# hey-yahei/Quantization.MXNet

Hardware: AMD Instinct MI355X
Metric: images/sec int8-sim MobileNet1.0 (per-layer W8A8, online input quant) (higher is better)
Workload: dtype f32

## Files before the change

### include/fakequant.h

```cpp
#ifndef FAKEQUANT_H_
#define FAKEQUANT_H_

#include <stddef.h>
#include <stdint.h>

#ifdef __cplusplus
extern "C" {
#endif

#define FQ_OK 0
#define FQ_ERR_INVALID 1
#define FQ_ERR_HIP 2

typedef void* fqStream_t;

#define FQ_ACT_SIGNED 1u
#define FQ_ACT_LO_NEG_MAX 2u
#define FQ_ACT_NO_ABS 4u
#define FQ_ACT_NO_EPS 8u

#define FQ_CODES_INT8 0
#define FQ_CODES_UINT8 1
#define FQ_CODES_RANGE 2
#define FQ_CODES_SCALE 3
// ... 10 lines not shown
#define FQ_KERNEL_HISTOGRAM 4
#define FQ_KERNEL_BN_ACT 5
#define FQ_KERNEL_DWCONV 6
#define FQ_KERNEL_PWCONV 7
#define FQ_KERNEL_STEM 8
#define FQ_KERNEL_POOL 9
#define FQ_KERNEL_GLOBAL_MAX 10
#define FQ_KERNEL_CONV3X3 11
#define FQ_KERNEL_DENSE 12
#define FQ_KERNEL_COUNT 13
int fq_profile_enable(int on);
int fq_profile_reset(void);
int fq_profile_read(int kernel_id, double* total_ms, int64_t* launches, double* total_bytes);
int fq_profile_read_moved(int kernel_id, double* total_moved_bytes);
int fq_profile_calibrate(void* scratch, int repeats, double* pair_ms, double* null_kernel_ms, fqStream_t stream);
int fq_profile_launch_overhead(void* scratch, int repeats, double spin_us, double* overhead_ms, double* spin_ms,
                               fqStream_t stream);

size_t fq_act_workspace_bytes(int64_t n);

int fq_absmax_per_sample(const float* x, int64_t n, int64_t inner, unsigned flags, float* out_max,
                         fqStream_t stream);

int fq_batch_mean(const float* v, int64_t n, float* out, fqStream_t stream);
int fq_batch_mean_rows(const float* v, int64_t rows, int64_t n, int64_t row_stride, float* out, fqStream_t stream);

int fq_stat_rows_sum(const float* v, int64_t rows, int64_t n, int64_t row_stride, double* out, fqStream_t stream);
int fq_mean_from_sums(const double* sums, int64_t rows, float* out, fqStream_t stream);

int fq_batch_mean_gathered(const float* packs, int world, int64_t stride, float* out, fqStream_t stream);

int fq_fake_quant_online(const float* x, float* y, int64_t n, int64_t inner, int width, unsigned flags,
                         float* out_current_max, int32_t* codes, void* ws, fqStream_t stream);

int fq_fake_quant_offline(const float* x, float* y, int64_t n, int64_t inner, const float* threshold, int width,
                          unsigned flags, float* out_current_max, int32_t* codes, void* ws, fqStream_t stream);

int fq_fake_quant_online_prestat(const float* x, float* y, int64_t n, int64_t inner, const float* stat, int width,
                                 unsigned flags, float* out_current_max, int32_t* codes, fqStream_t stream);

#define FQ_ACT_NONE 0
#define FQ_ACT_RELU 1
#define FQ_ACT_RELU6 2
#define FQ_STAT_PREZEROED 0x100
int fq_bn_act_stat(const float* x, float* y, int64_t n, int64_t c, int64_t hw, const float* scale,
                   const float* shift, int act, float* stat_out, fqStream_t stream);
int fq_bn_act_maxpool_stat(const float* x, float* y, int64_t n, int64_t c, int64_t h, int64_t w, const float* scale,
                           const float* shift, int act, float* stat_out, fqStream_t stream);

int fq_add_act_stat(const float* a, const float* b, float* y, int64_t n, int64_t inner, int act, float* stat_out,
                    fqStream_t stream);

int fq_bn_act_stat_hist(const float* x, float* y, int64_t n, int64_t c, int64_t hw, const float* scale,
                        const float* shift, int act, float* stat_out, const float* hist_max, int bins, uint64_t* hist,
                        uint32_t* neg_count, fqStream_t stream);
int fq_add_act_stat_hist(const float* a, const float* b, float* y, int64_t n, int64_t inner, int act, float* stat_out,
                         const float* hist_max, int bins, uint64_t* hist, uint32_t* neg_count, fqStream_t stream);

int fq_bn_add_act_stat(const float* x, const float* residual, float* y, int64_t n, int64_t c, int64_t hw, const float* scale,
                       const float* shift, int act, float* stat_out, fqStream_t stream);
int fq_bn_add_act_stat_hist(const float* x, const float* residual, float* y, int64_t n, int64_t c, int64_t hw,
                            const float* scale, const float* shift, int act, float* stat_out, const float* hist_max, int bins,
                            uint64_t* hist, uint32_t* neg_count, fqStream_t stream);

int fq_global_avg_pool_stat(const float* x, float* y, int64_t n, int64_t c, int64_t hw, int flags, float* stat_out,
                            fqStream_t stream);

int fq_gemm_i8_codes(const int8_t* xcodes, const int8_t* wcodes, const int32_t* wsum, int32_t* out, int64_t n,
                     int64_t l, int64_t k_pad, int64_t cout, int zoff, fqStream_t stream);

int fq_eval_counters(const float* logits, const int64_t* labels, int64_t n, int64_t classes, float* counters,
                     fqStream_t stream);

int fq_stem_conv3x3s2(const float* x, const float* w_tap_major, const float* bias, float* y, int64_t n, int64_t cin,
                      int64_t cout, int64_t h, int64_t w, const float* bn_scale, const float* bn_shift, int act,
                      float* stat_out, fqStream_t stream);
int fq_stem_conv3x3s2_c16(const float* x, const float* w_tap_major, const float* bias, void* y16, int64_t n, int64_t cin,
                          int64_t cout, int64_t h, int64_t w, const float* bn_scale, const float* bn_shift, int act,
                          float* stat_out, const float* out_thr, int out_width, unsigned out_flags, fqStream_t stream);
int fq_stem_conv7x7s2(const float* x, const float* w_tap_major, const float* bias, float* y, int64_t n, int64_t cin,
                      int64_t cout, int64_t h, int64_t w, const float* bn_scale, const float* bn_shift, int act,
                      float* stat_out, fqStream_t stream);
int fq_stem_conv7x7s2_pool_supported(int64_t h, int64_t w);
int fq_stem_conv7x7s2_pool(const float* x, const float* w_tap_major, const float* bias, float* y, int64_t n, int64_t cin,
                           int64_t cout, int64_t h, int64_t w, const float* bn_scale, const float* bn_shift, int act,
                           float* stat_out, fqStream_t stream);

int fq_dwconv3x3(const float* x, const float* w, const float* bias, float* y, int64_t n, int64_t c, int64_t h,
                 int64_t wdt, int stride, const float* in_stat, const float* in_thr, int in_width, unsigned in_flags,
                 float* out_current_max, const float* bn_scale, const float* bn_shift, int act, float* stat_out,
                 fqStream_t stream, void* x_codes_out);

int fq_weight_codes(const float* w, int64_t rows, int64_t row_len, int rows_per_scale, int width, int64_t row_pad,
                    int64_t rows_pad, int8_t* codes, float* scales, int32_t* rowsum, void* ws, fqStream_t stream);
#define FQ_PW_FORM(f) ((f) << 12)
size_t fq_pwconv_workspace_bytes(int64_t n, int64_t cin_pad, int64_t hw);
int fq_pwconv_i8(const float* x, const int8_t* wcodes, const float* wscale, const int32_t* wsum, const float* bias,
                 float* y, int64_t n, int64_t cin, int64_t cin_pad, int64_t cout, int64_t hw, const float* in_stat,
                 const float* in_thr, int in_width, unsigned in_flags, float* out_current_max,
                 const float* bn_scale, const float* bn_shift, int act, float* stat_out, void* ws,
                 fqStream_t stream);

size_t fq_dense_i8_eval_workspace_bytes(int64_t n, int64_t cout);
int fq_dense_i8_eval(const float* x, const int8_t* wcodes, const float* wscale, const int32_t* wsum, const float* bias,
                     float* y, int64_t n, int64_t cin, int64_t cin_pad, int64_t cout, const float* in_stat,
                     const float* in_thr, int in_width, unsigned in_flags, float* out_current_max,
                     const int64_t* labels, float* counters, void* eval_ws, void* ws, fqStream_t stream);

int fq_pwconv_i8_strided(const float* x, const int8_t* wcodes, const float* wscale, const int32_t* wsum,
                         const float* bias, float* y, int64_t n, int64_t cin, int64_t cin_pad, int64_t cout, int64_t h,
                         int64_t w, int stride, const float* in_stat, const float* in_thr, int in_width,
                         unsigned in_flags, float* out_current_max, const float* bn_scale, const float* bn_shift,
                         int act, float* stat_out, const float* residual, void* ws, fqStream_t stream);

int fq_pwconv_i8_sub2_supported(int64_t cin, int64_t cout);
int fq_pwconv_i8_sub2(const float* x, const int8_t* wcodes, const float* wscale, const int32_t* wsum, const float* bias,
                      float* y, int64_t n, int64_t cin, int64_t cin_pad, int64_t cout, int64_t h, int64_t w,
                      const float* in_stat, const float* in_thr, int in_width, unsigned in_flags, float* out_current_max,
                      const float* bn_scale, const float* bn_shift, int act, float* stat_out, const float* residual, void* ws,
                      fqStream_t stream);

int fq_pwconv_i8_shortcut_supported(int64_t cin, int64_t cin2, int64_t cout);
int fq_pwconv_i8_shortcut(const float* x, const int8_t* wcodes, const float* wscale, const int32_t* wsum, const float* bias,
                          float* y, int64_t n, int64_t cin, int64_t cin_pad, int64_t cout, int64_t hw, const float* in_stat,
                          const float* in_thr, int in_width, unsigned in_flags, float* out_current_max, const float* bn_scale,
                          const float* bn_shift, int act, float* stat_out, const float* x2, const int8_t* wcodes2,
                          const float* wscale2, const int32_t* wsum2, int64_t cin2, int64_t cin2_pad, const float* in_stat2,
                          const float* in_thr2, int in_width2, unsigned in_flags2, float* out_current_max2,
                          const float* bn_scale2, const float* bn_shift2, fqStream_t stream);

int fq_pwconv_i8_shortcut_c16(const void* x, const int8_t* wcodes, const float* wscale, const int32_t* wsum, const float* bias,
                              float* y, void* y16, int64_t n, int64_t cin, int64_t cin_pad, int64_t cout, int64_t hw,
                              const float* in_stat, const float* in_thr, int in_width, unsigned in_flags, float* out_current_max,
                              const float* bn_scale, const float* bn_shift, int act, float* stat_out, const void* x2, int x2_is_c16,
                              const int8_t* wcodes2, const float* wscale2, const int32_t* wsum2, int64_t cin2, int64_t cin2_pad,
                              const float* in_stat2, const float* in_thr2, int in_width2, unsigned in_flags2,
                              float* out_current_max2, const float* bn_scale2, const float* bn_shift2, const float* out_thr,
                              int out_width, unsigned out_flags, fqStream_t stream);

int fq_pwconv_i8_gap_supported(int64_t n, int64_t cin, int64_t cout, int64_t hw, int has_residual);
int fq_pwconv_i8_gap(const float* x, const int8_t* wcodes, const float* wscale, const int32_t* wsum, const float* bias,
                     float* y, int64_t n, int64_t cin, int64_t cin_pad, int64_t cout, int64_t hw, const float* in_stat,
                     const float* in_thr, int in_width, unsigned in_flags, float* out_current_max, const float* bn_scale,
                     const float* bn_shift, int act, float* stat_out, const float* residual, void* ws, fqStream_t stream);

int fq_pwconv_i8_stat_supported(int64_t n, int64_t cin, int64_t cout, int64_t hw, int64_t front_h, int64_t front_wdt);
int fq_pwconv_i8_stat(const float* x, const int8_t* wcodes, const float* wscale, const int32_t* wsum, const float* bias,
                      int64_t n, int64_t cin, int64_t cin_pad, int64_t cout_pad, int64_t cout, int64_t hw,
                      const float* in_stat, const float* in_thr, int in_width, unsigned in_flags, float* out_current_max,
                      const float* bn_scale, const float* bn_shift, int act, float* stat_out, void* x_codes_out,
                      fqStream_t stream, const void* front_codes, const float* front_w, const float* front_bias,
                      const float* front_bn_scale, const float* front_bn_shift, int front_act, const float* front_in_stat,
                      const float* front_in_thr, int front_width, unsigned front_flags, int64_t front_h, int64_t front_wdt);
int fq_pwdw_fused_supported(int64_t n, int64_t cin, int64_t cout, int64_t h, int64_t w, int stride);
int fq_debug_fast_quotient(const float* c, int64_t n, const float* d, float* out, int* took_fast_path, fqStream_t stream);
int fq_pwdw_fused(const float* x, const int8_t* wcodes, const float* wscale, const int32_t* wsum, const float* pw_bias,
                  int64_t n, int64_t cin, int64_t cin_pad, int64_t cout_pad, int64_t cout, int64_t h, int64_t w,
                  const float* in_stat, const float* in_thr, int in_width, unsigned in_flags, const float* pw_bn_scale,
                  const float* pw_bn_shift, int pw_act, const float* mid_stat, const float* mid_thr, int mid_width,
                  unsigned mid_flags, float* mid_current_max, const float* dw_w, const float* dw_bias, int dw_stride,
                  const float* dw_bn_scale, const float* dw_bn_shift, int dw_act, float* y, float* stat_out,
                  const void* x_codes, fqStream_t stream);

int fq_pwconv_i8_c16(const void* x, int x_is_c16, const int8_t* wcodes, const float* wscale, const int32_t* wsum,
                     const float* bias, void* y, int64_t n, int64_t cin, int64_t cin_pad, int64_t cout, int64_t h, int64_t w,
                     int stride, const float* in_stat, const float* in_thr, int in_width, unsigned in_flags,
                     float* out_current_max, const float* bn_scale, const float* bn_shift, int act, float* stat_out,
                     const float* residual, const float* out_thr, int out_width, unsigned out_flags, void* ws,
                     fqStream_t stream);

int fq_pwconv_i8_c16_dual(const void* x, const int8_t* wcodes, const float* wscale, const int32_t* wsum, const float* bias,
                          float* y, void* y16, int64_t n, int64_t cin, int64_t cin_pad, int64_t cout, int64_t h, int64_t w,
                          const float* in_stat, const float* in_thr, int in_width, unsigned in_flags, float* out_current_max,
                          const float* bn_scale, const float* bn_shift, int act, float* stat_out, const float* residual,
                          const float* out_thr, int out_width, unsigned out_flags, void* ws, fqStream_t stream);
int fq_pwconv_i8_c16_dual_sub2(const void* x, const int8_t* wcodes, const float* wscale, const int32_t* wsum, const float* bias,
                               float* y, void* y16, int64_t n, int64_t cin, int64_t cin_pad, int64_t cout, int64_t h, int64_t w,
                               const float* in_stat, const float* in_thr, int in_width, unsigned in_flags,
                               float* out_current_max, const float* bn_scale, const float* bn_shift, int act, float* stat_out,
                               const float* residual, const float* out_thr, int out_width, unsigned out_flags, void* ws,
                               fqStream_t stream);

int fq_conv3x3_i8(const float* x, const int8_t* wcodes, const float* wscale, const int32_t* wsum, const float* bias,
                  float* y, int64_t n, int64_t cin, int64_t cout, int64_t h, int64_t w, const float* in_stat,
                  const float* in_thr, int in_width, unsigned in_flags, float* out_current_max, const float* bn_scale,
                  const float* bn_shift, int act, float* stat_out, fqStream_t stream);

int fq_conv3x3_i8_c16(const void* x, int x_is_c16, const int8_t* wcodes, const float* wscale, const int32_t* wsum,
                      const float* bias, void* y, int64_t n, int64_t cin, int64_t cout, int64_t h, int64_t w,
                      const float* in_stat, const float* in_thr, int in_width, unsigned in_flags, float* out_current_max,
                      const float* bn_scale, const float* bn_shift, int act, float* stat_out, const float* out_thr,
                      int out_width, unsigned out_flags, fqStream_t stream);

int fq_dwconv3x3_c16(const void* x, const float* w, const float* bias, void* y, int64_t n, int64_t c, int64_t h, int64_t wdt,
                     int stride, const float* in_stat, const float* in_thr, int in_width, unsigned in_flags,
                     float* out_current_max, const float* bn_scale, const float* bn_shift, int act, float* stat_out,
                     const float* out_thr, int out_width, unsigned out_flags, fqStream_t stream);

int fq_weight_slices(const float* w, int64_t rows, int64_t row_len, int64_t row_pad, int64_t rows_pad, int8_t* codes,
                     float* pscale, int32_t* rowsum, void* ws, fqStream_t stream);
int fq_conv3x3_i8_sliced(const float* x, const int8_t* wslices, const float* pscale, const int32_t* wsum, const float* bias,
                         float* y, int64_t n, int64_t cin, int64_t cout, int64_t h, int64_t w, const float* in_stat,
                         const float* in_thr, int in_width, unsigned in_flags, float* out_current_max,
                         const float* bn_scale, const float* bn_shift, int act, float* stat_out, fqStream_t stream);

int fq_ste_forward(const float* x, float* y, int64_t rows, int64_t row_len, const float* scales, int has_clip,
                   float clip_lo, float clip_hi, float eps, fqStream_t stream);

size_t fq_weight_workspace_bytes(int64_t rows);
int fq_weight_fake_quant(const float* w, float* w_q, int64_t rows, int64_t row_len, int width, float* scales_out,
                         void* ws, fqStream_t stream);

int fq_wino_weight_fake_quant(const float* w, float* w_q, int64_t cout, int64_t cin_g, int t, const float* G,
                              const float* GI, const float* GTI, int width, float* scales_out, void* ws,
                              fqStream_t stream);

#define FQ_COMM_UNIQUE_ID_BYTES 128
#define FQ_COMM_SUM 0
#define FQ_COMM_MAX 1
int fq_comm_unique_id(void* id128);
int fq_comm_init(int rank, int world, const void* id128);
int fq_comm_world(void);
int fq_allreduce_f32(float* buf, int64_t count, int op, fqStream_t stream);
int fq_allreduce_f64(double* buf, int64_t count, int op, fqStream_t stream);
int fq_allreduce_i64(int64_t* buf, int64_t count, int op, fqStream_t stream);
int fq_comm_destroy(void);

int fq_ema_update(float* state, const float* current, int64_t count, double momentum, fqStream_t stream);

int fq_global_max(const float* x, int64_t numel, float* out, fqStream_t stream);

int fq_histogram_accumulate(const float* x, int64_t numel, const float* max_dev, int bins, uint64_t* hist,
                            uint32_t* neg_count, fqStream_t stream);
int fq_hist_to_float(const uint64_t* hist, float* out, int64_t count, fqStream_t stream);

size_t fq_kl_workspace_bytes(int64_t L, int bins);
int fq_kl_search(const float* hist, int64_t L, int bins, int levels, int min_bins, int32_t* out_best, void* ws,
                 fqStream_t stream);

int fq_quantize_codes(const float* x, int32_t* codes, int64_t numel, int mode, float* range_dev, void* ws,
                      fqStream_t stream);
int fq_dequantize(const int32_t* codes, float* y, int64_t numel, const float* scale_dev, fqStream_t stream);

size_t fq_qconv_weights_bytes(int64_t cin, int64_t cout, int kh, int kw, int sh, int sw, int ph, int pw, int groups);
int fq_qconv_kind(int64_t cin, int64_t cout, int kh, int kw, int sh, int sw, int ph, int pw, int groups);
int fq_qconv_weights_prepare(const float* w, int64_t cin, int64_t cout, int kh, int kw, int sh, int sw, int ph, int pw,
                             int groups, int weight_mode, float w_min, float w_max, void* wbuf, void* ws,
                             fqStream_t stream);
size_t fq_qconv_workspace_bytes(int64_t cout);
int fq_qconv_workspace_init(void* ws, fqStream_t stream);
int fq_qconv2d_forward(const float* x, const float* w, const void* wbuf, const float* bias, float* y, int64_t n, int64_t cin,
                       int64_t h, int64_t wdt, int64_t cout, int kh, int kw, int sh, int sw, int ph, int pw, int groups,
                       int input_mode, float in_min, float in_max, const float* in_stat, int act, const float* bn_scale,
                       const float* bn_shift, float* stat_out, void* ws, int force_direct, fqStream_t stream);

#ifdef __cplusplus
}
#endif
#endif
```

### quantization/mxnet_amd/_lib.py

```python
import ctypes
import os

__all__ = ["LIB", "check_call", "load", "library_path", "FakeQuantError", "EXPORTS"]

_HERE = os.path.dirname(os.path.abspath(__file__))
_LIB_PATH = os.environ.get("FQ_LIB_PATH") or os.path.join(_HERE, "csrc", "libfakequant.so")

c_f32p = ctypes.POINTER(ctypes.c_float)
c_i32p = ctypes.POINTER(ctypes.c_int32)
c_u32p = ctypes.POINTER(ctypes.c_uint32)
c_u64p = ctypes.POINTER(ctypes.c_uint64)
_vp, _i64, _int, _uint, _f32 = ctypes.c_void_p, ctypes.c_int64, ctypes.c_int, ctypes.c_uint, ctypes.c_float

EXPORTS = {
    "fq_last_error": (ctypes.c_char_p, []),
    "fq_version": (_int, []),
    "fq_build_id": (ctypes.c_char_p, []),
    "fq_device_info": (_int, [ctypes.c_char_p, _int, ctypes.POINTER(_int), ctypes.POINTER(_int)]),
    "fq_profile_enable": (_int, [_int]),
    "fq_profile_reset": (_int, []),
    "fq_profile_read": (_int, [_int, ctypes.POINTER(ctypes.c_double), ctypes.POINTER(_i64),
                               ctypes.POINTER(ctypes.c_double)]),
    "fq_profile_read_moved": (_int, [_int, ctypes.POINTER(ctypes.c_double)]),
    "fq_profile_calibrate": (_int, [_vp, _int, ctypes.POINTER(ctypes.c_double), ctypes.POINTER(ctypes.c_double), _vp]),
    "fq_profile_launch_overhead": (_int, [_vp, _int, ctypes.c_double, ctypes.POINTER(ctypes.c_double),
                                          ctypes.POINTER(ctypes.c_double), _vp]),
    "fq_act_workspace_bytes": (ctypes.c_size_t, [_i64]),
    "fq_absmax_per_sample": (_int, [_vp, _i64, _i64, _uint, _vp, _vp]),
    "fq_batch_mean": (_int, [_vp, _i64, _vp, _vp]),
    "fq_batch_mean_gathered": (_int, [_vp, _int, _i64, _vp, _vp]),
    "fq_stat_rows_sum": (_int, [_vp, _i64, _i64, _i64, _vp, _vp]),
    "fq_mean_from_sums": (_int, [_vp, _i64, _vp, _vp]),
    "fq_batch_mean_rows": (_int, [_vp, _i64, _i64, _i64, _vp, _vp]),
    "fq_fake_quant_online": (_int, [_vp, _vp, _i64, _i64, _int, _uint, _vp, _vp, _vp, _vp]),
    "fq_fake_quant_online_prestat": (_int, [_vp, _vp, _i64, _i64, _vp, _int, _uint, _vp, _vp, _vp]),
    "fq_bn_act_stat": (_int, [_vp, _vp, _i64, _i64, _i64, _vp, _vp, _int, _vp, _vp]),
    "fq_bn_act_maxpool_stat": (_int, [_vp, _vp, _i64, _i64, _i64, _i64, _vp, _vp, _int, _vp, _vp]),
    "fq_add_act_stat": (_int, [_vp, _vp, _vp, _i64, _i64, _int, _vp, _vp]),
    "fq_bn_act_stat_hist": (_int, [_vp, _vp, _i64, _i64, _i64, _vp, _vp, _int, _vp, _vp, _int, _vp, _vp, _vp]),
    "fq_add_act_stat_hist": (_int, [_vp, _vp, _vp, _i64, _i64, _int, _vp, _vp, _int, _vp, _vp, _vp]),
    "fq_bn_add_act_stat": (_int, [_vp, _vp, _vp, _i64, _i64, _i64, _vp, _vp, _int, _vp, _vp]),
    "fq_bn_add_act_stat_hist": (_int, [_vp, _vp, _vp, _i64, _i64, _i64, _vp, _vp, _int, _vp, _vp, _int, _vp, _vp, _vp]),
    "fq_global_avg_pool_stat": (_int, [_vp, _vp, _i64, _i64, _i64, _int, _vp, _vp]),
    "fq_gemm_i8_codes": (_int, [_vp, _vp, _vp, _vp, _i64, _i64, _i64, _i64, _int, _vp]),
    "fq_eval_counters": (_int, [_vp, _vp, _i64, _i64, _vp, _vp]),
    "fq_stem_conv3x3s2": (_int, [_vp, _vp, _vp, _vp, _i64, _i64, _i64, _i64, _i64, _vp, _vp, _int, _vp, _vp]),
    "fq_stem_conv7x7s2": (_int, [_vp, _vp, _vp, _vp, _i64, _i64, _i64, _i64, _i64, _vp, _vp, _int, _vp, _vp]),
    "fq_stem_conv7x7s2_pool": (_int, [_vp, _vp, _vp, _vp, _i64, _i64, _i64, _i64, _i64, _vp, _vp, _int, _vp, _vp]),
    "fq_stem_conv7x7s2_pool_supported": (_int, [_i64, _i64]),
    "fq_stem_conv3x3s2_c16": (_int, [_vp, _vp, _vp, _vp, _i64, _i64, _i64, _i64, _i64, _vp, _vp, _int, _vp, _vp, _int, _uint, _vp]),
    "fq_dwconv3x3": (_int, [_vp, _vp, _vp, _vp, _i64, _i64, _i64, _i64, _int, _vp, _vp, _int, _uint, _vp, _vp, _vp, _int,
                            _vp, _vp, _vp]),
    "fq_dwconv3x3_c16": (_int, [_vp, _vp, _vp, _vp, _i64, _i64, _i64, _i64, _int, _vp, _vp, _int, _uint, _vp, _vp, _vp, _int,
                                _vp, _vp, _int, _uint, _vp]),
    "fq_weight_codes": (_int, [_vp, _i64, _i64, _int, _int, _i64, _i64, _vp, _vp, _vp, _vp, _vp]),
    "fq_pwconv_workspace_bytes": (ctypes.c_size_t, [_i64, _i64, _i64]),
    "fq_pwconv_i8": (_int, [_vp, _vp, _vp, _vp, _vp, _vp, _i64, _i64, _i64, _i64, _i64, _vp, _vp, _int, _uint, _vp, _vp,
                            _vp, _int, _vp, _vp, _vp]),
    "fq_pwconv_i8_stat_supported": (_int, [_i64, _i64, _i64, _i64, _i64, _i64]),
    "fq_pwconv_i8_stat": (_int, [_vp, _vp, _vp, _vp, _vp, _i64, _i64, _i64, _i64, _i64, _i64, _vp, _vp, _int, _uint, _vp, _vp,
                                 _vp, _int, _vp, _vp, _vp, _vp, _vp, _vp, _vp, _vp, _int, _vp, _vp, _int, _uint, _i64, _i64]),
    "fq_pwdw_fused_supported": (_int, [_i64, _i64, _i64, _i64, _i64, _int]),
    "fq_pwdw_fused": (_int, [_vp, _vp, _vp, _vp, _vp, _i64, _i64, _i64, _i64, _i64, _i64, _i64, _vp, _vp, _int, _uint, _vp,
                             _vp, _int, _vp, _vp, _int, _uint, _vp, _vp, _vp, _int, _vp, _vp, _int, _vp, _vp, _vp, _vp]),
    "fq_debug_fast_quotient": (_int, [_vp, _i64, _vp, _vp, _vp, _vp]),
    "fq_dense_i8_eval_workspace_bytes": (ctypes.c_size_t, [_i64, _i64]),
    "fq_dense_i8_eval": (_int, [_vp, _vp, _vp, _vp, _vp, _vp, _i64, _i64, _i64, _i64, _vp, _vp, _int, _uint, _vp, _vp, _vp,
                                _vp, _vp, _vp]),
    "fq_pwconv_i8_strided": (_int, [_vp, _vp, _vp, _vp, _vp, _vp, _i64, _i64, _i64, _i64, _i64, _i64, _int, _vp, _vp, _int,
                                    _uint, _vp, _vp, _vp, _int, _vp, _vp, _vp, _vp]),
    "fq_pwconv_i8_shortcut_supported": (_int, [_i64, _i64, _i64]),
    "fq_pwconv_i8_shortcut": (_int, [_vp, _vp, _vp, _vp, _vp, _vp, _i64, _i64, _i64, _i64, _i64, _vp, _vp, _int, _uint, _vp, _vp,
                                     _vp, _int, _vp, _vp, _vp, _vp, _vp, _i64, _i64, _vp, _vp, _int, _uint, _vp, _vp, _vp, _vp]),
    "fq_pwconv_i8_shortcut_c16": (_int, [_vp, _vp, _vp, _vp, _vp, _vp, _vp, _i64, _i64, _i64, _i64, _i64, _vp, _vp, _int, _uint, _vp,
                                         _vp, _vp, _int, _vp, _vp, _int, _vp, _vp, _vp, _i64, _i64, _vp, _vp, _int, _uint, _vp, _vp,
                                         _vp, _vp, _int, _uint, _vp]),
    "fq_pwconv_i8_gap_supported": (_int, [_i64, _i64, _i64, _i64, _int]),
    "fq_pwconv_i8_gap": (_int, [_vp, _vp, _vp, _vp, _vp, _vp, _i64, _i64, _i64, _i64, _i64, _vp, _vp, _int, _uint, _vp, _vp, _vp,
                                _int, _vp, _vp, _vp, _vp]),
    "fq_pwconv_i8_sub2_supported": (_int, [_i64, _i64]),
    "fq_pwconv_i8_sub2": (_int, [_vp, _vp, _vp, _vp, _vp, _vp, _i64, _i64, _i64, _i64, _i64, _i64, _vp, _vp, _int,
                                 _uint, _vp, _vp, _vp, _int, _vp, _vp, _vp, _vp]),
    "fq_pwconv_i8_c16": (_int, [_vp, _int, _vp, _vp, _vp, _vp, _vp, _i64, _i64, _i64, _i64, _i64, _i64, _int, _vp, _vp, _int,
                                _uint, _vp, _vp, _vp, _int, _vp, _vp, _vp, _int, _uint, _vp, _vp]),
    "fq_pwconv_i8_c16_dual": (_int, [_vp, _vp, _vp, _vp, _vp, _vp, _vp, _i64, _i64, _i64, _i64, _i64, _i64, _vp, _vp, _int,
                                     _uint, _vp, _vp, _vp, _int, _vp, _vp, _vp, _int, _uint, _vp, _vp]),
    "fq_pwconv_i8_c16_dual_sub2": (_int, [_vp, _vp, _vp, _vp, _vp, _vp, _vp, _i64, _i64, _i64, _i64, _i64, _i64, _vp, _vp, _int,
                                          _uint, _vp, _vp, _vp, _int, _vp, _vp, _vp, _int, _uint, _vp, _vp]),
    "fq_conv3x3_i8": (_int, [_vp, _vp, _vp, _vp, _vp, _vp, _i64, _i64, _i64, _i64, _i64, _vp, _vp, _int, _uint, _vp, _vp,
                             _vp, _int, _vp, _vp]),
    "fq_conv3x3_i8_c16": (_int, [_vp, _int, _vp, _vp, _vp, _vp, _vp, _i64, _i64, _i64, _i64, _i64, _vp, _vp, _int, _uint, _vp,
                                 _vp, _vp, _int, _vp, _vp, _int, _uint, _vp]),
    "fq_conv3x3_i8_sliced": (_int, [_vp, _vp, _vp, _vp, _vp, _vp, _i64, _i64, _i64, _i64, _i64, _vp, _vp, _int, _uint, _vp,
                                    _vp, _vp, _int, _vp, _vp]),
    "fq_weight_slices": (_int, [_vp, _i64, _i64, _i64, _i64, _vp, _vp, _vp, _vp, _vp]),
    "fq_fake_quant_offline": (_int, [_vp, _vp, _i64, _i64, _vp, _int, _uint, _vp, _vp, _vp, _vp]),
    "fq_ste_forward": (_int, [_vp, _vp, _i64, _i64, _vp, _int, _f32, _f32, _f32, _vp]),
    "fq_weight_workspace_bytes": (ctypes.c_size_t, [_i64]),
    "fq_weight_fake_quant": (_int, [_vp, _vp, _i64, _i64, _int, _vp, _vp, _vp]),
    "fq_wino_weight_fake_quant": (_int, [_vp, _vp, _i64, _i64, _int, c_f32p, c_f32p, c_f32p, _int, _vp, _vp, _vp]),
    "fq_comm_unique_id": (_int, [_vp]),
    "fq_comm_init": (_int, [_int, _int, _vp]),
    "fq_comm_world": (_int, []),
    "fq_allreduce_f32": (_int, [_vp, _i64, _int, _vp]),
    "fq_allreduce_f64": (_int, [_vp, _i64, _int, _vp]),
    "fq_allreduce_i64": (_int, [_vp, _i64, _int, _vp]),
    "fq_comm_destroy": (_int, []),
    "fq_ema_update": (_int, [_vp, _vp, _i64, ctypes.c_double, _vp]),
    "fq_global_max": (_int, [_vp, _i64, _vp, _vp]),
    "fq_histogram_accumulate": (_int, [_vp, _i64, _vp, _int, _vp, _vp, _vp]),
    "fq_hist_to_float": (_int, [_vp, _vp, _i64, _vp]),
    "fq_kl_workspace_bytes": (ctypes.c_size_t, [_i64, _int]),
    "fq_kl_search": (_int, [_vp, _i64, _int, _int, _int, _vp, _vp, _vp]),
    "fq_quantize_codes": (_int, [_vp, _vp, _i64, _int, _vp, _vp, _vp]),
    "fq_dequantize": (_int, [_vp, _vp, _i64, _vp, _vp]),
    "fq_qconv_weights_bytes": (ctypes.c_size_t, [_i64, _i64, _int, _int, _int, _int, _int, _int, _int]),
    "fq_qconv_kind": (_int, [_i64, _i64, _int, _int, _int, _int, _int, _int, _int]),
    "fq_qconv_weights_prepare": (_int, [_vp, _i64, _i64, _int, _int, _int, _int, _int, _int, _int, _int, _f32, _f32, _vp,
                                        _vp, _vp]),
    "fq_qconv_workspace_bytes": (ctypes.c_size_t, [_i64]),
    "fq_qconv_workspace_init": (_int, [_vp, _vp]),
    "fq_qconv2d_forward": (_int, [_vp, _vp, _vp, _vp, _vp, _i64, _i64, _i64, _i64, _i64, _int, _int, _int, _int, _int, _int,
                                  _int, _int, _f32, _f32, _vp, _int, _vp, _vp, _vp, _vp, _int, _vp]),
}

FQ_ACT_SIGNED, FQ_ACT_LO_NEG_MAX, FQ_ACT_NO_ABS, FQ_ACT_NO_EPS = 1, 2, 4, 8
FQ_CODES_INT8, FQ_CODES_UINT8, FQ_CODES_RANGE, FQ_CODES_SCALE = 0, 1, 2, 3


class FakeQuantError(RuntimeError):
    """Error raised by the HIP library (the analogue of MXNetError)."""


class _Missing(object):
    def __init__(self, why):
        self._why = why

    def __getattr__(self, name):
        raise FakeQuantError(
            "libfakequant.so is not available (%s). Build it with `python -m quantization.mxnet_amd.csrc.build` "
            "(needs hipcc, target gfx950). There is no CPU fallback for the fake-quant path." % self._why)


def library_path():
    return _LIB_PATH


def load(path=None):
    import torch
    path = path or _LIB_PATH
    if not os.path.exists(path):
        return _Missing("no file at %s" % path)
    try:
        lib = ctypes.CDLL(path, mode=ctypes.RTLD_GLOBAL)
    except OSError as e:
        return _Missing(str(e))
    for name, (restype, argtypes) in EXPORTS.items():
        fn = getattr(lib, name)
        fn.restype = restype
        fn.argtypes = argtypes
    return lib


LIB = load()


def check_call(ret):
    if ret != 0:
        raise FakeQuantError(LIB.fq_last_error().decode("utf-8", "replace"))
```

### quantization/mxnet_amd/csrc/fq_core.hip

```cpp
#include "fq_common.h"

namespace fqi {

thread_local char g_err[512] = "";

int fail(int code, const char* fmt, ...) {
  va_list ap;
  va_start(ap, fmt);
  vsnprintf(g_err, sizeof(g_err), fmt, ap);
  va_end(ap);
  return code;
}

bool g_prof_on = false;
std::mutex g_prof_mu;
std::vector<ProfRec> g_prof;

void prof_push(const ProfRec& r) {
  std::lock_guard<std::mutex> lk(g_prof_mu);
  g_prof.push_back(r);
}

int num_cu() {
  constexpr int kMaxDev = 64;
  static int cache[kMaxDev] = {0};
  int dev = 0;
  if (hipGetDevice(&dev) != hipSuccess || dev < 0 || dev >= kMaxDev) return 256;
  if (cache[dev] == 0) {
    hipDeviceProp_t prop;
    int cu = 0;
    if (hipGetDeviceProperties(&prop, dev) == hipSuccess) cu = prop.multiProcessorCount;
    cache[dev] = cu > 0 ? cu : 256;
  }
  return cache[dev];
}

int max_lds_bytes() {
  constexpr int kMaxDev = 64;
  static int cache[kMaxDev] = {0};
  int dev = 0;
  if (hipGetDevice(&dev) != hipSuccess || dev < 0 || dev >= kMaxDev) return 160 * 1024;
  if (cache[dev] == 0) {
    int v = 0;
    if (hipDeviceGetAttribute(&v, hipDeviceAttributeMaxSharedMemoryPerBlock, dev) != hipSuccess || v <= 0) v = 160 * 1024;
    cache[dev] = v;
  }
  return cache[dev];
}

int env_int(const char* name, int dflt) {
  const char* e = getenv(name);
  return (e && *e) ? atoi(e) : dflt;
}

constexpr int kPolNtLoad_ = 1, kPolNtStore_ = 2, kPolReverse_ = 4;
int stream_policy(int kernel_id, int64_t numel) {
  static const int ov_stat = env_int("FQ_POLICY_STAT", -1);
  static const int ov_on = env_int("FQ_POLICY_ONLINE", -1);
  static const int ov_off = env_int("FQ_POLICY_OFFLINE", -1);
  static const int64_t big = (int64_t)env_int("FQ_POLICY_BIG_MB", 160) * 1000000;
  const bool is_big = numel * (int64_t)sizeof(float) >= big;
  switch (kernel_id) {
    case FQ_KERNEL_STAT:
      return ov_stat >= 0 ? ov_stat : 0;
    case FQ_KERNEL_APPLY_ONLINE:
      if (ov_on >= 0) return ov_on;
      return is_big ? (kPolReverse_ | kPolNtLoad_ | kPolNtStore_) : kPolReverse_;
    default:
      if (ov_off >= 0) return ov_off;
      return is_big ? (kPolNtLoad_ | kPolNtStore_) : 0;
  }
}

}

using namespace fqi;

extern "C" {

const char* fq_last_error(void) { return g_err; }
int fq_version(void) { return 101; }
#ifndef FQ_BUILD_ID
#define FQ_BUILD_ID "0000000000000000000000000000000000000000"
#endif
const char* fq_build_id(void) {
  static const char id[] = "FQ_BUILD_ID=" FQ_BUILD_ID;
  return id + 12;
}

int fq_device_info(char* arch, int arch_len, int* compute_units, int* wavefront) {
  int dev = 0;
  FQ_HIP(hipGetDevice(&dev));
  hipDeviceProp_t prop;
  FQ_HIP(hipGetDeviceProperties(&prop, dev));
  if (arch != nullptr && arch_len > 0) {
    strncpy(arch, prop.gcnArchName, (size_t)arch_len - 1);
    arch[arch_len - 1] = 0;
  }
  if (compute_units) *compute_units = prop.multiProcessorCount;
  if (wavefront) *wavefront = prop.warpSize;
  return FQ_OK;
}

int fq_profile_enable(int on) {
  g_prof_on = on != 0;
  return FQ_OK;
}

int fq_profile_reset(void) {
  std::lock_guard<std::mutex> lk(g_prof_mu);
  for (auto& r : g_prof) {
    (void)hipEventDestroy(r.a);
    (void)hipEventDestroy(r.b);
  }
  g_prof.clear();
  return FQ_OK;
}

int fq_profile_read_moved(int kernel_id, double* total_moved_bytes) {
  FQ_REQUIRE(kernel_id >= 0 && kernel_id < FQ_KERNEL_COUNT, "fq_profile_read_moved: bad kernel id %d", kernel_id);
  FQ_REQUIRE(total_moved_bytes, "fq_profile_read_moved: null pointer");
  std::lock_guard<std::mutex> lk(g_prof_mu);
  double moved = 0.0;
  for (auto& r : g_prof)
    if (r.kid == kernel_id) moved += r.moved;
  *total_moved_bytes = moved;
  return FQ_OK;
}

int fq_profile_read(int kernel_id, double* total_ms, int64_t* launches, double* total_bytes) {
  FQ_REQUIRE(kernel_id >= 0 && kernel_id < FQ_KERNEL_COUNT, "fq_profile_read: bad kernel id %d", kernel_id);
  FQ_REQUIRE(total_ms && launches && total_bytes, "fq_profile_read: null pointer");
  std::lock_guard<std::mutex> lk(g_prof_mu);
  double ms = 0.0, bytes = 0.0;
  int64_t cnt = 0;
  for (auto& r : g_prof) {
    if (r.kid != kernel_id) continue;
    FQ_HIP(hipEventSynchronize(r.b));
    float t = 0.f;
    FQ_HIP(hipEventElapsedTime(&t, r.a, r.b));
    ms += t;
    bytes += r.bytes;
    ++cnt;
  }
  *total_ms = ms;
  *launches = cnt;
  *total_bytes = bytes;
  return FQ_OK;
}

}

namespace {
__global__ void spin_kernel(unsigned long long* __restrict__ t, unsigned long long ticks) {
  const unsigned long long t0 = wall_clock64();
  unsigned long long t1 = t0;
  while (t1 - t0 < ticks) t1 = wall_clock64();
  if (threadIdx.x == 0) {
    t[0] = t0;
    t[1] = t1;
  }
}
}

extern "C" {

int fq_profile_calibrate(void* scratch, int repeats, double* pair_ms, double* null_kernel_ms, fqStream_t stream) {
  FQ_REQUIRE(scratch && pair_ms && null_kernel_ms && repeats > 0 && repeats <= 4096, "fq_profile_calibrate: bad arguments");
  hipStream_t st = (hipStream_t)stream;
  std::vector<hipEvent_t> ev((size_t)repeats * 2 + 2);
  for (auto& e : ev) FQ_HIP(hipEventCreate(&e));
  for (int i = 0; i < repeats; ++i) {
    FQ_HIP(hipEventRecord(ev[2 * i], st));
    hipLaunchKernelGGL(fill_kernel, dim3(1), dim3(64), 0, st, (float*)scratch, (int64_t)1, 0.0f);
    FQ_HIP(hipEventRecord(ev[2 * i + 1], st));
  }
  FQ_HIP(hipEventRecord(ev[2 * repeats], st));
  for (int i = 0; i < repeats; ++i)
    hipLaunchKernelGGL(fill_kernel, dim3(1), dim3(64), 0, st, (float*)scratch, (int64_t)1, 0.0f);
  FQ_HIP(hipEventRecord(ev[2 * repeats + 1], st));
  FQ_HIP(hipEventSynchronize(ev.back()));
  std::vector<float> ts;
  for (int i = 0; i < repeats; ++i) {
    float t = 0.f;
    FQ_HIP(hipEventElapsedTime(&t, ev[2 * i], ev[2 * i + 1]));
    ts.push_back(t);
  }
  float all = 0.f;
  FQ_HIP(hipEventElapsedTime(&all, ev[2 * repeats], ev[2 * repeats + 1]));
  for (auto& e : ev) (void)hipEventDestroy(e);
  std::sort(ts.begin(), ts.end());
  *pair_ms = ts[ts.size() / 2];
  *null_kernel_ms = (double)all / repeats;
  return FQ_OK;
}

int fq_profile_launch_overhead(void* scratch, int repeats, double spin_us, double* overhead_ms, double* spin_ms,
                               fqStream_t stream) {
  FQ_REQUIRE(scratch && overhead_ms && spin_ms && repeats > 0 && repeats <= 4096 && spin_us > 0 && spin_us < 1e5,
             "fq_profile_launch_overhead: bad arguments");
  hipStream_t st = (hipStream_t)stream;
  int dev = 0, khz = 0;
  FQ_HIP(hipGetDevice(&dev));
  FQ_HIP(hipDeviceGetAttribute(&khz, hipDeviceAttributeWallClockRate, dev));
  FQ_REQUIRE(khz > 0, "fq_profile_launch_overhead: the device reports no wall clock rate");
  const unsigned long long ticks = (unsigned long long)(spin_us * 1e-3 * khz);
  std::vector<hipEvent_t> ev((size_t)repeats * 2 + 2);
  for (auto& e : ev) FQ_HIP(hipEventCreate(&e));
  unsigned long long* t = (unsigned long long*)scratch;
  for (int i = 0; i < repeats; ++i) {
    FQ_HIP(hipEventRecord(ev[2 * i], st));
    hipLaunchKernelGGL(spin_kernel, dim3(1), dim3(64), 0, st, t + 2 * i, ticks);
    FQ_HIP(hipEventRecord(ev[2 * i + 1], st));
  }
  FQ_HIP(hipEventRecord(ev[2 * repeats], st));
  for (int i = 0; i < repeats; ++i) hipLaunchKernelGGL(spin_kernel, dim3(1), dim3(64), 0, st, t + 2 * i, ticks);
  FQ_HIP(hipEventRecord(ev[2 * repeats + 1], st));
  FQ_LAUNCH_CHECK();
  FQ_HIP(hipStreamSynchronize(st));
  std::vector<unsigned long long> host((size_t)repeats * 2);
  FQ_HIP(hipMemcpy(host.data(), t, host.size() * sizeof(unsigned long long), hipMemcpyDeviceToHost));
  std::vector<double> pair, own;
  for (int i = 0; i < repeats; ++i) {
    float el = 0.f;
    FQ_HIP(hipEventElapsedTime(&el, ev[2 * i], ev[2 * i + 1]));
    pair.push_back((double)el);
    own.push_back((double)(host[2 * i + 1] - host[2 * i]) / (double)khz);
  }
  float all = 0.f;
  FQ_HIP(hipEventElapsedTime(&all, ev[2 * repeats], ev[2 * repeats + 1]));
  for (auto& e : ev) (void)hipEventDestroy(e);
  std::sort(pair.begin(), pair.end());
  std::sort(own.begin(), own.end());
  *overhead_ms = pair[pair.size() / 2] - (double)all / repeats;
// ... 6 lines not shown
```

### quantization/mxnet_amd/csrc/fq_front_layout.h

```cpp
#pragma once

#include <cstddef>
#include <cstdint>

#if defined(__HIPCC__)
#define FQ_FL_FN __host__ __device__ __forceinline__
#else
#define FQ_FL_FN inline
#endif

namespace fqi {

constexpr int kFrontRows = 8;
constexpr int kFrontBandBytes = 32768;
constexpr int kStatLdsPerCU = 160 * 1024, kStatLdsMax = 120 * 1024;

struct FrontLayout {
  int js;
  int pl;
};

FQ_FL_FN FrontLayout front_layout(int q, int rows) {
  FrontLayout l;
  l.js = rows * q + ((8 - rows * q) & 15);
  l.pl = 4 * l.js + 16;
  return l;
}

FQ_FL_FN int front_slot(FrontLayout l, int p) { return (p & 3) * l.js + (p >> 2); }

FQ_FL_FN int front_byte(FrontLayout l, int c, int p) { return (((c >> 2) * l.pl + front_slot(l, p)) << 2) + (c & 3); }

inline size_t front_band_bytes(int q, int rows, int cin) { return (size_t)((cin + 3) / 4) * front_layout(q, rows).pl * 4; }

FQ_FL_FN int front_channel(int c0, int wave, int segs, int seg) { return c0 + wave * segs + seg; }

FQ_FL_FN int mfma_row_pixel(int i32) { return 16 * ((i32 >> 2) & 1) + 4 * (i32 >> 3) + (i32 & 3); }

inline int stat_wg_per_cu(size_t lds, int cap) {
  const int by_lds = (int)((size_t)kStatLdsPerCU / (lds + 1024));
  return by_lds > cap ? cap : (by_lds < 1 ? 1 : by_lds);
}

inline int front_rows_pick(int64_t n, int64_t h, int64_t w, int cin, size_t lds_fixed, int num_cu, int wg_cap, int forced = 0) {
  const int q = (int)(w / 4);
  int rmax = (int)(kFrontBandBytes / (32 * w));
  rmax = rmax > kFrontRows ? kFrontRows : rmax;
  rmax = rmax > h ? (int)h : rmax;
  while (rmax >= 1 && lds_fixed + front_band_bytes(q, rmax, cin) > (size_t)kStatLdsMax) --rmax;
  if (rmax < 1) return 0;
  if (forced > 0) return forced < rmax ? forced : rmax;
  double best = 1e30;
  int best_r = rmax;
  bool best_whole = false;
  for (int r = rmax; r >= 1; --r) {
    const int64_t wgs = n * ((h + r - 1) / r);
    const int64_t slots = (int64_t)num_cu * stat_wg_per_cu(lds_fixed + front_band_bytes(q, r, cin), wg_cap);
    const int64_t grid = wgs < slots ? wgs : slots, rounds = (wgs + grid - 1) / grid;
    const double cost = (double)(rounds * ((grid + num_cu - 1) / num_cu) * (r + 2));
    const bool whole = (r * w) % 32 == 0;
    if (cost < best - 1e-9 || (cost < best + 1e-9 && whole && !best_whole)) {
      best = cost;
      best_r = r;
      best_whole = whole;
    }
  }
  return best_r;
}

}
```

### quantization/mxnet_amd/csrc/fq_pwdw.hip

```cpp
#include "fq_pw.h"

#include "fq_front_layout.h"

#include <climits>

namespace {

struct PwDwGeom {
  int Cin, KTS, Cout, H, W, Ho, Wo;
  int strips, ctg, bands, RB;
  int zoff, pitch;
  int vw;
  FastDiv qv;
};

constexpr int kRowSlack = 8;

template <int KT, int S> struct PwDwRing {
  static constexpr int NB = S == 1 ? 2 : (KT <= 2 ? 3 : 4);
  static constexpr int NR = 2;
};

template <int KT, int CW, int S, int LZ, int FAST, int CODES>
__global__ __launch_bounds__(512) void pwdw_kernel(
    const float* __restrict__ x, const int8_t* __restrict__ xc, const int8_t* __restrict__ wfrag, const float* __restrict__ wscale,
    const int* __restrict__ wsum, const float* __restrict__ bias1, PwDwGeom g, const float* __restrict__ in_stat, int n,
    const float* __restrict__ in_thr, float levels1, int lo_neg1, float eps, const float* __restrict__ bn1_scale,
    const float* __restrict__ bn1_shift, int act1, const float* __restrict__ mid_stat, const float* __restrict__ mid_thr,
    float levels2, int lo_neg2, float* __restrict__ mid_cur_out, const float* __restrict__ dww,
    const float* __restrict__ bias2, const float* __restrict__ bn2_scale, const float* __restrict__ bn2_shift, int act2,
    float* __restrict__ y, float* __restrict__ stat_out) {
  constexpr int NB = CODES ? 1 : PwDwRing<KT, S>::NB, NR = CODES ? PwDwRing<KT, S>::NR : 1;
  extern __shared__ __attribute__((aligned(16))) unsigned char pwdw_smem[];
  __shared__ float red[8];
  const int CT = g.ctg * CW;
  v4i* ldsW = reinterpret_cast<v4i*>(pwdw_smem);
  const int rb_stride = g.Cout * g.pitch + kRowSlack;
  float* rowbuf = reinterpret_cast<float*>(pwdw_smem + (size_t)CT * KT * 1024) + kRowSlack;
  constexpr bool kDwLds = S == 1;
  float* ldsK = rowbuf + 2 * rb_stride;

  const int lane = threadIdx.x & 63, wave = threadIdx.x >> 6;
  const int h = lane >> 5, i32 = lane & 31;
  const int s = wave % g.strips, cgi = wave / g.strips;
  const int band = (int)(blockIdx.x % (unsigned)g.bands);
  const int smp = n - 1 - (int)(blockIdx.x / (unsigned)g.bands);
  const int HW = g.H * g.W;

  int c0;
  if (S == 1) c0 = (s == g.strips - 1) ? g.W - 30 : 30 * s;
  else c0 = 30 * s;
  const int pl = 16 * ((i32 >> 2) & 1) + 4 * (i32 >> 3) + (i32 & 3);
  int col_ld = c0 + pl - 1;
  col_ld = col_ld < 0 ? 0 : (col_ld >= g.W ? g.W - 1 : col_ld);
  const fq_rsrc rs = CODES ? make_rsrc(xc + (int64_t)smp * 2 * KT * HW * 16, (int64_t)2 * KT * HW * 16)
                           : make_rsrc(x + (int64_t)smp * g.Cin * HW, (int64_t)g.Cin * HW * 4);
  const unsigned voff = CODES ? (unsigned)((h * HW + col_ld) * 16) : (unsigned)((16 * h * HW + col_ld) * 4);
  const int obase = S == 1 ? c0 + 16 * h - 1 : 15 * s + 8 * h;

  const int ro0 = band * g.RB;
  const int ro1 = ro0 + g.RB < g.Ho ? ro0 + g.RB : g.Ho;
  const int t_first = S == 1 ? ro0 - 1 : 2 * ro0 - 1;
  const int t_last = S == 1 ? ro1 : 2 * (ro1 - 1) + 1;
  float* yb = y + (int64_t)smp * g.Cout * g.Ho * g.Wo;

  float raw[NB][16];
#pragma unroll
  for (int b = 0; b < NB; ++b)
#pragma unroll
    for (int i = 0; i < 16; ++i) raw[b][i] = 0.0f;
  auto issue = [&](int t, int kt, float (&v)[16]) __attribute__((always_inline)) {
    if (t < 0 || t >= g.H || t > t_last) return;
    const unsigned so = (unsigned)((kt * 32 * HW + t * g.W) * 4);
#pragma unroll
    for (int i = 0; i < 16; ++i) v[i] = buf_ld_f32(rs, voff, so + (unsigned)(i * HW * 4));
  };
  v4i crow[NR][KT];
#pragma unroll
  for (int b = 0; b < NR; ++b)
#pragma unroll
    for (int kt = 0; kt < KT; ++kt) crow[b][kt] = (v4i){0, 0, 0, 0};
  auto issue_row = [&](int t, v4i (&v)[KT]) __attribute__((always_inline)) {
    if (t < 0 || t >= g.H || t > t_last) return;
#pragma unroll
    for (int kt = 0; kt < KT; ++kt) v[kt] = buf_ld_v4i(rs, voff, (unsigned)((2 * kt * HW + t * g.W) * 16));
  };
  if constexpr (CODES) {
#pragma unroll
    for (int r = 0; r < NR - 1; ++r) issue_row(t_first + r, crow[r]);
  } else {
#pragma unroll
    for (int q = 0; q < NB - 1; ++q) issue(t_first + q / KT, q % KT, raw[q]);
  }
  FQ_PIN();

  const float max1 = input_threshold(in_stat, n, in_thr, nullptr, false);
  const float max2 = input_threshold(mid_stat, n, mid_thr, mid_cur_out, blockIdx.x == 0);
  const QParams q1 = make_qparams(max1, levels1, lo_neg1 != 0, eps);
  const QParams q2 = make_qparams(max2, levels2, lo_neg2 != 0, eps);
  const int ubias1 = 128 - g.zoff;
  const unsigned nn_xor1 = fq_nonneg_xor(ubias1);
  const bool relu6 = act1 == FQ_ACT_RELU6;
  const float top = relu6 ? 6.0f : INFINITY;

  for (int idx = threadIdx.x; idx < CT * KT * 64; idx += blockDim.x) {
    const int f = idx >> 6, ct = f / KT, kt = f - ct * KT;
    ldsW[idx] = *reinterpret_cast<const v4i*>(wfrag + (((int64_t)ct * g.KTS + kt) << 10) + ((idx & 63) << 4));
  }

  float k_sxw[CW], k_b1[CW], k_bsc1[CW], k_bsh1[CW], k_w[CW][9], k_b2[CW], k_bsc2[CW], k_bsh2[CW];
  int k_zs[CW];
  const bool has_b1 = bias1 != nullptr, has_bn1 = bn1_scale != nullptr, has_b2 = bias2 != nullptr, has_bn2 = bn2_scale != nullptr;
#pragma unroll
  for (int j = 0; j < CW; ++j) {
    const int c = (cgi * CW + j) * 32 + i32;
    k_sxw[j] = q1.scale * wscale[c];
    k_zs[j] = g.zoff * wsum[c];
    k_b1[j] = has_b1 ? bias1[c] : 0.0f;
    k_bsc1[j] = has_bn1 ? bn1_scale[c] : 1.0f;
    k_bsh1[j] = has_bn1 ? bn1_shift[c] : 0.0f;
#pragma unroll
    for (int t = 0; t < 9; ++t) k_w[j][t] = kDwLds ? 0.0f : dww[c * 9 + t];
    k_b2[j] = (has_b2 && !kDwLds) ? bias2[c] : 0.0f;
    k_bsc2[j] = (has_bn2 && !kDwLds) ? bn2_scale[c] : 1.0f;
    k_bsh2[j] = (has_bn2 && !kDwLds) ? bn2_shift[c] : 0.0f;
  }
  if (kDwLds)
    for (int c = threadIdx.x; c < g.Cout; c += blockDim.x) {
#pragma unroll
      for (int t = 0; t < 9; ++t) ldsK[c * 13 + t] = dww[c * 9 + t];
      ldsK[c * 13 + 9] = has_b2 ? bias2[c] : 0.0f;
      ldsK[c * 13 + 10] = has_bn2 ? bn2_scale[c] : 1.0f;
      ldsK[c * 13 + 11] = has_bn2 ? bn2_shift[c] : 0.0f;
    }
  const bool zero_left = (S == 1 && LZ != 0) ? (h == (LZ >> 4)) : (s == 0 && h == 0);
  const bool zero_right = S == 1 && s == g.strips - 1 && h == 1;
  __syncthreads();
  FQ_PIN();

  float m = 0.0f;
  const FastQuot fq1 = make_fast_quot(q1.denom), fq2 = make_fast_quot(q2.denom);
  auto body = [&](auto nn_c) __attribute__((always_inline)) {
    constexpr bool NN = decltype(nn_c)::value;
    auto pack_x = [&](float a, float b, float c, float d) __attribute__((always_inline)) {
      if constexpr (NN) {
        auto code = [&](float v) __attribute__((always_inline)) {
          int r;
          const float Q = fast_quot(fq_clip(v, q1), fq1);
          asm("v_cvt_rpi_i32_f32 %0, %1" : "=v"(r) : "v"(Q));
          return (unsigned)r;
        };
        unsigned u = code(a);
        u |= code(b) << 8;
        u |= code(c) << 16;
        u |= code(d) << 24;
        return (int)(u ^ nn_xor1);
      } else {
        return fq_pack4<false>(a, b, c, d, q1, ubias1, nn_xor1);
      }
    };
    constexpr int NO = S == 1 ? 16 : 8;
    float sumA[CW][NO], sumB[S == 1 ? CW : 1][NO];
#pragma unroll
    for (int j = 0; j < CW; ++j)
#pragma unroll
      for (int k = 0; k < NO; ++k) {
        sumA[j][k] = 0.0f;
        if (S == 1) sumB[j][k] = 0.0f;
      }
    QParams qc = q2;
    if (FAST) qc.hi = fminf(q2.hi, top);

    auto row = [&](int t, auto ph_c) __attribute__((always_inline)) {
      constexpr int PH = decltype(ph_c)::value;
      const bool row_ok = t >= 0 && t < g.H;
      v4i afrag[KT];
      if constexpr (CODES) {
        issue_row(t + NR - 1, crow[(PH + NR - 1) % NR]);
        FQ_PIN();
#pragma unroll
        for (int kt = 0; kt < KT; ++kt) afrag[kt] = crow[PH % NR][kt];
      } else {
#pragma unroll
        for (int kt = 0; kt < KT; ++kt) {
          const int qn = kt + NB - 1;
          issue(t + qn / KT, qn % KT, raw[(PH * KT + kt + NB - 1) % NB]);
          FQ_PIN();
          float (&mine)[16] = raw[(PH * KT + kt) % NB];
          v4i f;
#pragma unroll
          for (int d = 0; d < 4; ++d)
            f[d] = pack_x(mine[4 * d + 0], mine[4 * d + 1], mine[4 * d + 2], mine[4 * d + 3]);
          asm volatile("" : "+v"(f[0]), "+v"(f[1]), "+v"(f[2]), "+v"(f[3]));
          afrag[kt] = f;
          FQ_PIN();
        }
      }
      const int r_emit = S == 1 ? t - 1 : (t - 1) >> 1;
      const bool emits = (S == 1 || (t & 1)) && r_emit >= ro0 && r_emit < ro1;
      float* rbuf = rowbuf + (r_emit & 1) * rb_stride;
#pragma unroll
      for (int j = 0; j < CW; ++j) {
        const int ct = cgi * CW + j;
        const float* kc = ldsK + (ct * 32 + i32) * 13;
        auto finish_store = [&](const float (&sum)[NO]) __attribute__((always_inline)) {
          if (!emits) return;
          float* dst = rbuf + (ct * 32 + i32) * g.pitch + obase;
          const float b2 = kDwLds ? kc[9] : k_b2[j], bsc2 = kDwLds ? kc[10] : k_bsc2[j], bsh2 = kDwLds ? kc[11] : k_bsh2[j];
#pragma unroll
          for (int k = 0; k < NO; ++k) {
            float o;
            if (FAST == 0) {
              o = dw_finish<kEpiRuntime>(sum[k], has_b2, b2, has_bn2, bsc2, bsh2, act2);
            } else {
              o = sum[k] * bsc2;
              o = o + bsh2;
              o = __builtin_amdgcn_fmed3f(o, 0.0f, top);
            }
            if (S == 1 && k == 0) {
              if (h == 1) dst[k] = o;
            } else if (k == NO - 1) {
              if (h == 0) dst[k] = o;
            } else {
              dst[k] = o;
            }
          }
        };
        if (!row_ok) {
          if (S == 1) {
            finish_store(sumA[j]);
#pragma unroll
            for (int k = 0; k < 16; ++k) {
              sumA[j][k] = sumB[j][k];
              sumB[j][k] = 0.0f;
            }
          } else if (t & 1) {
            finish_store(sumA[j]);
#pragma unroll
            for (int c = 0; c < 8; ++c) sumA[j][c] = 0.0f;
          }
          FQ_PIN();
          continue;
        }
        float e[18];
        {
          v16i acc = {0, 0, 0, 0, 0, 0, 0, 0, 0, 0, 0, 0, 0, 0, 0, 0};
          int wl = lane;
          asm volatile("" : "+v"(wl));
#pragma unroll
          for (int kt = 0; kt < KT; ++kt)
            acc = __builtin_amdgcn_mfma_i32_32x32x32_i8(afrag[kt], ldsW[((ct * KT + kt) << 6) + wl], acc, 0, 0, 0);
#pragma unroll
          for (int k = 0; k < 16; ++k) {
            float v = (float)(acc[k] + k_zs[j]) * k_sxw[j];
            if (FAST == 0) {
              if (has_b1) v = v + k_b1[j];
              if (has_bn1) {
                v = v * k_bsc1[j];
                v = v + k_bsh1[j];
              }
              v = act_rt(v, act1);
              e[k + 1] = NN ? truncf(fast_quot(fq_clip(v, q2), fq2) + 0.49999997f) * q2.scale : fq_code(v, q2) * q2.scale;
            } else {
              v = v * k_bsc1[j];
              v = v + k_bsh1[j];
              if (NN) e[k + 1] = truncf(fast_quot(fq_clip(v, qc), fq2) + 0.49999997f) * q2.scale;
              else e[k + 1] = fq_code(act_rt(v, relu6 ? FQ_ACT_RELU6 : FQ_ACT_RELU), q2) * q2.scale;
            }
          }
          e[1 + (LZ & 15)] = zero_left ? 0.0f : e[1 + (LZ & 15)];
          if (S == 1) e[16] = zero_right ? 0.0f : e[16];
          const auto sw = __builtin_amdgcn_permlane32_swap(__float_as_uint(e[1]), __float_as_uint(e[16]), false, false);
          e[0] = __uint_as_float(sw[0]);
          e[17] = __uint_as_float(sw[1]);
        }
        float w[9];
        if (!kDwLds) {
#pragma unroll
          for (int t = 0; t < 9; ++t) w[t] = k_w[j][t];
        }
        if (S == 1) {
          w[6] = kc[6]; w[7] = kc[7]; w[8] = kc[8];
#pragma unroll
          for (int k = 0; k < 16; ++k) {
            float a = sumA[j][k];
            a = fmaf(w[6], e[k], a);
            a = fmaf(w[7], e[k + 1], a);
            a = fmaf(w[8], e[k + 2], a);
            sumA[j][k] = a;
          }
          finish_store(sumA[j]);
          w[0] = kc[0]; w[1] = kc[1]; w[2] = kc[2]; w[3] = kc[3]; w[4] = kc[4]; w[5] = kc[5];
#pragma unroll
          for (int k = 0; k < 16; ++k) {
            float b = sumB[j][k];
            b = fmaf(w[3], e[k], b);
            b = fmaf(w[4], e[k + 1], b);
            b = fmaf(w[5], e[k + 2], b);
            float c = 0.0f;
            c = fmaf(w[0], e[k], c);
            c = fmaf(w[1], e[k + 1], c);
            c = fmaf(w[2], e[k + 2], c);
            sumA[j][k] = b;
            sumB[j][k] = c;
          }
        } else {
          if (t & 1) {
#pragma unroll
            for (int c = 0; c < 8; ++c) {
              float a = sumA[j][c];
              a = fmaf(w[6], e[2 * c + 1], a);
              a = fmaf(w[7], e[2 * c + 2], a);
              a = fmaf(w[8], e[2 * c + 3], a);
              sumA[j][c] = a;
            }
            finish_store(sumA[j]);
#pragma unroll
            for (int c = 0; c < 8; ++c) {
              float a = 0.0f;
              a = fmaf(w[0], e[2 * c + 1], a);
              a = fmaf(w[1], e[2 * c + 2], a);
              a = fmaf(w[2], e[2 * c + 3], a);
              sumA[j][c] = a;
            }
          } else {
#pragma unroll
            for (int c = 0; c < 8; ++c) {
              float a = sumA[j][c];
              a = fmaf(w[3], e[2 * c + 1], a);
              a = fmaf(w[4], e[2 * c + 2], a);
              a = fmaf(w[5], e[2 * c + 3], a);
              sumA[j][c] = a;
            }
          }
        }
        FQ_PIN();
      }
      if (emits) {
        __syncthreads();
        const unsigned per_row = g.qv.d;
        const int vecs = g.Cout * (int)per_row;
        float* yr = yb + (int64_t)r_emit * g.Wo;
        for (int idx = threadIdx.x; idx < vecs; idx += blockDim.x) {
          const unsigned c = fast_div((unsigned)idx, g.qv), qd = (unsigned)idx - c * per_row;
          if (g.vw == 4) {
            const float* src = rbuf + c * g.pitch + 4 * qd;
            const f4 v = (f4){src[0], src[1], src[2], src[3]};
            m = fmaxf(fmaxf(m, fmaxf(fabsf(v.x), fabsf(v.y))), fmaxf(fabsf(v.z), fabsf(v.w)));
            *reinterpret_cast<f4*>(yr + (int64_t)c * g.Ho * g.Wo + 4 * qd) = v;
          } else if (g.vw == 2) {
            const float* src = rbuf + c * g.pitch + 2 * qd;
            const float2 v = make_float2(src[0], src[1]);
            m = fmaxf(m, fmaxf(fabsf(v.x), fabsf(v.y)));
            *reinterpret_cast<float2*>(yr + (int64_t)c * g.Ho * g.Wo + 2 * qd) = v;
          } else {
            const float v = rbuf[c * g.pitch + qd];
            m = fmaxf(m, fabsf(v));
            yr[(int64_t)c * g.Ho * g.Wo + qd] = v;
          }
        }
      }
    };
    constexpr int U = CODES ? NR : ((KT % NB == 0) ? 1 : ((2 * KT) % NB == 0 ? 2 : NB));
    static_assert(U <= 3, "the row loop below unrolls at most three phases");
    using std::integral_constant;
    for (int t = t_first; t <= t_last; t += U) {
      row(t, integral_constant<int, 0>{});
      if (U > 1 && t + 1 <= t_last) row(t + 1, integral_constant<int, 1 % U>{});
      if (U > 2 && t + 2 <= t_last) row(t + 2, integral_constant<int, 2 % U>{});
    }
  };
  using std::false_type;
  using std::true_type;
  if (fq_nonneg(q1) && fq_nonneg(q2) && fq1.ok && fq2.ok) body(true_type{});
  else body(false_type{});

  if (stat_out != nullptr) {
    m = wave_max_nonneg(m);
    __syncthreads();
    if (lane == 0) red[wave] = m;
    __syncthreads();
    if (threadIdx.x == 0) {
      float mm = 0.0f;
      for (int w = 0; w < (int)(blockDim.x >> 6); ++w) mm = fmaxf(mm, red[w]);
      if (__float_as_uint(mm) != 0u) FQ_STAT_FLUSH_MAX(reinterpret_cast<unsigned*>(stat_out) + smp, __float_as_uint(mm));
    }
  }
}

__device__ __forceinline__ void buf_st_v4i(fq_rsrc r, unsigned voff, v4i v) {
  typedef unsigned v4u __attribute__((ext_vector_type(4)));
  __builtin_amdgcn_raw_buffer_store_b128(__builtin_bit_cast(v4u, v), r, (int)voff, 0, 0);
  asm volatile("s_nop 1" : : "v"(v));
}

struct PwStatGeom {
  int Cin, KTS, Cout, CT, HW;
  int64_t cols, tiles;
  int zoff;
  int table;
  FastDiv hw;
};

struct PwFrontArgs {
  const int8_t* codes;
  const float *w, *bias, *bn_scale, *bn_shift;
  const float *in_stat, *in_thr;
  float levels;
  int act;
  int H, W, Q, segs, R, bands;
  FrontLayout lay;
};

template <int KT, int FEPI = -1, bool FSIGNED = false>
__global__ __launch_bounds__(kBlock, 3) void pw_stat_kernel(
    const float* __restrict__ x, const int8_t* __restrict__ wfrag, const float* __restrict__ wscale,
    const int* __restrict__ wsum, const float* __restrict__ bias, PwStatGeom g, const float* __restrict__ in_stat, int n,
    const float* __restrict__ in_thr, float levels, int lo_neg, float eps, float* __restrict__ cur_max_out,
    const float* __restrict__ bn_scale, const float* __restrict__ bn_shift, int act, float* __restrict__ stat_out,
    int8_t* __restrict__ x_codes_out, PwFrontArgs fa) {
  constexpr bool FRONT = FEPI >= 0;
  static_assert(!FRONT || KT == 1, "the front layer is built for one 32-channel slab");
  extern __shared__ __attribute__((aligned(16))) unsigned char pst_smem[];
  v4i* ldsW = reinterpret_cast<v4i*>(pst_smem);
  int* c_zs = reinterpret_cast<int*>(pst_smem + (size_t)g.CT * KT * 1024);
  float* c_k = reinterpret_cast<float*>(c_zs + g.CT * 32);
  int* accs = reinterpret_cast<int*>(c_k + 4 * g.CT * 32);
  float* dwk = reinterpret_cast<float*>(accs + 4 * g.CT * 128);
  unsigned char* zbuf = reinterpret_cast<unsigned char*>(dwk + g.Cin * 12);
  const int lane = threadIdx.x & 63, wave = threadIdx.x >> 6;
  const int h = lane >> 5, i32 = lane & 31;
  const unsigned HW = (unsigned)g.HW, cols = (unsigned)g.cols;
  const int64_t nwaves = (int64_t)gridDim.x * 4, wid = (int64_t)blockIdx.x * 4 + wave;
  const int64_t n_bands = FRONT ? (int64_t)(g.cols / g.HW) * fa.bands : 0;
  const int64_t t_begin = FRONT ? n_bands * blockIdx.x / gridDim.x : g.tiles * wid / nwaves;
  const int64_t t_end = FRONT ? n_bands * (blockIdx.x + 1) / gridDim.x : g.tiles * (wid + 1) / nwaves;
  const int pl = mfma_row_pixel(i32);
  int* my = accs + (size_t)wave * g.CT * 128;
  constexpr int kSlots = 8;
  __shared__ unsigned k_stat[kSlots];
  if (threadIdx.x < kSlots) k_stat[threadIdx.x] = 0u;
  unsigned s_base;
  if constexpr (FRONT) {
    s_base = (unsigned)((t_begin < n_bands ? t_begin : n_bands - 1) / fa.bands);
  } else {
    const int64_t t0 = g.tiles * ((int64_t)blockIdx.x * 4) / nwaves;
    const unsigned j0 = (unsigned)(t0 < g.tiles ? t0 : g.tiles - 1) * 32u;
    s_base = fast_div(j0 < cols ? j0 : cols - 1, g.hw);
  }

  struct Pix { unsigned smp, p; };
  auto pix_of = [&](int64_t t) __attribute__((always_inline)) {
    unsigned j = (unsigned)t * 32u + (unsigned)pl;
    j = j < cols ? j : cols - 1;
    Pix r;
    r.smp = fast_div(j, g.hw);
    r.p = j - r.smp * HW;
    return r;
  };
  constexpr int NB = 3;
  const fq_rsrc rs = make_rsrc(x, (int64_t)(cols / HW) * g.Cin * HW * 4);
  auto issue = [&](int64_t t, int kt, float (&v)[16]) __attribute__((always_inline)) {
    if (t >= t_end) return;
    const Pix px = pix_of(t);
    const bool ok = kt * 32 + 16 * h < g.Cin;
    const unsigned vo = ok ? (unsigned)(((px.smp * (unsigned)g.Cin + 16u * h) * HW + px.p) * 4u) : 0x80000000u;
    const unsigned so = (unsigned)kt * 32u * HW * 4u;
#pragma unroll
    for (int i = 0; i < 16; ++i) v[i] = buf_ld_f32(rs, vo, so + (unsigned)i * HW * 4u);
  };
  float raw[NB][16];
#pragma unroll
  for (int b2 = 0; b2 < NB; ++b2)
#pragma unroll
    for (int i = 0; i < 16; ++i) raw[b2][i] = 0.0f;
  if constexpr (!FRONT) {
#pragma unroll
    for (int qq = 0; qq < NB - 1; ++qq) issue(t_begin + qq / KT, qq % KT, raw[qq]);
  }
  FQ_PIN();
  float fscale = 0.0f;
  if constexpr (FRONT) fscale = input_threshold(fa.in_stat, n, fa.in_thr, nullptr, false) / fa.levels;
  const float max_ = input_threshold(in_stat, n, in_thr, cur_max_out, blockIdx.x == 0);
  const QParams q = make_qparams(max_, levels, lo_neg != 0, eps);
  const int ubias = 128 - g.zoff;
  const unsigned nn_xor = fq_nonneg_xor(ubias);
  const bool wr_codes = x_codes_out != nullptr;
  const fq_rsrc rcodes = make_rsrc(x_codes_out, wr_codes ? (int64_t)(cols / HW) * 2 * KT * HW * 16 : 0);
  for (int idx = threadIdx.x; idx < g.CT * KT * 64; idx += kBlock) {
    const int f = idx >> 6, ct = f / KT, kt = f - ct * KT;
    ldsW[idx] = *reinterpret_cast<const v4i*>(wfrag + (((int64_t)ct * g.KTS + kt) << 10) + ((idx & 63) << 4));
  }
  const int nchs = g.CT * 32;
  for (int i = threadIdx.x; i < nchs; i += kBlock) {
    const bool okc = i < g.Cout;
    c_zs[i] = okc ? g.zoff * wsum[i] : 0;
    c_k[i] = okc ? wscale[i] : 0.0f;
    c_k[nchs + i] = (okc && bias != nullptr) ? bias[i] : 0.0f;
    c_k[2 * nchs + i] = (okc && bn_scale != nullptr) ? bn_scale[i] : 1.0f;
    c_k[3 * nchs + i] = (okc && bn_scale != nullptr) ? bn_shift[i] : 0.0f;
  }
  if constexpr (FRONT)
    for (int i = threadIdx.x; i < g.Cin; i += kBlock) {
#pragma unroll
      for (int t = 0; t < 9; ++t) dwk[i * 12 + t] = fa.w[i * 9 + t];
      dwk[i * 12 + 9] = fa.bias != nullptr ? fa.bias[i] : 0.0f;
      dwk[i * 12 + 10] = fa.bn_scale != nullptr ? fa.bn_scale[i] : 1.0f;
      dwk[i * 12 + 11] = fa.bn_scale != nullptr ? fa.bn_shift[i] : 0.0f;
    }
  auto reset = [&]() __attribute__((always_inline)) {
    for (int ct = 0; ct < g.CT; ++ct) {
      my[ct * 128 + lane] = INT_MIN;
      my[ct * 128 + 64 + lane] = INT_MAX;
    }
  };
  reset();
  __syncthreads();
  const bool has_bn = bn_scale != nullptr;
  auto flush = [&](unsigned smp) __attribute__((always_inline)) {
    float m = 0.0f;
    for (int ct = 0; ct < g.CT; ++ct) {
      const int c = ct * 32 + i32;
      int hi = my[ct * 128 + lane], lo = my[ct * 128 + 64 + lane];
      const int ohi = __shfl_xor(hi, 32, 64), olo = __shfl_xor(lo, 32, 64);
      hi = hi > ohi ? hi : ohi;
      lo = lo < olo ? lo : olo;
      if (c < g.Cout && hi >= lo) {
        hi += c_zs[c];
        lo += c_zs[c];
        const float sxw = q.scale * c_k[c];
        const float bch = c_k[nchs + c];
        const float bsc = c_k[2 * nchs + c], bsh = c_k[3 * nchs + c];
        auto f = [&](int a) {
          float v = (float)a * sxw;
          if (bias != nullptr) v = v + bch;
          if (has_bn) {
            v = v * bsc;
            v = v + bsh;
          }
          return fabsf(act_rt(v, act));
        };
        m = fmaxf(m, fmaxf(f(hi), f(lo)));
      }
    }
    m = wave_max_nonneg(m);
    if (lane == 0 && __float_as_uint(m) != 0u) {
      const unsigned slot = smp - s_base;
      if (g.table && slot < (unsigned)kSlots) atomicMax(&k_stat[slot], __float_as_uint(m));
      else FQ_STAT_FLUSH_MAX(reinterpret_cast<unsigned*>(stat_out) + smp, __float_as_uint(m));
    }
    reset();
  };
  v4i afrag[KT];
  const FastQuot fqx = make_fast_quot(q.denom);
  auto quant = [&](int kt, const float (&v)[16], auto nn_c) __attribute__((always_inline)) {
    v4i f;
#pragma unroll
    for (int d = 0; d < 4; ++d) {
      if constexpr (decltype(nn_c)::value) {
        unsigned u = 0u;
#pragma unroll
        for (int b = 0; b < 4; ++b) {
          int r;
          const float Q = fast_quot(fq_clip(v[4 * d + b], q), fqx);
          asm("v_cvt_rpi_i32_f32 %0, %1" : "=v"(r) : "v"(Q));
          u |= (unsigned)r << (8 * b);
        }
        f[d] = (int)(u ^ nn_xor);
      } else {
        f[d] = fq_pack4<false>(v[4 * d + 0], v[4 * d + 1], v[4 * d + 2], v[4 * d + 3], q, ubias, nn_xor);
      }
    }
    asm volatile("" : "+v"(f[0]), "+v"(f[1]), "+v"(f[2]), "+v"(f[3]));
    afrag[kt] = f;
  };
// ... 4 lines not shown
      v16i acc = {0, 0, 0, 0, 0, 0, 0, 0, 0, 0, 0, 0, 0, 0, 0, 0};
#pragma unroll
      for (int kt = 0; kt < KT; ++kt)
        acc = __builtin_amdgcn_mfma_i32_32x32x32_i8(afrag[kt], ldsW[((ct * KT + kt) << 6) + lane], acc, 0, 0, 0);
      int hi = INT_MIN, lo = INT_MAX;
      if (whole) {
#pragma unroll
        for (int k = 0; k < 16; k += 2) {
          hi = max(max(acc[k], acc[k + 1]), hi);
          lo = min(min(acc[k], acc[k + 1]), lo);
        }
      } else {
#pragma unroll
        for (int k = 0; k < 16; ++k) {
          const int p = 16 * h + k;
          const bool in = p >= plo && p < phi;
          hi = in && acc[k] > hi ? acc[k] : hi;
          lo = in && acc[k] < lo ? acc[k] : lo;
        }
      }
      atomicMax(&my[ct * 128 + lane], hi);
      atomicMin(&my[ct * 128 + 64 + lane], lo);
    }
  };
  unsigned cur = FRONT ? s_base : fast_div((unsigned)((t_begin < g.tiles ? t_begin : g.tiles - 1) * 32), g.hw);
  auto run_tile = [&](int64_t t, auto ph_c, auto nn_c) __attribute__((always_inline)) {
    constexpr int PH = decltype(ph_c)::value;
    const Pix px = pix_of(t);
    const unsigned cvo = ((px.smp * (unsigned)(2 * KT) + (unsigned)h) * HW + px.p) * 16u;
#pragma unroll
    for (int kt = 0; kt < KT; ++kt) {
      const int qn = kt + NB - 1;
      issue(t + qn / KT, qn % KT, raw[(PH * KT + kt + NB - 1) % NB]);
      FQ_PIN();
      quant(kt, raw[(PH * KT + kt) % NB], nn_c);
      if (wr_codes) buf_st_v4i(rcodes, cvo + (unsigned)(2 * kt) * HW * 16u, afrag[kt]);
      FQ_PIN();
    }
    const unsigned j0 = (unsigned)t * 32u, j1 = j0 + 31u < cols ? j0 + 31u : cols - 1;
    const unsigned s0 = fast_div(j0, g.hw), s1 = fast_div(j1, g.hw);
    if (s0 != cur) {
      flush(cur);
      cur = s0;
    }
    if (s0 == s1) {
      reduce_tile(0, 32);
    } else {
      const int pb = (int)(s1 * HW - j0);
      reduce_tile(0, pb);
      flush(cur);
      cur = s1;
      reduce_tile(pb, 32);
    }
    FQ_PIN();
  };
  auto run_all = [&](auto nn_c) __attribute__((always_inline)) {
    constexpr int U = (KT % NB == 0) ? 1 : NB;
    using std::integral_constant;
    for (int64_t t = t_begin; t < t_end; t += U) {
      run_tile(t, integral_constant<int, 0>{}, nn_c);
      if (U > 1 && t + 1 < t_end) run_tile(t + 1, integral_constant<int, 1 % U>{}, nn_c);
      if (U > 2 && t + 2 < t_end) run_tile(t + 2, integral_constant<int, 2 % U>{}, nn_c);
      if (U > 3 && t + 3 < t_end) run_tile(t + 3, integral_constant<int, 3 % U>{}, nn_c);
    }
  };
  auto run_front = [&](auto nn_c) __attribute__((always_inline)) {
    constexpr bool NN = decltype(nn_c)::value;
    constexpr int FE = FRONT ? FEPI : kEpiRuntime;
    const int Q = fa.Q, W = fa.W, H = fa.H;
    const int seg = lane / Q, pos = lane - seg * Q;
    const bool first = pos == 0, last = pos == Q - 1;
    const bool has_fb = fa.bias != nullptr, has_fbn = fa.bn_scale != nullptr;
    QParams qc = q;
    if (NN && FE != kEpiRuntime) qc.hi = FE == kEpiBnRelu6 ? fminf(q.hi, 6.0f) : q.hi;
    const unsigned* xc32 = reinterpret_cast<const unsigned*>(fa.codes);
    const int z4 = stored_zero4(ubias);
    const v4i zero_frag = (v4i){z4, z4, z4, z4};
    auto deq = [&](unsigned wd, int b) __attribute__((always_inline)) {
      const int code = FSIGNED ? (int)(int8_t)(wd >> (8 * b)) : (int)((wd >> (8 * b)) & 255u);
      return (float)code * fscale;
    };
    for (int64_t bt = t_begin; bt < t_end; ++bt) {
      const unsigned smp = (unsigned)(bt / fa.bands);
      const int r0 = (int)(bt - (int64_t)smp * fa.bands) * fa.R;
      const int Rb = H - r0 < fa.R ? H - r0 : fa.R;
      if (smp != cur) {
        flush(cur);
        cur = smp;
      }
      for (int c0 = 0; c0 < g.Cin; c0 += 4 * fa.segs) {
        const int c = front_channel(c0, wave, fa.segs, seg);
        const bool c_ok = seg < fa.segs && c < g.Cin;
        const int cc = c_ok ? c : 0;
        const float* kc = dwk + cc * 12;
        const float w00 = kc[0], w01 = kc[1], w02 = kc[2], w10 = kc[3], w11 = kc[4], w12 = kc[5], w20 = kc[6], w21 = kc[7],
                    w22 = kc[8], bch = kc[9], bsc = kc[10], bsh = kc[11];
        const unsigned* src = xc32 + ((int64_t)(smp * (unsigned)g.Cin + (unsigned)cc) * H) * Q + pos;
        unsigned raw_c[kFrontRows + 2];
#pragma unroll
        for (int k = 0; k < kFrontRows + 2; ++k) {
          const int t = r0 - 1 + k, tc = t < 0 ? 0 : (t > H - 1 ? H - 1 : t);
          raw_c[k] = src[tc * Q] & ((t >= 0 && t < H) ? 0xFFFFFFFFu : 0u);
        }
        auto zcode = [&](float acc) __attribute__((always_inline)) {
          if constexpr (NN) {
            const float v = FE == kEpiRuntime ? dw_finish<kEpiRuntime>(acc, has_fb, bch, has_fbn, bsc, bsh, fa.act)
                                              : dw_finish<FE, false>(acc, false, 0.0f, true, bsc, bsh, 0);
            int r;
            const float Qv = fast_quot(fq_clip(v, qc), fqx);
            asm("v_cvt_rpi_i32_f32 %0, %1" : "=v"(r) : "v"(Qv));
            return (unsigned)r ^ (nn_xor & 255u);
          } else {
            const float v = dw_finish<FE>(acc, has_fb, bch, has_fbn, bsc, bsh, fa.act);
            return (unsigned)(fq_code_int(v, q) + ubias) ^ 0x80u;
          }
        };
        float a[6] = {0.f, 0.f, 0.f, 0.f, 0.f, 0.f}, b[6] = {0.f, 0.f, 0.f, 0.f, 0.f, 0.f};
        unsigned dst = (unsigned)front_byte(fa.lay, cc, 4 * pos);
        const unsigned jstep = (unsigned)(front_byte(fa.lay, 0, 1) - front_byte(fa.lay, 0, 0));
        const unsigned rstep = (unsigned)(front_byte(fa.lay, 0, 4 * Q) - front_byte(fa.lay, 0, 0));
#pragma unroll
        for (int k = 0; k < kFrontRows + 2; ++k) {
          if (k <= Rb + 1) {
            float cv[6];
#pragma unroll
            for (int j = 0; j < 4; ++j) cv[j + 1] = deq(raw_c[k], j);
            const float lp = lane_prev(cv[4]), ln = lane_next(cv[1]);
            cv[0] = first ? 0.0f : lp;
            cv[5] = last ? 0.0f : ln;
            if (k >= 2) {
#pragma unroll
              for (int j = 0; j < 4; ++j) {
                const unsigned code = zcode(dw_taps(w00, w01, w02, w10, w11, w12, w20, w21, w22, a[j], a[j + 1], a[j + 2], b[j],
                                                    b[j + 1], b[j + 2], cv[j], cv[j + 1], cv[j + 2]));
                if (c_ok) zbuf[dst + j * jstep] = (unsigned char)code;
              }
              dst += rstep;
              asm volatile("" : "+v"(dst));
            }
#pragma unroll
            for (int j = 0; j < 6; ++j) {
              a[j] = b[j];
              b[j] = cv[j];
            }
          }
        }
      }
      __syncthreads();
      const int npix = Rb * W, ntile = (npix + 31) >> 5;
      for (int tl = wave; tl < ntile; tl += 4) {
        int pp = tl * 32 + pl;
        pp = pp < npix ? pp : npix - 1;
        const unsigned* zp = reinterpret_cast<const unsigned*>(zbuf + front_byte(fa.lay, g.Cin <= 16 ? 0 : 16 * h, pp));
        v4i f;
#pragma unroll
        for (int u = 0; u < 4; ++u) f[u] = (int)zp[u * fa.lay.pl];
        if (g.Cin <= 16 && h == 1) f = zero_frag;
        if (wr_codes) buf_st_v4i(rcodes, ((smp * 2u + (unsigned)h) * HW + (unsigned)(r0 * W + pp)) * 16u, f);
        afrag[0] = f;
        const int valid = npix - tl * 32;
        reduce_tile(0, valid < 32 ? valid : 32);
      }
      __syncthreads();
    }
  };
  if constexpr (FRONT) {
    if (fq_nonneg(q) && fqx.ok) run_front(std::true_type{});
    else run_front(std::false_type{});
  } else {
    if (fq_nonneg(q) && fqx.ok) run_all(std::true_type{});
    else run_all(std::false_type{});
  }
  if (t_begin < t_end) flush(cur);
  __syncthreads();
  if (threadIdx.x < kSlots && k_stat[threadIdx.x] != 0u && s_base + threadIdx.x < cols / HW)
    FQ_STAT_FLUSH_MAX(reinterpret_cast<unsigned*>(stat_out) + s_base + threadIdx.x, k_stat[threadIdx.x]);
}

__global__ void fast_quotient_kernel(const float* __restrict__ c, int64_t n, const float* __restrict__ d, float* __restrict__ out,
                                     int* __restrict__ ok_out) {
  const FastQuot f = make_fast_quot(d[0]);
  const double rden = 1.0 / (double)d[0];
  const int64_t i = (int64_t)blockIdx.x * blockDim.x + threadIdx.x;
  if (i == 0) ok_out[0] = f.ok ? 1 : 0;
  if (i < n) out[i] = f.ok ? fast_quot(c[i], f) : ieee_div_by(c[i], rden);
}

struct PwDwPlan {
  int kt, cw, lz, strips, ctg, bands, rb, pitch, threads;
  size_t lds;
  bool ok;
};

PwDwPlan pwdw_plan(int64_t n, int64_t cin, int64_t cout, int64_t h, int64_t w, int stride) {
  PwDwPlan p;
  memset(&p, 0, sizeof(p));
  if (n <= 0 || cin <= 0 || cout <= 0 || h < 3 || w < 8 || (stride != 1 && stride != 2)) return p;
  if (cout % 32 != 0 || (stride == 2 && (w % 2 != 0 || h % 2 != 0))) return p;
  const int kt = (int)((cin + 31) / 32), ct = (int)(cout / 32);
  if (!(kt == 1 || kt == 2 || kt == 4 || kt == 8)) return p;
  const int wo = (int)((w - 1) / stride + 1), ho = (int)((h - 1) / stride + 1);
  p.kt = kt;
  p.cw = ct % 2 == 0 ? 2 : 1;
  p.strips = (int)((w + 29) / 30);
  p.lz = (stride == 1 && p.strips == 1) ? (int)(30 - w) : 0;
  if (!(p.lz == 0 || p.lz == 2)) return p;
  p.ctg = ct / p.cw;
  p.threads = 64 * p.strips * p.ctg;
  if (p.threads > 512) return p;
  const int reach = stride == 1 ? (int)w + 2 + p.lz : 15 * p.strips + 1;
  p.pitch = (reach > wo ? reach : wo) + p.lz;
  p.pitch |= 1;
  p.lds = (size_t)ct * kt * 1024 + 2 * ((size_t)cout * p.pitch + kRowSlack) * 4 + kRowSlack * 4 + (stride == 1 ? (size_t)cout * 13 * 4 : 0);
  if (p.lds + 10 * 1024 > (size_t)max_lds_bytes()) return p;
  static const int rb_env = env_int("FQ_PWDW_RB", 0);
  {
    const int waves = p.threads / 64;
    int occ = (int)((160 * 1024) / (p.lds + 512));
    const int by_regs = 8 / waves > 0 ? 8 / waves : 1;
    occ = occ < by_regs ? occ : by_regs;
    occ = occ < 1 ? 1 : occ;
    const double slots = (double)num_cu() * occ;
    double best = 1e30;
    int best_rb = ho;
    for (int b = 1; b <= ho; ++b) {
      const int rb = (ho + b - 1) / b, bands = (ho + rb - 1) / rb;
      const double wgs = (double)n * bands, rounds = ceil(wgs / slots), fill = wgs < slots ? wgs / slots : 1.0;
      const double cost = rounds * (stride * rb + 2) / fill;
      if (cost < best - 1e-9) {
        best = cost;
        best_rb = rb;
      }
    }
    p.rb = rb_env > 0 ? (rb_env < ho ? rb_env : ho) : best_rb;
  }
  p.bands = (ho + p.rb - 1) / p.rb;
  if (n * cin * h * w * 4 >= (1ll << 32) || n * cout * ho * wo >= (1ll << 31)) return p;
  p.ok = true;
  return p;
}

}

namespace fqi {

static size_t pw_stat_lds(int kt, int ct) { return (size_t)ct * kt * 1024 + 5 * (size_t)ct * 32 * 4 + 4 * (size_t)ct * 128 * 4; }

bool pw_stat_shape_ok(int64_t n, int64_t cin, int64_t cout, int64_t hw) {
  if (n <= 0 || cin <= 0 || cout <= 0 || hw < 32 || hw >= (1ll << 30) || n * hw >= (1ll << 31) - 512) return false;
  const int kt = (int)((cin + 31) / 32), ct = (int)((cout + 31) / 32);
  if (!(kt == 1 || kt == 2 || kt == 4 || kt == 8) || cin % 16 != 0) return false;
  return pw_stat_lds(kt, ct) <= (size_t)kStatLdsMax && n * cin * hw * 4 < (1ll << 32);
}

constexpr int kFrontWgCap = 4;

static int pw_front_rows(int64_t n, int64_t cin, int64_t cout, int64_t h, int64_t w) {
  const char* e = getenv("FQ_PWSTAT_FRONT_ROWS");
  static const int wg_env = env_int("FQ_PWSTAT_WG_PER_CU", 0);
  const size_t fixed = pw_stat_lds(1, (int)((cout + 31) / 32)) + (size_t)cin * 12 * 4;
  return front_rows_pick(n, h, w, (int)cin, fixed, num_cu(), wg_env > 0 ? wg_env : kFrontWgCap, e != nullptr ? atoi(e) : 0);
}

bool pw_stat_front_shape_ok(int64_t n, int64_t cin, int64_t cout, int64_t h, int64_t w) {
  if (h < 1 || w < 4 || w % 4 != 0 || w / 4 > 64 || !(cin == 16 || cin == 32) || !pw_stat_shape_ok(n, cin, cout, h * w)) return false;
  return pw_front_rows(n, cin, cout, h, w) >= 1 && n * cin * ((w / 4 + 61) / 62) < (1ll << 31) - 1024;
}

int pw_stat_launch(const PwCall& c) {
  const int kt = (int)((c.cin + 31) / 32), ct = (int)((c.cout + 31) / 32);
  size_t lds = pw_stat_lds(kt, ct);
  PwFrontArgs fa = {};
  if (c.front != nullptr) {
    const PwFront& f = *c.front;
    fa.codes = static_cast<const int8_t*>(f.codes);
    fa.w = f.w; fa.bias = f.bias; fa.bn_scale = f.bn_scale; fa.bn_shift = f.bn_shift;
    fa.in_stat = f.in_stat; fa.in_thr = f.in_thr; fa.levels = f.levels; fa.act = f.act;
    fa.H = (int)f.h; fa.W = (int)f.wdt; fa.Q = fa.W / 4; fa.segs = 64 / fa.Q;
    fa.R = pw_front_rows(c.n, c.cin, c.cout, f.h, f.wdt);
    FQ_REQUIRE(fa.R >= 1, "fq_pwconv_i8_stat: no band of the front layer fits the LDS");
    fa.bands = (fa.H + fa.R - 1) / fa.R;
    fa.lay = front_layout(fa.Q, fa.R);
    lds += (size_t)c.cin * 12 * 4 + front_band_bytes(fa.Q, fa.R, (int)c.cin);
  }
  PwStatGeom g;
  g.Cin = (int)c.cin; g.KTS = (int)(c.cin_pad / 32); g.Cout = (int)c.cout; g.CT = ct; g.HW = (int)c.hw;
  g.cols = c.n * c.hw; g.tiles = (g.cols + 31) / 32; g.zoff = c.zoff;
  g.hw = fast_div_for((unsigned)c.hw);
  if (int rc = pw_zero_stat(c)) return rc;
  int per_cu = stat_wg_per_cu(lds, c.front != nullptr ? kFrontWgCap : 3);
  static const int wg_env = env_int("FQ_PWSTAT_WG_PER_CU", 0);
  if (wg_env > 0) per_cu = wg_env;
  int64_t grid = (int64_t)num_cu() * per_cu;
  const int64_t need = c.front != nullptr ? c.n * fa.bands : (g.tiles + 3) / 4;
  if (grid > need) grid = need;
  static const int table_env = env_int("FQ_PWSTAT_TABLE", -1);
  g.table = table_env >= 0 ? table_env : (g.tiles < grid * 4 * 10 ? 1 : 0);
#define FQ_PST_GO(KT_)                                                                                                     \
  case KT_: {                                                                                                              \
    static const bool attr_ok = hipFuncSetAttribute(reinterpret_cast<const void*>(&pw_stat_kernel<KT_>),                   \
                                                    hipFuncAttributeMaxDynamicSharedMemorySize, 120 * 1024) == hipSuccess; \
    FQ_REQUIRE(attr_ok, "fq_pwconv_i8_stat: cannot raise the dynamic LDS limit");                                          \
    hipLaunchKernelGGL((pw_stat_kernel<KT_>), dim3((unsigned)grid), dim3(kBlock), lds, c.st, c.x, c.wcodes, c.wscale,       \
                       (const int*)c.wsum, c.bias, g, c.in_stat, (int)c.n, c.in_thr, c.levels, c.lo_neg, kEps,              \
                       c.out_current_max, c.bn_scale, c.bn_shift, c.act, c.stat_out, (int8_t*)c.x_codes_out, fa);          \
  } break;
#define FQ_PST_FRONT(EPI_, SG_)                                                                                            \
  {                                                                                                                        \
    static const bool attr_ok = hipFuncSetAttribute(reinterpret_cast<const void*>(&pw_stat_kernel<1, EPI_, SG_>),          \
                                                    hipFuncAttributeMaxDynamicSharedMemorySize, 120 * 1024) == hipSuccess; \
    FQ_REQUIRE(attr_ok, "fq_pwconv_i8_stat: cannot raise the dynamic LDS limit");                                          \
    hipLaunchKernelGGL((pw_stat_kernel<1, EPI_, SG_>), dim3((unsigned)grid), dim3(kBlock), lds, c.st, c.x, c.wcodes,       \
                       c.wscale, (const int*)c.wsum, c.bias, g, c.in_stat, (int)c.n, c.in_thr, c.levels, c.lo_neg, kEps,   \
                       c.out_current_max, c.bn_scale, c.bn_shift, c.act, c.stat_out, (int8_t*)c.x_codes_out, fa);          \
  }
#define FQ_PST_FRONT_S(EPI_)                                                                                               \
  {                                                                                                                        \
    if (c.front->is_signed) FQ_PST_FRONT(EPI_, true) else FQ_PST_FRONT(EPI_, false)                                        \
  }
  if (c.front != nullptr) {
    FQ_REQUIRE(kt == 1, "fq_pwconv_i8_stat: a front layer needs cin <= 32");
    if (c.front->epi == kEpiBnRelu) FQ_PST_FRONT_S(kEpiBnRelu)
    else if (c.front->epi == kEpiBnRelu6) FQ_PST_FRONT_S(kEpiBnRelu6)
    else FQ_PST_FRONT_S(kEpiRuntime)
  } else {
    switch (kt) {
      FQ_PST_GO(1) FQ_PST_GO(2) FQ_PST_GO(4) FQ_PST_GO(8)
      default: return fail(FQ_ERR_INVALID, "fq_pwconv_i8_stat: K / 32 = %d is not instantiated", kt);
    }
  }
#undef FQ_PST_FRONT_S
#undef FQ_PST_FRONT
#undef FQ_PST_GO
  FQ_LAUNCH_CHECK();
  return FQ_OK;
}

}

using namespace fqi;

extern "C" {

int fq_debug_fast_quotient(const float* c, int64_t n, const float* d, float* out, int* took_fast_path, fqStream_t stream) {
  FQ_REQUIRE(c && d && out && took_fast_path && n > 0, "fq_debug_fast_quotient: null pointer");
  hipLaunchKernelGGL(fast_quotient_kernel, dim3((unsigned)((n + 255) / 256)), dim3(256), 0, (hipStream_t)stream, c, n, d, out,
                     took_fast_path);
  FQ_LAUNCH_CHECK();
  return FQ_OK;
}

int fq_pwdw_fused_supported(int64_t n, int64_t cin, int64_t cout, int64_t h, int64_t w, int stride) {
  return pwdw_plan(n, cin, cout, h, w, stride).ok ? 1 : 0;
}

int fq_pwdw_fused(const float* x, const int8_t* wcodes, const float* wscale, const int32_t* wsum, const float* pw_bias,
                  int64_t n, int64_t cin, int64_t cin_pad, int64_t cout_pad, int64_t cout, int64_t h, int64_t w,
                  const float* in_stat, const float* in_thr, int in_width, unsigned in_flags, const float* pw_bn_scale,
                  const float* pw_bn_shift, int pw_act, const float* mid_stat, const float* mid_thr, int mid_width,
                  unsigned mid_flags, float* mid_current_max, const float* dw_w, const float* dw_bias, int dw_stride,
                  const float* dw_bn_scale, const float* dw_bn_shift, int dw_act, float* y, float* stat_out,
                  const void* x_codes, fqStream_t stream) {
  FQ_REQUIRE((x || x_codes) && wcodes && wscale && wsum && dw_w && y, "fq_pwdw_fused: null pointer");
  FQ_REQUIRE(in_stat != nullptr || in_thr != nullptr, "fq_pwdw_fused: give in_stat (online) or in_thr (offline)");
  FQ_REQUIRE(mid_stat != nullptr || mid_thr != nullptr, "fq_pwdw_fused: give mid_stat (the per-sample maxima of the pointwise "
             "output, from fq_pwconv_i8_stat) or mid_thr (a stored threshold)");
  FQ_REQUIRE(in_width >= 2 && in_width <= 8, "fq_pwdw_fused: input width %d does not fit int8 codes", in_width);
  FQ_REQUIRE(mid_width >= 2 && mid_width <= 16, "fq_pwdw_fused: bad width %d of the depthwise input", mid_width);
  FQ_REQUIRE(!((in_flags | mid_flags) & (FQ_ACT_NO_ABS | FQ_ACT_NO_EPS)), "fq_pwdw_fused: unsupported activation flags");
  FQ_REQUIRE((pw_bn_scale == nullptr) == (pw_bn_shift == nullptr) && (dw_bn_scale == nullptr) == (dw_bn_shift == nullptr),
             "fq_pwdw_fused: a BatchNorm's scale and shift go together");
  FQ_REQUIRE(cin_pad >= cin && cin_pad % 64 == 0 && cout_pad >= cout && cout_pad % 32 == 0,
             "fq_pwdw_fused: cin_pad / cout_pad must be those of fq_weight_codes");
  const bool prezeroed = (dw_act & FQ_STAT_PREZEROED) != 0;
  dw_act &= ~FQ_STAT_PREZEROED;
  FQ_REQUIRE(pw_act >= FQ_ACT_NONE && pw_act <= FQ_ACT_RELU6 && dw_act >= FQ_ACT_NONE && dw_act <= FQ_ACT_RELU6,
             "fq_pwdw_fused: unknown activation");
  FQ_REQUIRE(aligned16(wcodes) && (x_codes ? aligned16(x_codes) : aligned16(x)) && aligned16(y),
             "fq_pwdw_fused: x (x_codes when given), wcodes and y must be 16-byte aligned");
  const PwDwPlan p = pwdw_plan(n, cin, cout, h, w, dw_stride);
  FQ_REQUIRE(p.ok, "fq_pwdw_fused: shape not taken (n=%lld cin=%lld cout=%lld %lldx%lld stride %d): see fq_pwdw_fused_supported",
             (long long)n, (long long)cin, (long long)cout, (long long)h, (long long)w, dw_stride);
  hipStream_t st = (hipStream_t)stream;
  const int64_t ho = (h - 1) / dw_stride + 1, wo = (w - 1) / dw_stride + 1;
  if (stat_out && !prezeroed) FQ_HIP(hipMemsetAsync(stat_out, 0, n * sizeof(float), st));
  PwDwGeom g;
  g.Cin = (int)cin; g.KTS = (int)(cin_pad / 32); g.Cout = (int)cout; g.H = (int)h; g.W = (int)w; g.Ho = (int)ho; g.Wo = (int)wo;
  g.strips = p.strips; g.ctg = p.ctg; g.bands = p.bands; g.RB = p.rb;
  g.zoff = (in_flags & FQ_ACT_SIGNED) ? 0 : 128;
  g.pitch = p.pitch;
  g.vw = wo % 4 == 0 ? 4 : (wo % 2 == 0 ? 2 : 1);
  g.qv = fast_div_for((unsigned)(wo / g.vw));
  const int8_t* wfrag = wcodes + cout_pad * cin_pad;
  const float levels1 = act_levels(in_width, in_flags), levels2 = act_levels(mid_width, mid_flags);
  const int lo1 = (in_flags & FQ_ACT_LO_NEG_MAX) ? 1 : 0, lo2 = (mid_flags & FQ_ACT_LO_NEG_MAX) ? 1 : 0;
  int fast = 0;
  if (!pw_bias && !dw_bias && pw_bn_scale && dw_bn_scale && !lo1 && !lo2 && pw_act == dw_act &&
      (pw_act == FQ_ACT_RELU || pw_act == FQ_ACT_RELU6))
    fast = 1;
  static const int no_fast = env_int("FQ_PWDW_NO_FAST", 0);
  if (no_fast) fast = 0;
  const double in_elems = (double)n * cin * h * w, mid_elems = (double)n * cout * h * w, out_elems = (double)n * cout * ho * wo;
  const double in_moved = x_codes ? 32.0 * p.kt * (double)n * h * w : 4.0 * in_elems;
  ProfScope prof(FQ_KERNEL_DWCONV, 4.0 * (mid_elems + out_elems), st, in_moved + 4.0 * out_elems);
  const int8_t* xc = static_cast<const int8_t*>(x_codes);
  const unsigned grid = (unsigned)(n * p.bands);
#define FQ_PWDW_GO(KT_, CW_, S_, LZ_, F_, C_)                                                                               \
  {                                                                                                                        \
    static const bool attr_ok = hipFuncSetAttribute(reinterpret_cast<const void*>(&pwdw_kernel<KT_, CW_, S_, LZ_, F_, C_>), \
                                                    hipFuncAttributeMaxDynamicSharedMemorySize, 150 * 1024) == hipSuccess; \
    FQ_REQUIRE(attr_ok, "fq_pwdw_fused: cannot raise the dynamic LDS limit");                                              \
    hipLaunchKernelGGL((pwdw_kernel<KT_, CW_, S_, LZ_, F_, C_>), dim3(grid), dim3((unsigned)p.threads), p.lds, st, x, xc,   \
                       wfrag, wscale, (const int*)wsum, pw_bias, g, in_stat, (int)n, in_thr, levels1, lo1, kEps,            \
                       pw_bn_scale, pw_bn_shift, pw_act, mid_stat, mid_thr, levels2, lo2, mid_current_max, dw_w, dw_bias,   \
                       dw_bn_scale, dw_bn_shift, dw_act, y, stat_out);                                                     \
  }
#define FQ_PWDW_C(KT_, CW_, S_, LZ_, F_)                                                                                    \
  {                                                                                                                        \
    if (xc != nullptr) FQ_PWDW_GO(KT_, CW_, S_, LZ_, F_, 1) else FQ_PWDW_GO(KT_, CW_, S_, LZ_, F_, 0)                       \
  }
#define FQ_PWDW_F(KT_, CW_, S_, LZ_)                                                                                        \
  {                                                                                                                        \
    if (fast == 1) FQ_PWDW_C(KT_, CW_, S_, LZ_, 1) else FQ_PWDW_C(KT_, CW_, S_, LZ_, 0)                                     \
  }
#define FQ_PWDW_S(KT_, CW_)                                                                                                 \
  {                                                                                                                        \
    if (dw_stride == 2) FQ_PWDW_F(KT_, CW_, 2, 0)                                                                          \
    else if (p.lz == 0) FQ_PWDW_F(KT_, CW_, 1, 0) else FQ_PWDW_F(KT_, CW_, 1, 2)                                            \
  }
#define FQ_PWDW_K(KT_)                                                                                                      \
  case KT_:                                                                                                                \
    if (p.cw == 2) FQ_PWDW_S(KT_, 2) else FQ_PWDW_S(KT_, 1)                                                                \
    break;
  switch (p.kt) {
    FQ_PWDW_K(1) FQ_PWDW_K(2) FQ_PWDW_K(4) FQ_PWDW_K(8)
    default: break;
  }
#undef FQ_PWDW_K
#undef FQ_PWDW_S
#undef FQ_PWDW_F
#undef FQ_PWDW_C
#undef FQ_PWDW_GO
  FQ_LAUNCH_CHECK();
  return FQ_OK;
}

}
```

### quantization/mxnet_amd/ops.py

```python
import ctypes
import threading

import numpy as np
import torch

from . import _lib
from ._lib import FakeQuantError

__all__ = ["comm_unique_id", "comm_init", "comm_world", "comm_allreduce", "comm_destroy", "add_act_stat", "bn_act_maxpool_stat", "stat_rows_sum", "mean_from_sums", "fake_quant_online_prestat", "bn_act_stat", "stem_conv3x3s2", "stem_conv_s2", "stem_conv_supported", "eval_counters", "dense_i8_eval", "gemm_i8_codes", "global_avg_pool_stat", "dwconv3x3", "dwconv3x3_c16", "weight_codes", "pwconv_i8", "pwconv_strided_supported", "weight_codes_3x3", "weight_slices_3x3", "conv3x3_i8", "Codes16", "batch_mean_rows", "batch_mean_gathered", "ste_forward", "absmax_per_sample", "batch_mean", "fake_quant_online", "fake_quant_offline", "weight_fake_quant",
           "wino_weight_fake_quant", "ema_update", "global_max", "histogram_accumulate", "hist_to_float",
           "kl_search", "quantize_codes", "dequantize", "qconv_kind", "qconv_weights", "qconv_workspace", "qconv2d",
           "batches_in_flight", "in_flight", "winograd_matrices", "device_info", "act_flags"]

_WS = {}


def _lib_():
    return _lib.LIB


_DEVICE_TLS = threading.local()


def _stream(t):
# ... 422 lines not shown
    check_call(_lib_().fq_dense_i8_eval(_ptr(x), _ptr(wcodes), _ptr(wscale), _ptr(wsum), _ptr(bias), _ptr(y), n, cin,
                                        cin_pad, cout, _ptr(in_stat), _ptr(in_thr), int(width), int(flags), _ptr(cur_out),
                                        lb.data_ptr(), _ptr(counters), ews.data_ptr(), _ptr(ws), _stream(x)))
    return y


def eval_counters(logits, labels, counters):
    _check(logits, "logits")
    _check(counters, "counters")
    require_hip(labels.device, "labels")
    if logits.dim() != 2 or labels.dim() != 1 or labels.shape[0] != logits.shape[0] or labels.dtype != torch.int64:
        raise ValueError("eval_counters wants logits (N, classes) float32 and labels (N,) int64")
    n, classes = logits.shape
    if counters.numel() != 2 + 2 * classes or not counters.is_contiguous():
        raise ValueError("counters must hold 2 + 2*classes contiguous floats")
    lg = logits if logits.is_contiguous() else logits.contiguous()
    lb = labels if labels.is_contiguous() else labels.contiguous()
    check_call(_lib_().fq_eval_counters(_ptr(lg), lb.data_ptr(), n, classes, _ptr(counters), _stream(logits)))
    return counters


def stem_conv_s2(x, w, bias=None, bn_scale=None, bn_shift=None, act=None, want_stat=True, w_tap_major=None, out_codes=None,
                 pool=False):
    _check(x, "x")
    _check(w, "w")
    if x.dim() != 4 or w.dim() != 4 or w.shape[2] != w.shape[3] or w.shape[2] not in (3, 7) or w.shape[1] != x.shape[1]:
        raise ValueError("stem_conv_s2 wants x (N,C,H,W) and w (Cout,C,K,K), K = 3 or 7; got %s and %s"
                         % (tuple(x.shape), tuple(w.shape)))
    for name, t in (("bias", bias), ("bn_scale", bn_scale), ("bn_shift", bn_shift), ("w_tap_major", w_tap_major)):
        if t is not None:
            _check(t, name)
    act = act or "none"
    if act not in _ACTS:
        raise ValueError("unknown activation %r" % (act,))
    n, cin, h, wd = x.shape
    cout, ks = w.shape[0], w.shape[2]
    pad = ks // 2
    wt = w_tap_major if w_tap_major is not None else w.permute(1, 2, 3, 0).contiguous()
    y = torch.empty((n, cout, (h + 2 * pad - ks) // 2 + 1, (wd + 2 * pad - ks) // 2 + 1), dtype=torch.float32,
                    device=x.device)
    stat, zflag = _stat_target(n, x.device, want_stat)
    if out_codes is not None:
        if ks != 3:
            raise ValueError("the first convolution hands codes over in its 3x3 form only")
        othr = _check(out_codes["thr"], "out_codes['thr']")
        yc = Codes16.empty(tuple(y.shape), x.device, othr, out_codes.get("width", 8), out_codes.get("flags", 0))
        check_call(_lib_().fq_stem_conv3x3s2_c16(_ptr(x), _ptr(wt), _ptr(bias), _ptr(yc.t), n, cin, cout, h, wd, _ptr(bn_scale),
                                                 _ptr(bn_shift), _ACTS[act] | zflag, _ptr(stat), _ptr(othr), int(yc.width),
                                                 int(yc.flags), _stream(x)))
        return yc, stat
    if pool:
        if ks != 7 or not stem_pool_supported(h, wd):
            raise ValueError("the pooled form is built for the 7x7 first convolution on planes whose output rows cut into four "
                             "tiles of at most 32 columns; got K = %d on %d x %d" % (ks, h, wd))
        ho, wo = y.shape[2], y.shape[3]
        yp = torch.empty((n, cout, (ho - 1) // 2 + 1, (wo - 1) // 2 + 1), dtype=torch.float32, device=x.device)
        check_call(_lib_().fq_stem_conv7x7s2_pool(_ptr(x), _ptr(wt), _ptr(bias), _ptr(yp), n, cin, cout, h, wd, _ptr(bn_scale),
                                                  _ptr(bn_shift), _ACTS[act] | zflag, _ptr(stat), _stream(x)))
        return yp, stat
    entry = _lib_().fq_stem_conv3x3s2 if ks == 3 else _lib_().fq_stem_conv7x7s2
    check_call(entry(_ptr(x), _ptr(wt), _ptr(bias), _ptr(y), n, cin, cout, h, wd, _ptr(bn_scale), _ptr(bn_shift),
                     _ACTS[act] | zflag, _ptr(stat), _stream(x)))
    return y, stat


stem_conv3x3s2 = stem_conv_s2


def stem_pool_supported(h, w):
    return bool(_lib_().fq_stem_conv7x7s2_pool_supported(int(h), int(w)))


def stem_conv_supported(cin, cout, kernel, stride, pad):
    k, s, p = tuple(kernel), tuple(stride), tuple(pad)
    return cin == 3 and s == (2, 2) and ((cout == 32 and k == (3, 3) and p == (1, 1)) or
                                         (cout == 64 and k == (7, 7) and p == (3, 3)))


def front_codes_shape(xshape):
    n, c, h, w = (int(v) for v in xshape)
    return (n, c, h * w)


def _check_front_codes(t, name, xshape, device):
    _check(t, name, torch.int8)
    if len(xshape) != 4 or tuple(t.shape) != front_codes_shape(xshape):
        raise ValueError("%s must be int8 %s for a depthwise input %s; got %s"
                         % (name, front_codes_shape(xshape) if len(xshape) == 4 else "(4-d x)", tuple(xshape), tuple(t.shape)))
    if t.device != device:
        raise ValueError("%s lives on %s, x on %s" % (name, t.device, device))
    if t.data_ptr() % 16:
        raise ValueError("%s must be 16-byte aligned" % name)
    return t


def dwconv3x3(x, w, bias=None, stride=1, in_stat=None, in_thr=None, width=8, flags=0, cur_out=None, bn_scale=None,
              bn_shift=None, act=None, want_stat=True, store=True, x_codes_out=None):
    _check(x, "x")
    _check(w, "w")
    if x.dim() != 4 or w.dim() != 4 or tuple(w.shape[1:]) != (1, 3, 3) or w.shape[0] != x.shape[1]:
        raise ValueError("dwconv3x3 wants x (N,C,H,W) and w (C,1,3,3); got %s and %s" % (tuple(x.shape), tuple(w.shape)))
    for name, t in (("bias", bias), ("in_stat", in_stat), ("in_thr", in_thr), ("bn_scale", bn_scale),
                    ("bn_shift", bn_shift), ("cur_out", cur_out)):
        if t is not None:
            _check(t, name)
    n, c, h, wd = x.shape
    ho, wo = (h - 1) // stride + 1, (wd - 1) // stride + 1
    if not store and not want_stat:
        raise ValueError("dwconv3x3(store=False) leaves nothing but the statistic: want_stat must be set")
    if x_codes_out is not None:
        if store:
            raise ValueError("dwconv3x3 keeps the codes of x only in its statistic pass (store=False)")
        _check_front_codes(x_codes_out, "x_codes_out", tuple(x.shape), x.device)
    y = torch.empty((n, c, ho, wo), dtype=torch.float32, device=x.device) if store else None
    stat, zflag = _stat_target(n, x.device, want_stat)
    check_call(_lib_().fq_dwconv3x3(_ptr(x), _ptr(w), _ptr(bias), _ptr(y), n, c, h, wd, int(stride), _ptr(in_stat),
                                    _ptr(in_thr), int(width), int(flags), _ptr(cur_out), _ptr(bn_scale),
                                    _ptr(bn_shift), _ACTS[act] | zflag, _ptr(stat), _stream(x), _ptr(x_codes_out)))
    return y, stat


def dwconv3x3_c16(x, w, bias=None, stride=1, in_stat=None, in_thr=None, width=8, flags=0, cur_out=None, bn_scale=None,
                  bn_shift=None, act=None, want_stat=True, out_codes=None):
    if not isinstance(x, Codes16) or in_thr is None or not x.matches(in_thr, width, flags):
        raise ValueError("dwconv3x3_c16 wants a Codes16 input quantised with this call's in_thr / width / signedness")
    if out_codes is None:
        raise ValueError("dwconv3x3_c16 writes codes: give out_codes")
    _check(x.t, "x", torch.int8)
    _check(w, "w")
    n, c, h, wd = x.shape
    if w.dim() != 4 or tuple(w.shape[1:]) != (1, 3, 3) or w.shape[0] != c:
        raise ValueError("dwconv3x3_c16 wants w (C,1,3,3); got %s for C = %d" % (tuple(w.shape), c))
    for name, t in (("bias", bias), ("in_stat", in_stat), ("in_thr", in_thr), ("bn_scale", bn_scale),
                    ("bn_shift", bn_shift), ("cur_out", cur_out)):
        if t is not None:
            _check(t, name)
    dev = x.t.device
    ho, wo = (h - 1) // stride + 1, (wd - 1) // stride + 1
    othr = _check(out_codes["thr"], "out_codes['thr']")
    y = Codes16.empty((n, c, ho, wo), dev, othr, out_codes.get("width", 8), out_codes.get("flags", 0))
    if in_stat is not None and cur_out is None:
        cur_out = torch.empty(1, dtype=torch.float32, device=dev)
    stat, zflag = _stat_target(n, dev, want_stat)
    check_call(_lib_().fq_dwconv3x3_c16(_ptr(x.t), _ptr(w), _ptr(bias), _ptr(y.t), n, c, h, wd, int(stride), _ptr(in_stat),
                                        _ptr(in_thr), int(width), int(flags), _ptr(cur_out), _ptr(bn_scale), _ptr(bn_shift),
                                        _ACTS[act] | zflag, _ptr(stat), _ptr(othr), y.width, y.flags, _stream(w)))
    return y, stat


def pwdw_supported(xshape, cout, stride):
    n, cin, h, w = (int(v) for v in xshape)
    lib = _lib_()
    return bool(lib.fq_pwconv_i8_stat_supported(n, cin, int(cout), h * w, 0, 0)) and \
        bool(lib.fq_pwdw_fused_supported(n, cin, int(cout), h, w, int(stride)))


def pwconv_front_supported(xshape, cout):
    n, cin, h, w = (int(v) for v in xshape)
    return bool(_lib_().fq_pwconv_i8_stat_supported(n, cin, int(cout), h * w, h, w))


def pair_codes_shape(xshape):
    n, cin, h, w = (int(v) for v in xshape)
    return (n, 2 * ((cin + 31) // 32), h * w, 16)


def _check_pair_codes(t, name, x):
    _check(t, name, torch.int8)
    if x.dim() != 4 or tuple(t.shape) != pair_codes_shape(x.shape):
        raise ValueError("%s must be int8 %s for x %s; got %s" % (name, pair_codes_shape(x.shape) if x.dim() == 4 else "(4-d x)",
                                                                  tuple(x.shape), tuple(t.shape)))
    if t.device != x.device:
        raise ValueError("%s lives on %s, x on %s" % (name, t.device, x.device))
    return t


def pwconv_i8_stat(x, wcodes, wscale, wsum, bias=None, in_stat=None, in_thr=None, width=8, flags=0, cur_out=None,
                   bn_scale=None, bn_shift=None, act=None, x_codes_out=None, front=None):
    _check(x, "x")
    _check(wcodes, "wcodes", torch.int8)
    _check(wscale, "wscale")
    _check(wsum, "wsum", torch.int32)
    for name, t in (("bias", bias), ("in_stat", in_stat), ("in_thr", in_thr), ("bn_scale", bn_scale),
                    ("bn_shift", bn_shift), ("cur_out", cur_out)):
        if t is not None:
            _check(t, name)
    n, cin = x.shape[0], x.shape[1]
    cout = wscale.numel()
    cin_pad = wcodes.shape[1]
    if (cin + 63) // 64 * 64 != cin_pad:
        raise ValueError("x has %d channels but the weight codes were made for a row length that pads to %d" % (cin, cin_pad))
    if in_stat is not None and cur_out is None:
        cur_out = torch.empty(1, dtype=torch.float32, device=x.device)
    if x_codes_out is not None:
        _check_pair_codes(x_codes_out, "x_codes_out", x)
    f_args = (_ptr(None),) * 5 + (0, _ptr(None), _ptr(None), 0, 0, 0, 0)
    if front is not None:
        unknown = set(front) - {"x_codes", "w", "bias", "bn_scale", "bn_shift", "act", "in_stat", "in_thr", "width", "flags"}
        if unknown or x.dim() != 4:
            raise ValueError("pwconv_i8_stat(front=) wants x (N, Cin, H, W) and the keys of a depthwise call; got %s, %s"
                             % (tuple(x.shape), sorted(unknown)))
        fw = _check(front["w"], "front['w']")
        if tuple(fw.shape) != (cin, 1, 3, 3):
            raise ValueError("front['w'] must be (%d,1,3,3); got %s" % (cin, tuple(fw.shape)))
        _check_front_codes(front["x_codes"], "front['x_codes']", tuple(x.shape), x.device)
        for name in ("bias", "bn_scale", "bn_shift", "in_stat", "in_thr"):
            if front.get(name) is not None:
                _check(front[name], "front['%s']" % name)
        if not pwconv_front_supported(x.shape, cout):
            raise ValueError("pwconv_i8_stat(front=) does not take x %s -> %d channels: see pwconv_front_supported"
                             % (tuple(x.shape), cout))
        f_args = (_ptr(front["x_codes"]), _ptr(fw), _ptr(front.get("bias")), _ptr(front.get("bn_scale")),
                  _ptr(front.get("bn_shift")), _ACTS[front.get("act")], _ptr(front.get("in_stat")), _ptr(front.get("in_thr")),
                  int(front.get("width", 8)), int(front.get("flags", 0)), int(x.shape[2]), int(x.shape[3]))
    stat, zflag = _stat_target(n, x.device, True)
    hw = x.numel() // (n * cin)
    check_call(_lib_().fq_pwconv_i8_stat(_ptr(x), _ptr(wcodes), _ptr(wscale), _ptr(wsum), _ptr(bias), n, cin, cin_pad,
                                         wcodes.shape[0], cout, hw, _ptr(in_stat), _ptr(in_thr), int(width), int(flags), _ptr(cur_out),
                                         _ptr(bn_scale), _ptr(bn_shift), _ACTS[act] | zflag, _ptr(stat), _ptr(x_codes_out),
                                         _stream(x), *f_args))
    return stat


def pwdw_fused(x, wcodes, wscale, wsum, dw_w, pw_bias=None, in_stat=None, in_thr=None, width=8, flags=0, pw_bn_scale=None,
               pw_bn_shift=None, pw_act=None, mid_stat=None, mid_thr=None, mid_width=8, mid_flags=0, mid_cur_out=None,
               dw_bias=None, stride=1, dw_bn_scale=None, dw_bn_shift=None, dw_act=None, want_stat=True, x_codes=None):
    _check(x, "x")
    _check(wcodes, "wcodes", torch.int8)
    _check(wscale, "wscale")
    _check(wsum, "wsum", torch.int32)
    _check(dw_w, "dw_w")
    for name, t in (("pw_bias", pw_bias), ("in_stat", in_stat), ("in_thr", in_thr), ("pw_bn_scale", pw_bn_scale),
                    ("pw_bn_shift", pw_bn_shift), ("mid_stat", mid_stat), ("mid_thr", mid_thr), ("mid_cur_out", mid_cur_out),
                    ("dw_bias", dw_bias), ("dw_bn_scale", dw_bn_scale), ("dw_bn_shift", dw_bn_shift)):
        if t is not None:
            _check(t, name)
    if x.dim() != 4:
        raise ValueError("pwdw_fused wants x (N, Cin, H, W); got %s" % (tuple(x.shape),))
    n, cin, h, w = x.shape
    cout = wscale.numel()
    if dw_w.dim() != 4 or tuple(dw_w.shape) != (cout, 1, 3, 3):
        raise ValueError("pwdw_fused wants dw_w (%d,1,3,3); got %s" % (cout, tuple(dw_w.shape)))
    cout_pad, cin_pad = wcodes.shape
    if (cin + 63) // 64 * 64 != cin_pad:
        raise ValueError("x has %d channels but the weight codes were made for a row length that pads to %d" % (cin, cin_pad))
    if x_codes is not None:
        _check_pair_codes(x_codes, "x_codes", x)
    ho, wo = (h - 1) // stride + 1, (w - 1) // stride + 1
    y = torch.empty((n, cout, ho, wo), dtype=torch.float32, device=x.device)
    stat, zflag = _stat_target(n, x.device, want_stat)
    check_call(_lib_().fq_pwdw_fused(_ptr(x), _ptr(wcodes), _ptr(wscale), _ptr(wsum), _ptr(pw_bias), n, cin, cin_pad, cout_pad,
                                     cout, h, w, _ptr(in_stat), _ptr(in_thr), int(width), int(flags), _ptr(pw_bn_scale),
                                     _ptr(pw_bn_shift), _ACTS[pw_act], _ptr(mid_stat), _ptr(mid_thr), int(mid_width),
                                     int(mid_flags), _ptr(mid_cur_out), _ptr(dw_w), _ptr(dw_bias), int(stride),
                                     _ptr(dw_bn_scale), _ptr(dw_bn_shift), _ACTS[dw_act] | zflag, _ptr(y), _ptr(stat),
                                     _ptr(x_codes), _stream(x)))
    return y, stat


def weight_codes(w, rows_per_scale, width=8):
    _check(w, "w")
    rows = w.shape[0]
    row_len = w.numel() // rows
    row_pad = (row_len + 63) // 64 * 64
    rows_pad = (rows + 63) // 64 * 64
    buf = torch.empty(2 * rows_pad * row_pad, dtype=torch.int8, device=w.device)
    codes = buf[:rows_pad * row_pad].view(rows_pad, row_pad)
    scales = torch.empty(rows, dtype=torch.float32, device=w.device)
    rowsum = torch.empty(rows, dtype=torch.int32, device=w.device)
    ws = _workspace(w.device, _lib_().fq_weight_workspace_bytes(rows))
    check_call(_lib_().fq_weight_codes(_ptr(w), rows, row_len, int(rows_per_scale), int(width), row_pad, rows_pad,
                                       _ptr(codes), _ptr(scales), _ptr(rowsum), _ptr(ws), _stream(w)))
    return codes, scales, rowsum


def weight_codes_reproduce(w, codes, scales):
    rows = w.shape[0]
    w2 = w.reshape(rows, -1)
    back = codes[:rows, :w2.shape[1]].to(torch.float32) * scales.reshape(rows, 1)
    return bool(torch.equal(back, w2))


class Codes16(object):
    __slots__ = ("t", "shape", "thr", "width", "flags")

    def __init__(self, t, shape, thr, width, flags):
        self.t, self.shape, self.thr, self.width, self.flags = t, tuple(int(d) for d in shape), thr, int(width), int(flags)

    @staticmethod
    def empty(shape, device, thr, width, flags):
        n, c, h, w = shape
        t = torch.empty((n, (c + 15) // 16, h * w, 16), dtype=torch.int8, device=device)
        return Codes16(t, shape, thr, width, flags)

    def matches(self, thr, width, flags):
        return self.thr.data_ptr() == thr.data_ptr() and self.width == int(width) and \
            (self.flags & 3) == (int(flags) & 3)


PW_FORMS = {None: 0, "auto": 0, "two_kernels": 1, "stream": 3, "split": 6, "sample": 7, "rows": 8}


SPLIT_KT = (2, 4, 6, 8, 10, 12, 16, 18, 30, 32, 64)


def pwconv_strided_supported(cin):
    return ((int(cin) + 63) // 64 * 64) // 32 in SPLIT_KT


def pwconv_residual_supported(cin):
    return ((int(cin) + 63) // 64 * 64) // 32 in SPLIT_KT


def pwconv_shortcut_supported(cin, cin2, cout):
    return bool(_lib_().fq_pwconv_i8_shortcut_supported(int(cin), int(cin2), int(cout)))


def pwconv_i8_shortcut(x, wcodes, wscale, wsum, bias=None, in_stat=None, in_thr=None, width=8, flags=0, cur_out=None,
                       bn_scale=None, bn_shift=None, act=None, x2=None, wcodes2=None, wscale2=None, wsum2=None, in_stat2=None,
                       in_thr2=None, width2=8, flags2=0, cur_out2=None, bn_scale2=None, bn_shift2=None, side_codes=None):
    a16, b16 = isinstance(x, Codes16), isinstance(x2, Codes16)
    if a16 != (side_codes is not None) or (b16 and not a16):
        raise ValueError("pwconv_i8_shortcut: fp32 on every side, or a Codes16 x with side_codes (x2 then fp32 or Codes16)")
    if a16 and (in_thr is None or not x.matches(in_thr, width, flags)):
        raise ValueError("the C16 input was quantised with another threshold / width / signedness than this call names")
    if b16 and (in_thr2 is None or not x2.matches(in_thr2, width2, flags2)):
        raise ValueError("the C16 shortcut input was quantised with another threshold / width / signedness than this call names")
    xt, x2t = (x.t if a16 else x), (x2.t if b16 else x2)
    xs, x2s = (x.shape if a16 else tuple(x.shape)), (x2.shape if b16 else tuple(x2.shape))
    for name, t, dt in (("x", xt, torch.int8 if a16 else None), ("wcodes", wcodes, torch.int8), ("wscale", wscale, None),
                        ("wsum", wsum, torch.int32), ("x2", x2t, torch.int8 if b16 else None), ("wcodes2", wcodes2, torch.int8),
                        ("wscale2", wscale2, None), ("wsum2", wsum2, torch.int32), ("bn_scale2", bn_scale2, None),
                        ("bn_shift2", bn_shift2, None)):
        if dt is None:
            _check(t, name)
        else:
            _check(t, name, dt)
    for name, t in (("bias", bias), ("in_stat", in_stat), ("in_thr", in_thr), ("bn_scale", bn_scale), ("bn_shift", bn_shift),
                    ("cur_out", cur_out), ("in_stat2", in_stat2), ("in_thr2", in_thr2), ("cur_out2", cur_out2)):
        if t is not None:
            _check(t, name)
    if len(xs) != 4 or len(x2s) != 4 or tuple(xs[2:]) != tuple(x2s[2:]) or xs[0] != x2s[0]:
        raise ValueError("pwconv_i8_shortcut wants x (N, Cin, H, W) and x2 (N, Cin2, H, W); got %s and %s" % (tuple(xs), tuple(x2s)))
    n, cin, h, w = xs
    cin2 = x2s[1]
    dev = xt.device
    cout = wscale.numel()
    if wscale2.numel() != cout:
        raise ValueError("the two convolutions must have the same number of filters (%d and %d)" % (cout, wscale2.numel()))
    if wcodes.shape[1] != cin or wcodes2.shape[1] != cin2 or not pwconv_shortcut_supported(cin, cin2, cout):
        raise ValueError("pwconv_i8_shortcut: %d / %d -> %d channels is not a shape it takes" % (cin, cin2, cout))
    if in_stat is not None and cur_out is None:
        cur_out = torch.empty(1, dtype=torch.float32, device=dev)
    if in_stat2 is not None and cur_out2 is None:
        cur_out2 = torch.empty(1, dtype=torch.float32, device=dev)
    y = torch.empty((n, cout, h, w), dtype=torch.float32, device=dev)
    stat, zflag = _stat_target(n, dev, True)
    if not a16:
        check_call(_lib_().fq_pwconv_i8_shortcut(_ptr(xt), _ptr(wcodes), _ptr(wscale), _ptr(wsum), _ptr(bias), _ptr(y), n, cin, cin,
                                                 cout, h * w, _ptr(in_stat), _ptr(in_thr), int(width), int(flags), _ptr(cur_out),
                                                 _ptr(bn_scale), _ptr(bn_shift), _ACTS[act] | zflag, _ptr(stat), _ptr(x2t),
                                                 _ptr(wcodes2), _ptr(wscale2), _ptr(wsum2), cin2, cin2, _ptr(in_stat2), _ptr(in_thr2),
                                                 int(width2), int(flags2), _ptr(cur_out2), _ptr(bn_scale2), _ptr(bn_shift2),
                                                 _stream(xt)))
        return y, stat
    sthr = _check(side_codes["thr"], "side_codes['thr']")
    y16 = Codes16.empty((n, cout, h, w), dev, sthr, side_codes.get("width", 8), side_codes.get("flags", 0))
    check_call(_lib_().fq_pwconv_i8_shortcut_c16(_ptr(xt), _ptr(wcodes), _ptr(wscale), _ptr(wsum), _ptr(bias), _ptr(y), _ptr(y16.t), n,
                                                 cin, cin, cout, h * w, _ptr(in_stat), _ptr(in_thr), int(width), int(flags),
                                                 _ptr(cur_out), _ptr(bn_scale), _ptr(bn_shift), _ACTS[act] | zflag, _ptr(stat),
                                                 _ptr(x2t), 1 if b16 else 0, _ptr(wcodes2), _ptr(wscale2), _ptr(wsum2), cin2, cin2,
                                                 _ptr(in_stat2), _ptr(in_thr2), int(width2), int(flags2), _ptr(cur_out2),
                                                 _ptr(bn_scale2), _ptr(bn_shift2), _ptr(sthr), int(y16.width), int(y16.flags),
                                                 _stream(wcodes)))
    return y, stat, y16


def pwconv_gap_supported(xshape, cout, residual=False):
    if len(xshape) != 4:
        return False
    return bool(_lib_().fq_pwconv_i8_gap_supported(int(xshape[0]), int(xshape[1]), int(cout), int(xshape[2]) * int(xshape[3]),
                                                    1 if residual else 0))


def pwconv_i8_gap(x, wcodes, wscale, wsum, bias=None, in_stat=None, in_thr=None, width=8, flags=0, cur_out=None,
                  bn_scale=None, bn_shift=None, act=None, residual=None):
    _check(x, "x")
    _check(wcodes, "wcodes", torch.int8)
    _check(wscale, "wscale")
    _check(wsum, "wsum", torch.int32)
    for name, t in (("bias", bias), ("in_stat", in_stat), ("in_thr", in_thr), ("bn_scale", bn_scale), ("bn_shift", bn_shift),
                    ("cur_out", cur_out), ("residual", residual)):
        if t is not None:
            _check(t, name)
    if x.dim() != 4:
        raise ValueError("pwconv_i8_gap wants x (N, Cin, H, W); got %s" % (tuple(x.shape),))
    n, cin, h, w = x.shape
    cout = wscale.numel()
    cin_pad = wcodes.shape[1]
    if cin != cin_pad:
        raise ValueError("pwconv_i8_gap: Cin = %d must be a multiple of 64" % cin)
    if residual is not None and tuple(residual.shape) != (n, cout, h, w):
        raise ValueError("the residual must have the convolution output's shape %s, got %s" % ((n, cout, h, w), tuple(residual.shape)))
    if not pwconv_gap_supported(tuple(x.shape), cout, residual is not None):
        raise ValueError("pwconv_i8_gap: shape %s -> %d channels is not taken (fq_pwconv_i8_gap_supported)" % (tuple(x.shape), cout))
    if in_stat is not None and cur_out is None:
        cur_out = torch.empty(1, dtype=torch.float32, device=x.device)
    y = torch.empty((n, cout, 1, 1), dtype=torch.float32, device=x.device)
    stat, zflag = _stat_target(n, x.device, True)
# ... 482 lines not shown
```

### quantization/mxnet_amd/quantize/convert/convert_conv2d.py

```python
from collections import namedtuple

import os

import torch

from ...mx import nd
from ...mx import autograd
from ...mx.ndarray import NDArray
from ...mx.gluon.nn import Conv2D
from ... import ops
from .._state import DeviceScalar
from ._blocks import INPUT_RANGE, BatchNormTerms, contiguous, rebind_forward, scalar_slot

__all__ = ['gen_conv2d_converter']

QuantizedArgs = namedtuple("ConvQuantizedArgs",
                           "quantize_input in_signed in_width "
                           "wt_width quant_type "
                           "fake_bn wino_quantize")

WINOGRAD_VARIANTS = ("F23", "F43", "F63")


def current_slot(block, like):
    return scalar_slot(block, like)[0]


class _InputView(object):

    def __init__(self, block, x):
        self.t = x._t if getattr(x, "_fq_deferred", None) is not None else contiguous(x._t)
        self.n = self.t.shape[0]
        self.cur, self.side = scalar_slot(block, self.t)
        rows = getattr(block, "_fq_stat_ws", None)
        if rows is not None and (rows.device != self.t.device or rows.numel() < self.n):
            rows = None
        self.rows = rows
        self.exchange = getattr(block, "_fq_global_stat", None)
        hint = x._fq_stat if x._t is self.t else None
        if hint is not None and (hint.numel() != self.n or hint.device != self.t.device):
            hint = None
        self.hint = hint

    def per_sample(self):
        if self.hint is None:
            return ops.absmax_per_sample(self.t, out=None if self.rows is None else self.rows[:self.n])
        if self.rows is not None:
            self.rows[:self.n].copy_(self.hint)
            return self.rows[:self.n]
        return self.hint

    def finish(self, block):
        if self.side:
            return
        block._fq_last_n = self.n
        block.current_input_max = DeviceScalar(self.cur)


def fake_quant_block_input(block, x, input_max, flags, width):
    v = _InputView(block, x)
    wanted = block.quantize_input
    offline = block.quantize_input_offline
    y = None
    if v.exchange is not None and v.rows is not None:
        v.exchange(v.per_sample(), v.n, v.cur)
        if wanted:
            y = ops.fake_quant_offline(v.t, input_max._t if offline else v.cur, width, flags, want_stat=False)[0]
    elif v.hint is not None or (v.rows is not None and getattr(block, "_fq_keep_rows", False)):
        stat = v.per_sample()
        if wanted and not offline:
            y = ops.fake_quant_online_prestat(v.t, stat, width, flags, cur_out=v.cur)[0]
        else:
            ops.batch_mean(stat, out=v.cur)
            if wanted:
                y = ops.fake_quant_offline(v.t, input_max._t, width, flags, want_stat=False)[0]
    elif not wanted:
        ops.batch_mean(v.per_sample(), out=v.cur)
    elif offline:
        y = ops.fake_quant_offline(v.t, input_max._t, width, flags, cur_out=v.cur, stat_ws=v.rows,
                                   want_stat=getattr(block, "track_input_stat", True))[0]
    else:
        y = ops.fake_quant_online(v.t, width, flags, cur_out=v.cur, stat_ws=v.rows)[0]
    v.finish(block)
    if y is None:
        return x
    return NDArray(autograd.ste_link(v.t, y))


def fused_input_plan(block, x, input_max, flags, width):
    v = _InputView(block, x)
    wanted = block.quantize_input
    online = wanted and not block.quantize_input_offline
    stat = None
    if online or v.exchange is not None or getattr(block, "track_input_stat", True):
        stat = v.per_sample()
    plan = {}
    if v.exchange is not None and v.rows is not None:
        v.exchange(stat, v.n, v.cur)
        if wanted:
            plan = dict(in_thr=input_max._t if block.quantize_input_offline else v.cur, width=width, flags=flags)
    elif online:
        plan = dict(in_stat=stat, width=width, flags=flags, cur_out=v.cur)
    elif wanted:
        plan = dict(in_thr=input_max._t, width=width, flags=flags)
        if stat is not None:
            plan.update(in_stat=stat, cur_out=v.cur)
    elif stat is not None:
        ops.batch_mean(stat, out=v.cur)
    v.finish(block)
    return plan


def depthwise_fused(block, x, weight_q, bias, plan):
    fz = block._fq_dw_fused
    scale, shift = fz["constants"]() if fz["bn"] is not None else (None, None)
    c16_in = getattr(x, "_fq_c16", None)
    if c16_in is not None:
        out_codes = handover_target(block, fz) if "in_thr" in plan else None
        if out_codes is not None:
            yc, stat = ops.dwconv3x3_c16(c16_in, contiguous(weight_q._t), None if bias is None else bias._t,
                                         stride=block._kwargs["stride"][0], bn_scale=scale, bn_shift=shift, act=fz["act"],
                                         out_codes=out_codes, **plan)
            out = NDArray(yc.t)
            out._fq_c16 = yc
            out._fq_stat = stat
            return out
        x = NDArray(codes16_to_fake_quant(c16_in))
        plan = {}
    call = dict(x=contiguous(x._t), w=contiguous(weight_q._t), bias=None if bias is None else bias._t,
                stride=block._kwargs["stride"][0], bn_scale=scale, bn_shift=shift, act=fz["act"], **plan)
    front = front_target(block, fz, x, plan) if c16_in is None else None
    if front is not None:
        xcodes = torch.empty(ops.front_codes_shape(call["x"].shape), dtype=torch.int8, device=call["x"].device)
        stat = _dwconv3x3(call, store=False, x_codes_out=xcodes)[1]
        out = NDArray(_placeholder(tuple(call["x"].shape), call["x"].device))
        out._fq_stat = stat
        out._fq_deferred = dict(kind="front", consumer=front, call=call, x_codes=xcodes)
        return out
    y, stat = _dwconv3x3(call)
    out = NDArray(y)
    out._fq_stat = stat
    return out


def _dwconv3x3(call, **more):
    kw = dict(call)
    return ops.dwconv3x3(kw.pop("x"), **kw, **more)


def front_target(block, fz, x, plan):
    from .. import fuse as _fuse
    nxt = fz.get("front_pw")
    if nxt is None or not _fuse.PAIR_CODES or not (int(_fuse.PAIR_FRONT) >= 2 or (_fuse.PAIR_FRONT and ops.in_flight())) \
            or block._kwargs["stride"] != (1, 1) \
            or block.quantize_args.fake_bn or "in_stat" not in plan or "in_thr" in plan or plan["width"] > 8:
        return None
    pz, a = nxt._fq_pw_fused, nxt.quantize_args
    if not (nxt.enable_quantize and a.quantize_input and nxt.quantize_input and not nxt.quantize_input_offline
            and a.in_width <= 8 and a.wt_width <= 8 and not getattr(nxt, "_fq_no_int8", False) and not a.fake_bn
            and getattr(nxt, "_fq_global_stat", None) is None and getattr(nxt, "_fq_residual", None) is None):
        return None
    if any(_hooked(b) for b in (block, fz.get("bn"), fz.get("act_block"))):
        return None
    if recompute_target(nxt, pz, x, dict(in_stat=None), None) is None or handover_target(nxt) is not None:
        return None
    if not ops.pwconv_front_supported(tuple(x._t.shape), nxt._kwargs["num_filter"]):
        return None
    return nxt


def _weight_rows_per_scale(block, args):
    cout = block._kwargs["num_filter"]
    per_channel = args.quant_type == "channel" or (args.quant_type == "group" and block._kwargs["num_group"] == cout)
    return 1 if per_channel else cout


def _pointwise_weight_codes(block, args, weight_raw, weight_q):
    param_t = block.weight.data()._t
    key = (param_t.data_ptr(), param_t._version)
    held = getattr(block, "_fq_pw_cache", None)
    if block.fixed_params == 1 and held is not None and held[3] == key:
        return held[:3]
    three = block._fq_pw_fused.get("kind") == "3x3"
    if block._fq_pw_fused.get("sliced"):
        codes = ops.weight_slices_3x3(contiguous(weight_q._t))
        if block.fixed_params == 1:
            block._fq_pw_cache = tuple(codes) + (key,)
        return codes
    make = ops.weight_codes_3x3 if three else ops.weight_codes
    rederived = block.fixed_params == 1 and held is not None
    src = contiguous((weight_q if rederived else weight_raw)._t)
    live = None if rederived else block.__dict__.get("_fq_pw_live")
    if live is not None and live[0] is weight_raw._t and live[1] == weight_raw._t._version:
        codes = live[2]
    else:
        codes = make(src, _weight_rows_per_scale(block, args), args.wt_width)
        if not rederived and block.fixed_params != 1 and weight_raw._t is param_t:
            block.__dict__["_fq_pw_live"] = (weight_raw._t, weight_raw._t._version, codes)
    if block.fixed_params == 1:
        block.__dict__.pop("_fq_pw_live", None)
    if rederived:
        ref = src.permute(0, 2, 3, 1).contiguous() if three else src
        if not ops.weight_codes_reproduce(ref, codes[0], codes[1]):
            block._fq_no_int8 = True
            block.__dict__.pop("_fq_pw_cache", None)
            return None
    if block.fixed_params == 1:
        block._fq_pw_cache = tuple(codes) + (key,)
    return codes


_DW_C16_MIN_PIXELS = int(os.environ.get("FQ_DW_C16_MIN_PIXELS", "1"))


def _consumer_takes_codes(nxt):
    a = nxt.quantize_args
    return (nxt.enable_quantize and a.quantize_input and nxt.quantize_input and nxt.quantize_input_offline
            and a.in_width <= 8 and a.wt_width <= 8 and not getattr(nxt, "_fq_no_int8", False)
            and getattr(nxt, "input_max", None) is not None and getattr(nxt, "_fq_global_stat", None) is None)


def _hooked(b):
    return b is not None and bool(getattr(b, "_forward_hooks", None) or getattr(b, "_forward_pre_hooks", None))


def handover_target(block, fz=None):
    from .. import fuse as _fuse
    fz = fz if fz is not None else block._fq_pw_fused
    nxt = fz.get("next")
    if nxt is None or not _fuse.HANDOVER or autograd.is_recording() or not _consumer_takes_codes(nxt):
        return None
    if any(_hooked(b) for b in (block, nxt, fz.get("bn"), fz.get("act_block")) + tuple(fz.get("via", ()))):
        return None
    dw = getattr(nxt, "_fq_dw_fused", None)
    if dw is not None and (handover_target(nxt, dw) is None or not fz.get("c16_pays", True)):
        return None
    a = nxt.quantize_args
    return dict(thr=nxt.input_max.data()._t, width=a.in_width, flags=ops.act_flags(signed=a.in_signed))


def _same_quantiser(block, other, plan, codes):
    from .. import fuse as _fuse
    if not _fuse.SIDE_CODES or codes.width != int(plan["width"]) or (codes.flags & 3) != (int(plan["flags"]) & 3):
        return False
    ta, tb = plan["in_thr"], getattr(other, "input_max", None)
    if tb is None:
        return False
    tb = tb.data()._t
    if tb.data_ptr() != codes.thr.data_ptr():
        return False
    key = (ta.data_ptr(), ta._version, tb.data_ptr(), tb._version, ops.state_epoch())
    memo = block.__dict__.get("_fq_same_thr")
    if memo is None or memo[0] != key:
        if ta.is_cuda and torch.cuda.is_current_stream_capturing():
            return False
        memo = block.__dict__["_fq_same_thr"] = (key, bool(torch.equal(ta.reshape(-1)[:1], tb.reshape(-1)[:1])))
    return memo[1]


_THIN_FORMS = os.environ.get("FQ_PWS_THIN", "1") != "0"
_SIDE_MAX_CIN = int(os.environ.get("FQ_SIDE_MAX_CIN", "512"))


def side_target(block, c16_in):
    from .. import fuse as _fuse
    nxt = block._fq_pw_fused.get("side_next")
    if nxt is None or c16_in is None or not _fuse.SIDE_CODES or not _fuse.HANDOVER or autograd.is_recording():
        return None
    if not _consumer_takes_codes(nxt) or getattr(nxt, "_fq_pw_fused", None) is None or nxt.quantize_args.in_signed:
        return None
    cin, cout = c16_in.shape[1], block._kwargs["num_filter"]
    if cin not in (64, 128, 256, 512) or cin > _SIDE_MAX_CIN or cout % 32 or cout < 256:
        return None
    return nxt


def sub_target(block, fz, xshape):
    from .. import fuse as _fuse
    link = fz.get("sub_next")
    if link is None or not _fuse.SUBSAMPLE or autograd.is_recording() or _fuse._collection is not None:
        return None
    if getattr(ops.StatArena._tls, "current", None) is None or len(xshape) != 4:
        return None
    for r in link["readers"]:
        k = r._kwargs
        if k["kernel"] != (1, 1) or k["stride"] != (2, 2) or k["pad"] != (0, 0) or getattr(r, "_fq_pw_fused", None) is None:
            return None
    if any(_hooked(b) for b in (block, fz.get("bn"), fz.get("act_block")) + tuple(link["readers"]) + tuple(link["via"])):
        return None
    for r in link["readers"]:
        rz = r._fq_pw_fused
        if any(_hooked(b) for b in (rz.get("bn"), rz.get("act_block"))):
            return None
    if not ops.pwconv_sub2_supported(xshape[1], block._kwargs["num_filter"]):
        return None
    return link


def gap_target(block, fz, c16_in, xshape, residual):
    from .. import fuse as _fuse
    link = fz.get("gap_next")
    if link is None or not _fuse.GAP_FUSE or c16_in is not None or autograd.is_recording() or _fuse._collection is not None:
        return None
    if getattr(ops.StatArena._tls, "current", None) is None or block._kwargs["stride"] != (1, 1):
        return None
    if any(_hooked(b) for b in (block, fz.get("bn"), fz.get("act_block"), link["gap"]) + tuple(link["via"])):
        return None
    if not ops.pwconv_gap_supported(xshape, block._kwargs["num_filter"], residual):
        return None
    return link["gap"]


def defer_shortcut(block, fz, x, x_arg, c16_in, codes3, bias, scale, shift, plan, stride_, extra):
    from .. import fuse as _fuse
    if not getattr(block, "_fq_defer_short", False):
        return None
    block._fq_defer_short = False
    if extra or bias is not None or scale is None or fz["act"] != "none" or stride_ != 1:
        return None
    if c16_in is not None and "in_thr" not in plan:
        return None
    if autograd.is_recording() or _fuse._collection is not None or getattr(ops.StatArena._tls, "current", None) is None:
        return None
    if any(_hooked(b) for b in (block, fz.get("bn"))) or not plan:
        return None
    xs = tuple(x_arg.shape)
    dev = x_arg.t.device if isinstance(x_arg, ops.Codes16) else x_arg.device
    out = NDArray(_placeholder((xs[0], block._kwargs["num_filter"], xs[2], xs[3]), dev))
    out._fq_short = dict(x=x_arg, codes=codes3, bn=(scale, shift), plan=dict(plan), block=block)
    return out


def materialise_shortcut_record(d):
    return ops.pwconv_i8(d["x"], *d["codes"], None, bn_scale=d["bn"][0], bn_shift=d["bn"][1], act=None, want_stat=False,
                         **d["plan"])[0]


def materialise_shortcut(s):
    return NDArray(materialise_shortcut_record(s._fq_short))


def _convolve(block, F, x, weight, bias):
    if getattr(x, "_fq_sub2", None) is None:
        return block.origin_forward(F, x, weight, bias)
    out = F.Convolution(x, weight, bias, name="fwd", **dict(block._kwargs, stride=(1, 1)))
    return out if block.act is None else block.act(out)


_PLACEHOLDERS = {}


def _placeholder(shape, device):
    one = _PLACEHOLDERS.get(device)
    if one is None:
        one = _PLACEHOLDERS[device] = torch.zeros(1, dtype=torch.int8, device=device)
    return one.expand(*shape)


def recompute_target(block, fz, x, plan, c16_in):
    from .. import fuse as _fuse
    nxt = fz.get("pair_dw")
    if nxt is None or not _fuse.RECOMPUTE or c16_in is not None or autograd.is_recording() or _fuse._collection is not None:
        return None
    if getattr(ops.StatArena._tls, "current", None) is None:
        return None
    if "in_stat" not in plan or "in_thr" in plan or getattr(block, "_fq_residual", None) is not None:
        return None
    a = nxt.quantize_args
    if not (nxt.enable_quantize and a.quantize_input and nxt.quantize_input and not nxt.quantize_input_offline
            and getattr(nxt, "_fq_global_stat", None) is None and not a.fake_bn and nxt._kwargs["num_group"] == block._kwargs["num_filter"]):
        return None
    if any(_hooked(b) for b in (block, nxt, fz.get("bn"), fz.get("act_block"))):
        return None
    t = x._t
    if t.dim() != 4 or t.shape[2] * t.shape[3] < _fuse.RECOMPUTE_MIN_PIXELS or t.shape[1] > _fuse.RECOMPUTE_MAX_CIN:
        return None
    if not ops.pwdw_supported(tuple(t.shape), block._kwargs["num_filter"], nxt._kwargs["stride"][0]):
        return None
    return nxt


def _materialise(x):
    d = x._fq_deferred
    if d.get("kind") == "front":
        y, stat = _dwconv3x3(d["call"])
    else:
        src = d["x"] if d.get("front") is None else _dwconv3x3(d["front"]["call"])[0]
        y, stat = ops.pwconv_i8(src, *d["codes"], d["bias"], bn_scale=d["bn"][0], bn_shift=d["bn"][1], act=d["act"],
                                **d["plan"])
    out = NDArray(y)
    out._fq_stat = stat
    return out


def depthwise_recompute(block, x, weight_q, bias, flags, width):
    d = x._fq_deferred
    fz = block._fq_dw_fused
    scale, shift = fz["constants"]() if fz["bn"] is not None else (None, None)
    src = d["x"]
    n = src.shape[0]
    cur, side = scalar_slot(block, src)
    stat = x._fq_stat
    rows = getattr(block, "_fq_stat_ws", None)
    if rows is not None and rows.device == src.device and rows.numel() >= n:
        rows[:n].copy_(stat)
    p = d["plan"]
    z, zstat = ops.pwdw_fused(src, *d["codes"], contiguous(weight_q._t), pw_bias=d["bias"], in_stat=p["in_stat"],
                              width=p["width"], flags=p["flags"], pw_bn_scale=d["bn"][0], pw_bn_shift=d["bn"][1],
                              pw_act=d["act"], mid_stat=stat, mid_width=width, mid_flags=flags, mid_cur_out=cur,
                              dw_bias=None if bias is None else bias._t, stride=block._kwargs["stride"][0],
                              dw_bn_scale=scale, dw_bn_shift=shift, dw_act=fz["act"], x_codes=d.get("x_codes"))
    if not side:
        block._fq_last_n = n
        block.current_input_max = DeviceScalar(cur)
    out = NDArray(z)
    out._fq_stat = zstat
    return out


def _handed_over(x):
    return getattr(x, "_fq_c16", None)


def codes16_to_fake_quant(c16):
    n, c, h, w = c16.shape
    signed = bool(c16.flags & 1)
    b = (c16.t.to(torch.int16) & 255) ^ 0x80
    codes = (b - 128).to(torch.int8).to(torch.float32) if signed else b.to(torch.float32)
    levels = float((1 << (c16.width - 1)) - 1) if signed else float((1 << c16.width) - 1)
    scale = c16.thr.reshape(()) / levels
    t = codes.reshape(n, -1, h * w, 16).permute(0, 1, 3, 2).reshape(n, -1, h, w)[:, :c]
    return (t * scale).contiguous()


def pointwise_fused(block, F, x, weight_raw, weight_q, bias, plan, weights_quantised):
    fz = block._fq_pw_fused
    args = block.quantize_args
    scale, shift = fz["constants"]() if fz["bn"] is not None else (None, None)
    on_codes = bool(plan) and weights_quantised and args.in_width <= 8 and args.wt_width <= 8 \
        and not getattr(block, "_fq_no_int8", False)
    held = _pointwise_weight_codes(block, args, weight_raw, weight_q) if on_codes else None
    on_codes = held is not None
    front = getattr(x, "_fq_deferred", None)
    if front is not None:
        from .. import fuse as _fuse
        if not (on_codes and fz.get("kind") == "1x1" and _fuse.PAIR_CODES and getattr(block, "_fq_residual", None) is None
                and handover_target(block) is None and recompute_target(block, fz, x, plan, None) is not None):
            x, front = _materialise(x), None
    res0 = getattr(block, "_fq_residual", None)
    if res0 is not None and res0.get("short") is not None and not (on_codes and fz.get("kind") == "1x1"):
        res0["t"], res0["short"] = materialise_shortcut_record(res0["short"]), None
    c16_in = _handed_over(x)
    stride_ = 1 if getattr(x, "_fq_sub2", None) is not None else block._kwargs["stride"][0]
    if c16_in is None and on_codes and "in_thr" in plan:
        side = getattr(x, "_fq_side", None)
        if side is not None and not autograd.is_recording():
            if side[0] is block and side[1].matches(plan["in_thr"], plan["width"], plan["flags"]):
                c16_in = side[1]
            elif side[0] is not block and _same_quantiser(block, side[0], plan, side[1]):
                c16_in = ops.Codes16(side[1].t, side[1].shape, plan["in_thr"], plan["width"], plan["flags"])
    if c16_in is not None and not (on_codes and "in_thr" in plan):
        x = NDArray(codes16_to_fake_quant(c16_in))
        plan, c16_in = {}, None
    if on_codes:
        codes, scales, rowsum = held
        if front is not None:
            x_arg = torch.empty(tuple(x._t.shape), dtype=torch.float32, device=x._t.device)
        else:
            x_arg = c16_in if c16_in is not None else contiguous(x._t)
        if fz.get("kind") == "3x3":
            out_codes = None if fz.get("sliced") else handover_target(block)
            y, stat = ops.conv3x3_i8(x_arg, codes, scales, rowsum, None if bias is None else bias._t,
                                     bn_scale=scale, bn_shift=shift, act=fz["act"],
                                     **({} if fz.get("sliced") or out_codes is None else dict(out_codes=out_codes)), **plan)
        else:
            res = getattr(block, "_fq_residual", None)
            extra = {}
            xshape = c16_in.shape if c16_in is not None else tuple(x._t.shape)
            side_blk = sub_link = None
            if res is not None and res.get("short") is not None:
                d = res["short"]
                side_s = side_target(block, c16_in) if c16_in is not None else None
                d16 = isinstance(d["x"], ops.Codes16)
                if (block._kwargs["stride"][0] == 1 and scale is not None and not _hooked(block)
                        and (c16_in is None and not d16 or (side_s is not None and "in_thr" in plan))
                        and tuple(d["x"].shape[2:]) == tuple(xshape[2:]) and d["x"].shape[0] == xshape[0]
                        and ops.pwconv_shortcut_supported(xshape[1], d["x"].shape[1], block._kwargs["num_filter"])
                        and (c16_in is None or block._kwargs["num_filter"] % 512 == 0 or xshape[1] == 64)
                        and not autograd.is_recording()):
                    p2 = d["plan"]
                    kw2 = dict(x2=d["x"], wcodes2=d["codes"][0], wscale2=d["codes"][1], wsum2=d["codes"][2], in_stat2=p2.get("in_stat"),
                               in_thr2=p2.get("in_thr"), width2=p2["width"], flags2=p2["flags"], cur_out2=p2.get("cur_out"),
                               bn_scale2=d["bn"][0], bn_shift2=d["bn"][1])
                    if side_s is not None:
                        a_ = side_s.quantize_args
                        kw2["side_codes"] = dict(thr=side_s.input_max.data()._t, width=a_.in_width, flags=ops.act_flags(signed=a_.in_signed))
                    out = ops.pwconv_i8_shortcut(x_arg, codes, scales, rowsum, None if bias is None else bias._t, bn_scale=scale,
                                                 bn_shift=shift, act=res["act"], **kw2, **plan)
                    res["used"] = True
                    folded = NDArray(out[0])
                    folded._fq_stat = out[1]
                    if side_s is not None:
                        folded._fq_side = (side_s, out[2])
                    return folded
                res["t"] = materialise_shortcut_record(d)
                res["short"] = None
            if res is not None and block._kwargs["stride"][0] == 1 and tuple(res["t"].shape[2:]) == tuple(xshape[2:]) \
                    and res["t"].shape[1] == block._kwargs["num_filter"] and ops.pwconv_residual_supported(xshape[1]):
                extra = dict(residual=res["t"])
                res["used"] = True
                side_blk = side_target(block, c16_in)
                if side_blk is not None:
                    a_ = side_blk.quantize_args
                    extra["side_codes"] = dict(thr=side_blk.input_max.data()._t, width=a_.in_width,
                                               flags=ops.act_flags(signed=a_.in_signed))
                if side_blk is not None or c16_in is None:
                    sub_link = sub_target(block, fz, xshape)
                    if sub_link is not None:
                        extra["subsample"] = True
            if not extra and (c16_in is None or xshape[1] >= 256 or
                              (xshape[1] <= 32 and xshape[0] * xshape[2] * xshape[3] > 32 * 4096 and _THIN_FORMS)):
                xs = c16_in.shape if c16_in is not None else tuple(x._t.shape)
                s_ = stride_
                fz["c16_pays"] = len(xs) == 4 and ((xs[2] - 1) // s_ + 1) * ((xs[3] - 1) // s_ + 1) >= _DW_C16_MIN_PIXELS
                out_codes = handover_target(block)
                if out_codes is not None and fz.get("via") is not None:
                    co = block._kwargs["num_filter"]
                    if not (co >= 256 or (co <= 32 and xs[0] * ((xs[2] - 1) // s_ + 1) * ((xs[3] - 1) // s_ + 1) > 32 * 4096
                                          and _THIN_FORMS)):
                        out_codes = None
                if out_codes is not None:
                    extra = dict(out_codes=out_codes)
            if not extra or (set(extra) == {"residual"} and side_blk is None):
                gap = gap_target(block, fz, c16_in, xshape, "residual" in extra)
                if gap is not None:
                    y, stat = ops.pwconv_i8_gap(x_arg, codes, scales, rowsum, None if bias is None else bias._t, bn_scale=scale,
                                                bn_shift=shift, act=res["act"] if "residual" in extra else fz["act"],
                                                residual=extra.get("residual"), **plan)
                    pooled = NDArray(y)
                    pooled._fq_stat = stat
                    pooled._fq_pooled_by = gap
                    return pooled
            short = defer_shortcut(block, fz, x, x_arg, c16_in, (codes, scales, rowsum), bias, scale, shift, plan, stride_, extra)
            if short is not None:
                return short
            pair = recompute_target(block, fz, x, plan, c16_in) if not extra else None
            if pair is not None:
                b_ = None if bias is None else bias._t
                from .. import fuse as _fuse
                xcodes = torch.empty(ops.pair_codes_shape(x_arg.shape), dtype=torch.int8, device=x_arg.device) \
                    if _fuse.PAIR_CODES else None
                fkw = {}
                if front is not None:
                    c_ = front["call"]
                    fkw = dict(front=dict(x_codes=front["x_codes"], w=c_["w"], bias=c_["bias"], bn_scale=c_["bn_scale"],
                                          bn_shift=c_["bn_shift"], act=c_["act"], in_stat=c_["in_stat"], width=c_["width"],
                                          flags=c_["flags"]))
                stat = ops.pwconv_i8_stat(x_arg, codes, scales, rowsum, b_, bn_scale=scale, bn_shift=shift, act=fz["act"],
                                          x_codes_out=xcodes, **fkw, **plan)
                xs = tuple(x_arg.shape)
                res_ = NDArray(_placeholder((xs[0], block._kwargs["num_filter"], xs[2], xs[3]), x_arg.device))
                res_._fq_stat = stat
                res_._fq_deferred = dict(x=x_arg, codes=(codes, scales, rowsum), bias=b_, bn=(scale, shift), act=fz["act"],
                                         plan=dict(in_stat=plan["in_stat"], width=plan["width"], flags=plan["flags"],
                                                   cur_out=plan.get("cur_out")), consumer=pair, x_codes=xcodes, front=front)
                return res_
            out = ops.pwconv_i8(x_arg, codes, scales, rowsum, None if bias is None else bias._t,
                                bn_scale=scale, bn_shift=shift,
                                act=res["act"] if "residual" in extra else fz["act"],
# ... 197 lines not shown
```

### quantization/mxnet_amd/quantize/fuse.py

```python
import types

import torch

from ..mx.gluon import nn
from ..mx.ndarray import NDArray
from .. import ops

__all__ = ["fuse_inference", "unfuse", "refresh", "eval_head", "EvalHead"]


def _is_relu6_block(b):
    return type(b).__name__ == "RELU6"


def _act_kind(b):
    if isinstance(b, nn.Activation) and b._act_type == "relu" and not hasattr(b, "quantize_args") \
            and b.hybrid_forward.__func__ is nn.Activation.hybrid_forward:
        return "relu"
    if _is_relu6_block(b):
        return "relu6"
    return None


def _tensors_key(*tensors):
    return tuple((t.data_ptr(), t._version) for t in tensors)


def _bn_constants(bn):
    g0, b = bn.gamma.data()._t, bn.beta.data()._t
    mean, var = bn.running_mean.data()._t, bn.running_var.data()._t
    g = torch.ones_like(g0) if bn._kwargs.get("fix_gamma", False) else g0
    scale = g / torch.sqrt(var + bn._kwargs["eps"])
    shift = b - mean * scale
    return scale.contiguous(), shift.contiguous(), _tensors_key(g0, b, mean, var)


_collection = None
_collection_calls = {}


def begin_collection():
    global _collection
    _collection = {}
    _collection_calls.clear()
    return _collection


def end_collection():
    global _collection
    _collection = None
    _collection_calls.clear()


def collection_calls():
    return _collection_calls


def _kl_sink(producer):
    if _collection is None:
        return None
    _collection_calls[producer] = _collection_calls.get(producer, 0) + 1
    return _collection.get(producer)


def _fused_bn_forward(self, F, x, gamma, beta, running_mean, running_var):
    st = self._fq_fused
    key = _tensors_key(gamma._t, beta._t, running_mean._t, running_var._t)
    if st["key"] != key:
        st["scale"], st["shift"], st["key"] = _bn_constants(self)
    t = x._t if x._t.is_contiguous() else x._t.contiguous()
    if st.get("pool") is not None and t.dim() == 4 and t.shape[3] % 4 == 0:
        y, stat = ops.bn_act_maxpool_stat(t, st["scale"], st["shift"], st["act"], want_stat=True)
        out = NDArray(y)
        out._fq_stat = stat
        out._fq_pooled_by = st["pool"]
        return out
    else:
        sink = _kl_sink(self)
        y, stat = ops.bn_act_stat(t, st["scale"], st["shift"], st["act"], want_stat=True, hist=sink)
        out = NDArray(y)
        out._fq_stat = stat
        if _collection is not None:
            out._fq_kl = (self, sink)
        return out


def _pool_after_bn_forward(self, F, x):
    if getattr(x, "_fq_pooled_by", None) is self:
        x._fq_pooled_by = None
        return x
    return self._fq_pool_fused["orig"](F, x)


def _pool_stat_forward(self, F, x):
    if getattr(x, "_fq_pooled_by", None) is self:
        x._fq_pooled_by = None
        return x
    t = x._t if x._t.is_contiguous() else x._t.contiguous()
    if t.dim() != 4 or t.shape[3] % 4 or not t.is_cuda:
        return self._fq_pool_fused["orig"](F, x)
    st = self._fq_pool_fused
    c = t.shape[1]
    if st.get("ones") is None or st["ones"].numel() != c or st["ones"].device != t.device:
        st["ones"] = torch.ones(c, dtype=torch.float32, device=t.device)
        st["zeros"] = torch.zeros(c, dtype=torch.float32, device=t.device)
    y, stat = ops.bn_act_maxpool_stat(t, st["ones"], st["zeros"], "none", want_stat=True)
    out = NDArray(y)
    out._fq_stat = stat
    return out


def _is_maxpool_3x3s2p1(b):
    if type(b) is not nn.MaxPool2D or b.hybrid_forward.__func__ is not nn.MaxPool2D.hybrid_forward:
        return False
    k = b._kwargs
    return (k["kernel"] == (3, 3) and k["stride"] == (2, 2) and k["pad"] == (1, 1) and not k["global_pool"]
            and k["pooling_convention"] == "valid")


import os as _os

HANDOVER = _os.environ.get("FQ_HANDOVER", "1") != "0"
SIDE_CODES = _os.environ.get("FQ_HANDOVER_SIDE", "1") != "0"
STEM_CODES = _os.environ.get("FQ_HANDOVER_STEM", "1") != "0"
WINO_SLICED = _os.environ.get("FQ_WINO_SLICED", "1") != "0"
BN_ADD = _os.environ.get("FQ_BN_ADD", "1") != "0"
RECOMPUTE = _os.environ.get("FQ_RECOMPUTE", "1") != "0"
RECOMPUTE_MIN_PIXELS = int(_os.environ.get("FQ_RECOMPUTE_MIN_PIXELS", "3136"))
RECOMPUTE_MAX_CIN = int(_os.environ.get("FQ_RECOMPUTE_MAX_CIN", "128"))
PAIR_CODES = _os.environ.get("FQ_PWDW_CODES", "1") != "0"
PAIR_FRONT = int(_os.environ.get("FQ_PWDW_FRONT", "1"))
SUBSAMPLE = _os.environ.get("FQ_SUBSAMPLE", "1") != "0"
GAP_FUSE = _os.environ.get("FQ_GAP_FUSE", "1") != "0"
SHORTCUT_FUSE = _os.environ.get("FQ_SHORTCUT_FUSE", "1") != "0"
UNIT_LINKS = _os.environ.get("FQ_HANDOVER_UNITS", "1") != "0"


def _identity_forward(self, F, x, *args, **kwargs):
    return x


def _is_dw3x3(b):
    if type(b) is not nn.Conv2D:
        return False
    k = b._kwargs
    cin = b.weight.shape[1] if b.weight.shape else 0
    return (k["kernel"] == (3, 3) and k["pad"] == (1, 1) and k["dilate"] == (1, 1) and k["stride"] in ((1, 1), (2, 2))
            and k["num_group"] == k["num_filter"] and cin == 1 and k["layout"] == "NCHW" and b.act is None
            and not getattr(getattr(b, "quantize_args", None), "fake_bn", False))


def _is_pw1x1(b):
    if type(b) is not nn.Conv2D or not hasattr(b, "quantize_args"):
        return False
    k = b._kwargs
    if not (k["kernel"] == (1, 1) and k["pad"] == (0, 0) and k["dilate"] == (1, 1) and k["num_group"] == 1
            and k["layout"] == "NCHW" and b.act is None and not b.quantize_args.fake_bn):
        return False
    if k["stride"] == (1, 1):
        return True
    cin = b.weight.shape[1] if b.weight.shape is not None and len(b.weight.shape) == 4 else 0
    return k["stride"] == (2, 2) and cin > 0 and ops.pwconv_strided_supported(cin)


def _is_dense3x3(b):
    if type(b) is not nn.Conv2D or not hasattr(b, "quantize_args"):
        return False
    k = b._kwargs
    a = b.quantize_args
    cin = b.weight.shape[1] if b.weight.shape is not None and len(b.weight.shape) == 4 else 0
    return (k["kernel"] == (3, 3) and k["pad"] == (1, 1) and k["dilate"] == (1, 1) and k["stride"] == (1, 1)
            and k["num_group"] == 1 and k["layout"] == "NCHW" and b.act is None and not a.fake_bn
            and cin in (64, 128, 256, 512) and k["num_filter"] >= 32
            and (not _wino_sliced(b) or (k["num_filter"] % 32 == 0 and WINO_SLICED)))


def _wino_sliced(b):
    a = b.quantize_args
    return a.quant_type == "channel" and a.wino_quantize != "none"


def _is_stem3x3s2(b):
    if type(b) is not nn.Conv2D or hasattr(b, "quantize_args"):
        return False
    if b.hybrid_forward.__func__ is not nn.Conv2D.hybrid_forward:
        return False
    k = b._kwargs
    shp = b.weight.shape
    return (len(shp) == 4 and k["num_group"] == 1 and k["dilate"] == (1, 1) and k["layout"] == "NCHW" and b.act is None
            and ops.stem_conv_supported(shp[1], shp[0], k["kernel"], k["stride"], k["pad"]))


def _stem_forward(self, F, x, weight, bias=None):
    st = self._fq_stem_fused
    w = weight._t
    key = (w.data_ptr(), w._version)
    if st["wkey"] != key:
        st["wt"], st["wkey"] = w.permute(1, 2, 3, 0).contiguous(), key
    scale = shift = None
    if st["constants"] is not None:
        scale, shift = st["constants"]()
    t = x._t if x._t.is_contiguous() else x._t.contiguous()
    out_codes = None
    if st.get("next") is not None and w.shape[2] == 3 and STEM_CODES:
        from .convert.convert_conv2d import handover_target
        out_codes = handover_target(self, st)
    pool = st.get("pool")
    hooked = any(bool(getattr(b, "_forward_hooks", None) or getattr(b, "_forward_pre_hooks", None))
                 for b in (self, st.get("bn"), st.get("act_block"), pool) if b is not None)
    pooled = (pool is not None and STEM_POOL and out_codes is None and w.shape[2] == 7 and t.dim() == 4 and not hooked
              and ops.stem_pool_supported(t.shape[2], t.shape[3]))
    y, stat = ops.stem_conv_s2(t, w, None if bias is None else bias._t, bn_scale=scale, bn_shift=shift,
                               act=st["act"], want_stat=True, w_tap_major=st["wt"], pool=pooled,
                               **({} if out_codes is None else dict(out_codes=out_codes)))
    if out_codes is not None:
        out = NDArray(y.t)
        out._fq_c16 = y
    else:
        out = NDArray(y)
    if pooled:
        out._fq_pooled_by = pool
    out._fq_stat = stat
    return out


def _gap_stat_forward(self, F, x):
    if getattr(x, "_fq_pooled_by", None) is self:
        x._fq_pooled_by = None
        return x
    t = x._t if x._t.is_contiguous() else x._t.contiguous()
    y, stat = ops.global_avg_pool_stat(t, want_stat=True)
    out = NDArray(y)
    out._fq_stat = stat
    return out


def _flatten_keep_stat_forward(self, F, x):
    out = NDArray(x._t.reshape(x._t.shape[0], -1))
    out._fq_stat = x._fq_stat
    return out


def _plain_dw_forward(self, F, x, weight, bias=None):
    from .convert.convert_conv2d import depthwise_fused
    return depthwise_fused(self, x, weight, bias, {})


def _tail_conv(seq):
    kids = list(seq._children.values()) if isinstance(seq, (nn.Sequential, nn.HybridSequential)) else []
    if kids and isinstance(kids[-1], (nn.Sequential, nn.HybridSequential)):
        return _tail_conv(kids[-1])
    if len(kids) < 2 or type(kids[-1]) is not nn.BatchNorm:
        return None
    conv, bn = kids[-2], kids[-1]
    fz = getattr(conv, "_fq_pw_fused", None)
    if fz is None or fz.get("kind") != "1x1" or fz["bn"] is not bn or fz["act"] != "none":
        return None
    return conv if conv._kwargs["stride"] == (1, 1) else None


def _with_residual(conv, shortcut, act, run, owner=None):
    short = getattr(shortcut, "_fq_short", None)
    t = None if short is not None else (shortcut._t if shortcut._t.is_contiguous() else shortcut._t.contiguous())
    conv._fq_residual = {"t": t, "short": short, "act": act, "used": False, "owner": owner}
    try:
        out = run()
        return out, conv._fq_residual["used"]
    finally:
        conv._fq_residual = None


def _residual_unit_forward(self, x):
    from ..mx import autograd
    if autograd.is_recording():
        raise RuntimeError("this net was rewired by quantize.fuse.fuse_inference (inference only): call "
                           "quantize.fuse.unfuse(net) before recording gradients")
    sub = getattr(x, "_fq_sub2", None)
    if sub is not None and sub["unit"] is not self:
        raise RuntimeError("a subsampled trunk (fq_pwconv_i8_sub2) reached a unit it was not made for")
    tail = _tail_conv(self.body)
    sc = _shortcut_conv(self) if (tail is not None and SHORTCUT_FUSE) else None
    if sc is not None:
        sc._fq_defer_short = True
    try:
# ... 511 lines not shown
```

Before: 155,100.

## Chain fused pw+dw statistic pass into next pointwise front without storing float output

Adds a statistic-only mode to the fused pointwise+depthwise kernel. In this mode it packs the 1x1 output's int8 codes straight to global memory and computes only the depthwise output max, skipping the float depthwise store. The next pointwise layer then recomputes the depthwise conv as its front stage from those codes. The front stage is widened to take up to 128 input channels (KT up to 4), and the front-row picker now prefers a band size that keeps two workgroups per CU. The risk is redundant depthwise computation plus more template instantiations and added register pressure.

After: 161,500 (median of 6 runs). 4.1% higher.

```diff
diff --git a/include/fakequant.h b/include/fakequant.h
--- a/include/fakequant.h
+++ b/include/fakequant.h
@@ -186,7 +186,7 @@
                       fqStream_t stream, const void* front_codes, const float* front_w, const float* front_bias,
                       const float* front_bn_scale, const float* front_bn_shift, int front_act, const float* front_in_stat,
                       const float* front_in_thr, int front_width, unsigned front_flags, int64_t front_h, int64_t front_wdt);
-int fq_pwdw_fused_supported(int64_t n, int64_t cin, int64_t cout, int64_t h, int64_t w, int stride);
+int fq_pwdw_fused_supported(int64_t n, int64_t cin, int64_t cout, int64_t h, int64_t w, int stride, int stat_mode);
 int fq_debug_fast_quotient(const float* c, int64_t n, const float* d, float* out, int* took_fast_path, fqStream_t stream);
 int fq_pwdw_fused(const float* x, const int8_t* wcodes, const float* wscale, const int32_t* wsum, const float* pw_bias,
                   int64_t n, int64_t cin, int64_t cin_pad, int64_t cout_pad, int64_t cout, int64_t h, int64_t w,
@@ -194,7 +194,7 @@
                   const float* pw_bn_shift, int pw_act, const float* mid_stat, const float* mid_thr, int mid_width,
                   unsigned mid_flags, float* mid_current_max, const float* dw_w, const float* dw_bias, int dw_stride,
                   const float* dw_bn_scale, const float* dw_bn_shift, int dw_act, float* y, float* stat_out,
-                  const void* x_codes, fqStream_t stream);
+                  const void* x_codes, fqStream_t stream, void* mid_codes_out);
 
 int fq_pwconv_i8_c16(const void* x, int x_is_c16, const int8_t* wcodes, const float* wscale, const int32_t* wsum,
                      const float* bias, void* y, int64_t n, int64_t cin, int64_t cin_pad, int64_t cout, int64_t h, int64_t w,
diff --git a/quantization/mxnet_amd/_lib.py b/quantization/mxnet_amd/_lib.py
--- a/quantization/mxnet_amd/_lib.py
+++ b/quantization/mxnet_amd/_lib.py
@@ -60,9 +60,9 @@
     "fq_pwconv_i8_stat_supported": (_int, [_i64, _i64, _i64, _i64, _i64, _i64]),
     "fq_pwconv_i8_stat": (_int, [_vp, _vp, _vp, _vp, _vp, _i64, _i64, _i64, _i64, _i64, _i64, _vp, _vp, _int, _uint, _vp, _vp,
                                  _vp, _int, _vp, _vp, _vp, _vp, _vp, _vp, _vp, _vp, _int, _vp, _vp, _int, _uint, _i64, _i64]),
-    "fq_pwdw_fused_supported": (_int, [_i64, _i64, _i64, _i64, _i64, _int]),
+    "fq_pwdw_fused_supported": (_int, [_i64, _i64, _i64, _i64, _i64, _int, _int]),
     "fq_pwdw_fused": (_int, [_vp, _vp, _vp, _vp, _vp, _i64, _i64, _i64, _i64, _i64, _i64, _i64, _vp, _vp, _int, _uint, _vp,
-                             _vp, _int, _vp, _vp, _int, _uint, _vp, _vp, _vp, _int, _vp, _vp, _int, _vp, _vp, _vp, _vp]),
+                             _vp, _int, _vp, _vp, _int, _uint, _vp, _vp, _vp, _int, _vp, _vp, _int, _vp, _vp, _vp, _vp, _vp]),
     "fq_debug_fast_quotient": (_int, [_vp, _i64, _vp, _vp, _vp, _vp]),
     "fq_dense_i8_eval_workspace_bytes": (ctypes.c_size_t, [_i64, _i64]),
     "fq_dense_i8_eval": (_int, [_vp, _vp, _vp, _vp, _vp, _vp, _i64, _i64, _i64, _i64, _vp, _vp, _int, _uint, _vp, _vp, _vp,
diff --git a/quantization/mxnet_amd/csrc/fq_core.hip b/quantization/mxnet_amd/csrc/fq_core.hip
--- a/quantization/mxnet_amd/csrc/fq_core.hip
+++ b/quantization/mxnet_amd/csrc/fq_core.hip
@@ -79,7 +79,7 @@
 extern "C" {
 
 const char* fq_last_error(void) { return g_err; }
-int fq_version(void) { return 101; }
+int fq_version(void) { return 102; }
 #ifndef FQ_BUILD_ID
 #define FQ_BUILD_ID "0000000000000000000000000000000000000000"
 #endif
diff --git a/quantization/mxnet_amd/csrc/fq_front_layout.h b/quantization/mxnet_amd/csrc/fq_front_layout.h
--- a/quantization/mxnet_amd/csrc/fq_front_layout.h
+++ b/quantization/mxnet_amd/csrc/fq_front_layout.h
@@ -50,6 +50,11 @@
   while (rmax >= 1 && lds_fixed + front_band_bytes(q, rmax, cin) > (size_t)kStatLdsMax) --rmax;
   if (rmax < 1) return 0;
   if (forced > 0) return forced < rmax ? forced : rmax;
+  {
+    int r2 = rmax;
+    while (r2 >= 1 && stat_wg_per_cu(lds_fixed + front_band_bytes(q, r2, cin), wg_cap) < 2) --r2;
+    if (r2 >= 1) rmax = r2;
+  }
   double best = 1e30;
   int best_r = rmax;
   bool best_whole = false;
diff --git a/quantization/mxnet_amd/csrc/fq_pwdw.hip b/quantization/mxnet_amd/csrc/fq_pwdw.hip
--- a/quantization/mxnet_amd/csrc/fq_pwdw.hip
+++ b/quantization/mxnet_amd/csrc/fq_pwdw.hip
@@ -21,7 +21,7 @@
   static constexpr int NR = 2;
 };
 
-template <int KT, int CW, int S, int LZ, int FAST, int CODES>
+template <int KT, int CW, int S, int LZ, int FAST, int CODES, int NS = 0>
 __global__ __launch_bounds__(512) void pwdw_kernel(
     const float* __restrict__ x, const int8_t* __restrict__ xc, const int8_t* __restrict__ wfrag, const float* __restrict__ wscale,
     const int* __restrict__ wsum, const float* __restrict__ bias1, PwDwGeom g, const float* __restrict__ in_stat, int n,
@@ -31,6 +31,7 @@
     const float* __restrict__ bias2, const float* __restrict__ bn2_scale, const float* __restrict__ bn2_shift, int act2,
     float* __restrict__ y, float* __restrict__ stat_out) {
   constexpr int NB = CODES ? 1 : PwDwRing<KT, S>::NB, NR = CODES ? PwDwRing<KT, S>::NR : 1;
+  static_assert(!NS || (S == 1 && CODES == 1), "the statistic mode is built for stride 1 on code input");
   extern __shared__ __attribute__((aligned(16))) unsigned char pwdw_smem[];
   __shared__ float red[8];
   const int CT = g.ctg * CW;
@@ -38,7 +39,7 @@
   const int rb_stride = g.Cout * g.pitch + kRowSlack;
   float* rowbuf = reinterpret_cast<float*>(pwdw_smem + (size_t)CT * KT * 1024) + kRowSlack;
   constexpr bool kDwLds = S == 1;
-  float* ldsK = rowbuf + 2 * rb_stride;
+  float* ldsK = NS ? reinterpret_cast<float*>(pwdw_smem + (size_t)CT * KT * 1024) : rowbuf + 2 * rb_stride;
 
   const int lane = threadIdx.x & 63, wave = threadIdx.x >> 6;
   const int h = lane >> 5, i32 = lane & 31;
@@ -63,6 +64,14 @@
   const int t_first = S == 1 ? ro0 - 1 : 2 * ro0 - 1;
   const int t_last = S == 1 ? ro1 : 2 * (ro1 - 1) + 1;
   float* yb = y + (int64_t)smp * g.Cout * g.Ho * g.Wo;
+  const bool ns_par2 = (c0 & 2) != 0;
+  const int ns_col3 = c0 + 16 * h + (ns_par2 ? 2 : 0);
+  const int ns_colx = ns_par2 ? (h ? c0 + 14 : c0) : c0 + 16 * h + 12;
+  const bool ns_x4 = ns_par2 ? h == 1 : h == 0;
+  const bool ns_ok3 = ns_col3 >= 0 && ns_col3 + 12 <= g.W;
+  const bool ns_okx = ns_colx >= 0 && ns_colx + (ns_x4 ? 4 : 2) <= g.W;
+  const fq_rsrc rsy = make_rsrc(NS ? reinterpret_cast<int8_t*>(y) + (int64_t)smp * g.Cout * HW : nullptr,
+                                NS ? (int64_t)g.Cout * HW : 0);
 
   float raw[NB][16];
 #pragma unroll
@@ -206,6 +215,7 @@
         auto finish_store = [&](const float (&sum)[NO]) __attribute__((always_inline)) {
           if (!emits) return;
           float* dst = rbuf + (ct * 32 + i32) * g.pitch + obase;
+          float mrow = 0.0f;
           const float b2 = kDwLds ? kc[9] : k_b2[j], bsc2 = kDwLds ? kc[10] : k_bsc2[j], bsh2 = kDwLds ? kc[11] : k_bsh2[j];
 #pragma unroll
           for (int k = 0; k < NO; ++k) {
@@ -217,7 +227,10 @@
               o = o + bsh2;
               o = __builtin_amdgcn_fmed3f(o, 0.0f, top);
             }
-            if (S == 1 && k == 0) {
+            if constexpr (NS != 0) {
+              const bool is_out = k == 0 ? h == 1 : (k == NO - 1 ? h == 0 : (LZ == 0 || k > LZ || h == 1));
+              mrow = fmaxf(mrow, is_out ? fabsf(o) : 0.0f);
+            } else if (S == 1 && k == 0) {
               if (h == 1) dst[k] = o;
             } else if (k == NO - 1) {
               if (h == 0) dst[k] = o;
@@ -225,6 +238,7 @@
               dst[k] = o;
             }
           }
+          if constexpr (NS != 0) m = fmaxf(m, mrow);
         };
         if (!row_ok) {
           if (S == 1) {
@@ -243,6 +257,7 @@
           continue;
         }
         float e[18];
+        float cf[NS ? 18 : 1];
         {
           v16i acc = {0, 0, 0, 0, 0, 0, 0, 0, 0, 0, 0, 0, 0, 0, 0, 0};
           int wl = lane;
@@ -260,12 +275,52 @@
                 v = v + k_bsh1[j];
               }
               v = act_rt(v, act1);
-              e[k + 1] = NN ? truncf(fast_quot(fq_clip(v, q2), fq2) + 0.49999997f) * q2.scale : fq_code(v, q2) * q2.scale;
+              const float code = NN ? truncf(fast_quot(fq_clip(v, q2), fq2) + 0.49999997f) : fq_code(v, q2);
+              e[k + 1] = code * q2.scale;
+              if constexpr (NS != 0) cf[k + 1] = code;
             } else {
               v = v * k_bsc1[j];
               v = v + k_bsh1[j];
-              if (NN) e[k + 1] = truncf(fast_quot(fq_clip(v, qc), fq2) + 0.49999997f) * q2.scale;
-              else e[k + 1] = fq_code(act_rt(v, relu6 ? FQ_ACT_RELU6 : FQ_ACT_RELU), q2) * q2.scale;
+              const float code = NN ? truncf(fast_quot(fq_clip(v, qc), fq2) + 0.49999997f)
+                                    : fq_code(act_rt(v, relu6 ? FQ_ACT_RELU6 : FQ_ACT_RELU), q2);
+              e[k + 1] = code * q2.scale;
+              if constexpr (NS != 0) cf[k + 1] = code;
+            }
+          }
+          if constexpr (NS != 0) {
+            const auto sc = __builtin_amdgcn_permlane32_swap(__float_as_uint(cf[1]), __float_as_uint(cf[16]), false, false);
+            cf[0] = __uint_as_float(sc[0]);
+            cf[17] = __uint_as_float(sc[1]);
+            auto pk4 = [&](float a, float b, float c, float d) __attribute__((always_inline)) {
+              if constexpr (NN) {
+                unsigned u = __builtin_amdgcn_cvt_pk_u8_f32(a, 0, 0u);
+                u = __builtin_amdgcn_cvt_pk_u8_f32(b, 1, u);
+                u = __builtin_amdgcn_cvt_pk_u8_f32(c, 2, u);
+                return (int)__builtin_amdgcn_cvt_pk_u8_f32(d, 3, u);
+              } else {
+                return (int)(((unsigned)(int)a & 255u) | (((unsigned)(int)b & 255u) << 8) | (((unsigned)(int)c & 255u) << 16) |
+                             ((unsigned)(int)d << 24));
+              }
+            };
+            typedef int v3i __attribute__((ext_vector_type(3)));
+            typedef unsigned v3u __attribute__((ext_vector_type(3)));
+            v3i d3;
+            int dx;
+            if (ns_par2) {
+              d3 = (v3i){pk4(cf[4], cf[5], cf[6], cf[7]), pk4(cf[8], cf[9], cf[10], cf[11]), pk4(cf[12], cf[13], cf[14], cf[15])};
+              dx = pk4(h ? cf[0] : cf[2], h ? cf[1] : cf[3], cf[2], cf[3]);
+            } else {
+              d3 = (v3i){pk4(cf[2], cf[3], cf[4], cf[5]), pk4(cf[6], cf[7], cf[8], cf[9]), pk4(cf[10], cf[11], cf[12], cf[13])};
+              dx = pk4(cf[14], cf[15], cf[16], cf[17]);
+            }
+            const unsigned rowb = (unsigned)((ct * 32 + i32) * HW + t * g.W);
+            if (ns_ok3) {
+              __builtin_amdgcn_raw_buffer_store_b96(__builtin_bit_cast(v3u, d3), rsy, (int)(rowb + (unsigned)ns_col3), 0, 0);
+              asm volatile("s_nop 1" : : "v"(d3));
+            }
+            if (ns_okx) {
+              if (ns_x4) __builtin_amdgcn_raw_buffer_store_b32((unsigned)dx, rsy, (int)(rowb + (unsigned)ns_colx), 0, 0);
+              else __builtin_amdgcn_raw_buffer_store_b16((unsigned short)dx, rsy, (int)(rowb + (unsigned)ns_colx), 0, 0);
             }
           }
           e[1 + (LZ & 15)] = zero_left ? 0.0f : e[1 + (LZ & 15)];
@@ -336,7 +391,7 @@
         }
         FQ_PIN();
       }
-      if (emits) {
+      if (NS == 0 && emits) {
         __syncthreads();
         const unsigned per_row = g.qv.d;
         const int vecs = g.Cout * (int)per_row;
@@ -420,7 +475,7 @@
     const float* __restrict__ bn_scale, const float* __restrict__ bn_shift, int act, float* __restrict__ stat_out,
     int8_t* __restrict__ x_codes_out, PwFrontArgs fa) {
   constexpr bool FRONT = FEPI >= 0;
-  static_assert(!FRONT || KT == 1, "the front layer is built for one 32-channel slab");
+  static_assert(!FRONT || KT <= 4, "the front layer is built for up to four 32-channel slabs");
   extern __shared__ __attribute__((aligned(16))) unsigned char pst_smem[];
   v4i* ldsW = reinterpret_cast<v4i*>(pst_smem);
   int* c_zs = reinterpret_cast<int*>(pst_smem + (size_t)g.CT * KT * 1024);
@@ -731,12 +786,16 @@
         int pp = tl * 32 + pl;
         pp = pp < npix ? pp : npix - 1;
         const unsigned* zp = reinterpret_cast<const unsigned*>(zbuf + front_byte(fa.lay, g.Cin <= 16 ? 0 : 16 * h, pp));
-        v4i f;
-#pragma unroll
-        for (int u = 0; u < 4; ++u) f[u] = (int)zp[u * fa.lay.pl];
-        if (g.Cin <= 16 && h == 1) f = zero_frag;
-        if (wr_codes) buf_st_v4i(rcodes, ((smp * 2u + (unsigned)h) * HW + (unsigned)(r0 * W + pp)) * 16u, f);
-        afrag[0] = f;
+#pragma unroll
+        for (int kt = 0; kt < KT; ++kt) {
+          v4i f;
+#pragma unroll
+          for (int u = 0; u < 4; ++u) f[u] = (int)zp[(8 * kt + u) * fa.lay.pl];
+          if (KT == 1 && g.Cin <= 16 && h == 1) f = zero_frag;
+          if (wr_codes)
+            buf_st_v4i(rcodes, ((smp * (unsigned)(2 * KT) + (unsigned)(2 * kt + h)) * HW + (unsigned)(r0 * W + pp)) * 16u, f);
+          afrag[kt] = f;
+        }
         const int valid = npix - tl * 32;
         reduce_tile(0, valid < 32 ? valid : 32);
       }
@@ -792,7 +851,8 @@
   p.pitch |= 1;
   p.lds = (size_t)ct * kt * 1024 + 2 * ((size_t)cout * p.pitch + kRowSlack) * 4 + kRowSlack * 4 + (stride == 1 ? (size_t)cout * 13 * 4 : 0);
   if (p.lds + 10 * 1024 > (size_t)max_lds_bytes()) return p;
-  static const int rb_env = env_int("FQ_PWDW_RB", 0);
+  const char* rb_e = getenv("FQ_PWDW_RB");
+  const int rb_env = rb_e != nullptr ? atoi(rb_e) : 0;
   {
     const int waves = p.threads / 64;
     int occ = (int)((160 * 1024) / (p.lds + 512));
@@ -837,12 +897,14 @@
 static int pw_front_rows(int64_t n, int64_t cin, int64_t cout, int64_t h, int64_t w) {
   const char* e = getenv("FQ_PWSTAT_FRONT_ROWS");
   static const int wg_env = env_int("FQ_PWSTAT_WG_PER_CU", 0);
-  const size_t fixed = pw_stat_lds(1, (int)((cout + 31) / 32)) + (size_t)cin * 12 * 4;
+  const size_t fixed = pw_stat_lds((int)((cin + 31) / 32), (int)((cout + 31) / 32)) + (size_t)cin * 12 * 4;
   return front_rows_pick(n, h, w, (int)cin, fixed, num_cu(), wg_env > 0 ? wg_env : kFrontWgCap, e != nullptr ? atoi(e) : 0);
 }
 
 bool pw_stat_front_shape_ok(int64_t n, int64_t cin, int64_t cout, int64_t h, int64_t w) {
-  if (h < 1 || w < 4 || w % 4 != 0 || w / 4 > 64 || !(cin == 16 || cin == 32) || !pw_stat_shape_ok(n, cin, cout, h * w)) return false;
+  if (h < 1 || w < 4 || w % 4 != 0 || w / 4 > 64 || !(cin == 16 || cin == 32 || cin == 64 || cin == 128) ||
+      !pw_stat_shape_ok(n, cin, cout, h * w))
+    return false;
   return pw_front_rows(n, cin, cout, h, w) >= 1 && n * cin * ((w / 4 + 61) / 62) < (1ll << 31) - 1024;
 }
 
@@ -884,30 +946,35 @@
                        (const int*)c.wsum, c.bias, g, c.in_stat, (int)c.n, c.in_thr, c.levels, c.lo_neg, kEps,              \
                        c.out_current_max, c.bn_scale, c.bn_shift, c.act, c.stat_out, (int8_t*)c.x_codes_out, fa);          \
   } break;
-#define FQ_PST_FRONT(EPI_, SG_)                                                                                            \
+#define FQ_PST_FRONT(KT_, EPI_, SG_)                                                                                       \
   {                                                                                                                        \
-    static const bool attr_ok = hipFuncSetAttribute(reinterpret_cast<const void*>(&pw_stat_kernel<1, EPI_, SG_>),          \
+    static const bool attr_ok = hipFuncSetAttribute(reinterpret_cast<const void*>(&pw_stat_kernel<KT_, EPI_, SG_>),        \
                                                     hipFuncAttributeMaxDynamicSharedMemorySize, 120 * 1024) == hipSuccess; \
     FQ_REQUIRE(attr_ok, "fq_pwconv_i8_stat: cannot raise the dynamic LDS limit");                                          \
-    hipLaunchKernelGGL((pw_stat_kernel<1, EPI_, SG_>), dim3((unsigned)grid), dim3(kBlock), lds, c.st, c.x, c.wcodes,       \
+    hipLaunchKernelGGL((pw_stat_kernel<KT_, EPI_, SG_>), dim3((unsigned)grid), dim3(kBlock), lds, c.st, c.x, c.wcodes,     \
                        c.wscale, (const int*)c.wsum, c.bias, g, c.in_stat, (int)c.n, c.in_thr, c.levels, c.lo_neg, kEps,   \
                        c.out_current_max, c.bn_scale, c.bn_shift, c.act, c.stat_out, (int8_t*)c.x_codes_out, fa);          \
   }
-#define FQ_PST_FRONT_S(EPI_)                                                                                               \
+#define FQ_PST_FRONT_S(KT_, EPI_)                                                                                          \
   {                                                                                                                        \
-    if (c.front->is_signed) FQ_PST_FRONT(EPI_, true) else FQ_PST_FRONT(EPI_, false)                                        \
+    if (c.front->is_signed) FQ_PST_FRONT(KT_, EPI_, true) else FQ_PST_FRONT(KT_, EPI_, false)                              \
+  }
+#define FQ_PST_FRONT_E(KT_)                                                                                                \
+  {                                                                                                                        \
+    if (c.front->epi == kEpiBnRelu) FQ_PST_FRONT_S(KT_, kEpiBnRelu)                                                        \
+    else if (c.front->epi == kEpiBnRelu6) FQ_PST_FRONT_S(KT_, kEpiBnRelu6)                                                 \
+    else FQ_PST_FRONT_S(KT_, kEpiRuntime)                                                                                  \
   }
   if (c.front != nullptr) {
-    FQ_REQUIRE(kt == 1, "fq_pwconv_i8_stat: a front layer needs cin <= 32");
-    if (c.front->epi == kEpiBnRelu) FQ_PST_FRONT_S(kEpiBnRelu)
-    else if (c.front->epi == kEpiBnRelu6) FQ_PST_FRONT_S(kEpiBnRelu6)
-    else FQ_PST_FRONT_S(kEpiRuntime)
+    FQ_REQUIRE(kt == 1 || kt == 2 || kt == 4, "fq_pwconv_i8_stat: a front layer needs cin <= 128");
+    if (kt == 1) FQ_PST_FRONT_E(1) else if (kt == 2) FQ_PST_FRONT_E(2) else FQ_PST_FRONT_E(4)
   } else {
     switch (kt) {
       FQ_PST_GO(1) FQ_PST_GO(2) FQ_PST_GO(4) FQ_PST_GO(8)
       default: return fail(FQ_ERR_INVALID, "fq_pwconv_i8_stat: K / 32 = %d is not instantiated", kt);
     }
   }
+#undef FQ_PST_FRONT_E
 #undef FQ_PST_FRONT_S
 #undef FQ_PST_FRONT
 #undef FQ_PST_GO
@@ -929,18 +996,30 @@
   return FQ_OK;
 }
 
-int fq_pwdw_fused_supported(int64_t n, int64_t cin, int64_t cout, int64_t h, int64_t w, int stride) {
+int fq_pwdw_fused_supported(int64_t n, int64_t cin, int64_t cout, int64_t h, int64_t w, int stride, int stat_mode) {
+  if (stat_mode != 0 && !(stride == 1 && w % 4 == 0 && n * cout * h * w < (1ll << 31))) return 0;
   return pwdw_plan(n, cin, cout, h, w, stride).ok ? 1 : 0;
 }
 
-int fq_pwdw_fused(const float* x, const int8_t* wcodes, const float* wscale, const int32_t* wsum, const float* pw_bias,
-                  int64_t n, int64_t cin, int64_t cin_pad, int64_t cout_pad, int64_t cout, int64_t h, int64_t w,
-                  const float* in_stat, const float* in_thr, int in_width, unsigned in_flags, const float* pw_bn_scale,
-                  const float* pw_bn_shift, int pw_act, const float* mid_stat, const float* mid_thr, int mid_width,
-                  unsigned mid_flags, float* mid_current_max, const float* dw_w, const float* dw_bias, int dw_stride,
-                  const float* dw_bn_scale, const float* dw_bn_shift, int dw_act, float* y, float* stat_out,
-                  const void* x_codes, fqStream_t stream) {
-  FQ_REQUIRE((x || x_codes) && wcodes && wscale && wsum && dw_w && y, "fq_pwdw_fused: null pointer");
+}
+
+static int pwdw_fused_impl(const float* x, const int8_t* wcodes, const float* wscale, const int32_t* wsum, const float* pw_bias,
+                           int64_t n, int64_t cin, int64_t cin_pad, int64_t cout_pad, int64_t cout, int64_t h, int64_t w,
+                           const float* in_stat, const float* in_thr, int in_width, unsigned in_flags, const float* pw_bn_scale,
+                           const float* pw_bn_shift, int pw_act, const float* mid_stat, const float* mid_thr, int mid_width,
+                           unsigned mid_flags, float* mid_current_max, const float* dw_w, const float* dw_bias, int dw_stride,
+                           const float* dw_bn_scale, const float* dw_bn_shift, int dw_act, float* y, void* mid_codes_out,
+                           float* stat_out, const void* x_codes, fqStream_t stream) {
+  const bool ns = mid_codes_out != nullptr;
+  FQ_REQUIRE((x || x_codes) && wcodes && wscale && wsum && dw_w && (y || ns), "fq_pwdw_fused: null pointer");
+  if (ns) {
+    FQ_REQUIRE(y == nullptr && stat_out && x_codes && dw_stride == 1 && aligned16(mid_codes_out),
+               "fq_pwdw_fused: the statistic mode (mid_codes_out) wants y == NULL, stat_out, x_codes, stride 1 and a 16-byte aligned buffer");
+    FQ_REQUIRE(w % 4 == 0 && mid_width <= 8 && ((mid_flags & FQ_ACT_SIGNED) || !(mid_flags & FQ_ACT_LO_NEG_MAX)) &&
+                   n * cout * h * w < (1ll << 31) && cout * h * w < (1ll << 31) - 64,
+               "fq_pwdw_fused: statistic mode: shape or quantiser not taken (rows of whole dwords, codes that fit a byte): see "
+               "fq_pwdw_fused_supported(..., stat_mode = 1)");
+  }
   FQ_REQUIRE(in_stat != nullptr || in_thr != nullptr, "fq_pwdw_fused: give in_stat (online) or in_thr (offline)");
   FQ_REQUIRE(mid_stat != nullptr || mid_thr != nullptr, "fq_pwdw_fused: give mid_stat (the per-sample maxima of the pointwise "
              "output, from fq_pwconv_i8_stat) or mid_thr (a stored threshold)");
@@ -955,7 +1034,7 @@
   dw_act &= ~FQ_STAT_PREZEROED;
   FQ_REQUIRE(pw_act >= FQ_ACT_NONE && pw_act <= FQ_ACT_RELU6 && dw_act >= FQ_ACT_NONE && dw_act <= FQ_ACT_RELU6,
              "fq_pwdw_fused: unknown activation");
-  FQ_REQUIRE(aligned16(wcodes) && (x_codes ? aligned16(x_codes) : aligned16(x)) && aligned16(y),
+  FQ_REQUIRE(aligned16(wcodes) && (x_codes ? aligned16(x_codes) : aligned16(x)) && (ns || aligned16(y)),
              "fq_pwdw_fused: x (x_codes when given), wcodes and y must be 16-byte aligned");
   const PwDwPlan p = pwdw_plan(n, cin, cout, h, w, dw_stride);
   FQ_REQUIRE(p.ok, "fq_pwdw_fused: shape not taken (n=%lld cin=%lld cout=%lld %lldx%lld stride %d): see fq_pwdw_fused_supported",
@@ -981,31 +1060,41 @@
   if (no_fast) fast = 0;
   const double in_elems = (double)n * cin * h * w, mid_elems = (double)n * cout * h * w, out_elems = (double)n * cout * ho * wo;
   const double in_moved = x_codes ? 32.0 * p.kt * (double)n * h * w : 4.0 * in_elems;
-  ProfScope prof(FQ_KERNEL_DWCONV, 4.0 * (mid_elems + out_elems), st, in_moved + 4.0 * out_elems);
+  const double out_moved = ns ? (double)n * cout * w * (h + 2.0 * (p.bands - 1)) : 4.0 * out_elems;
+  ProfScope prof(FQ_KERNEL_DWCONV, 4.0 * (mid_elems + out_elems), st, in_moved + out_moved);
   const int8_t* xc = static_cast<const int8_t*>(x_codes);
   const unsigned grid = (unsigned)(n * p.bands);
-#define FQ_PWDW_GO(KT_, CW_, S_, LZ_, F_, C_)                                                                               \
+  const size_t lds = ns ? (size_t)(cout / 32) * p.kt * 1024 + (size_t)cout * 13 * 4 : p.lds;
+  float* const y_arg = ns ? static_cast<float*>(mid_codes_out) : y;
+#define FQ_PWDW_GO(KT_, CW_, S_, LZ_, F_, C_, NS_)                                                                          \
   {                                                                                                                        \
-    static const bool attr_ok = hipFuncSetAttribute(reinterpret_cast<const void*>(&pwdw_kernel<KT_, CW_, S_, LZ_, F_, C_>), \
-                                                    hipFuncAttributeMaxDynamicSharedMemorySize, 150 * 1024) == hipSuccess; \
+    static const bool attr_ok =                                                                                            \
+        hipFuncSetAttribute(reinterpret_cast<const void*>(&pwdw_kernel<KT_, CW_, S_, LZ_, F_, C_, NS_>),                    \
+                            hipFuncAttributeMaxDynamicSharedMemorySize, 150 * 1024) == hipSuccess;                         \
     FQ_REQUIRE(attr_ok, "fq_pwdw_fused: cannot raise the dynamic LDS limit");                                              \
-    hipLaunchKernelGGL((pwdw_kernel<KT_, CW_, S_, LZ_, F_, C_>), dim3(grid), dim3((unsigned)p.threads), p.lds, st, x, xc,   \
-                       wfrag, wscale, (const int*)wsum, pw_bias, g, in_stat, (int)n, in_thr, levels1, lo1, kEps,            \
+    hipLaunchKernelGGL((pwdw_kernel<KT_, CW_, S_, LZ_, F_, C_, NS_>), dim3(grid), dim3((unsigned)p.threads), lds, st, x,    \
+                       xc, wfrag, wscale, (const int*)wsum, pw_bias, g, in_stat, (int)n, in_thr, levels1, lo1, kEps,        \
                        pw_bn_scale, pw_bn_shift, pw_act, mid_stat, mid_thr, levels2, lo2, mid_current_max, dw_w, dw_bias,   \
-                       dw_bn_scale, dw_bn_shift, dw_act, y, stat_out);                                                     \
+                       dw_bn_scale, dw_bn_shift, dw_act, y_arg, stat_out);                                                 \
   }
 #define FQ_PWDW_C(KT_, CW_, S_, LZ_, F_)                                                                                    \
   {                                                                                                                        \
-    if (xc != nullptr) FQ_PWDW_GO(KT_, CW_, S_, LZ_, F_, 1) else FQ_PWDW_GO(KT_, CW_, S_, LZ_, F_, 0)                       \
+    if (xc != nullptr) FQ_PWDW_GO(KT_, CW_, S_, LZ_, F_, 1, 0) else FQ_PWDW_GO(KT_, CW_, S_, LZ_, F_, 0, 0)                 \
   }
 #define FQ_PWDW_F(KT_, CW_, S_, LZ_)                                                                                        \
   {                                                                                                                        \
     if (fast == 1) FQ_PWDW_C(KT_, CW_, S_, LZ_, 1) else FQ_PWDW_C(KT_, CW_, S_, LZ_, 0)                                     \
   }
+#define FQ_PWDW_N(KT_, CW_, LZ_)                                                                                            \
+  {                                                                                                                        \
+    if (fast == 1) FQ_PWDW_GO(KT_, CW_, 1, LZ_, 1, 1, 1) else FQ_PWDW_GO(KT_, CW_, 1, LZ_, 0, 1, 1)                         \
+  }
 #define FQ_PWDW_S(KT_, CW_)                                                                                                 \
   {                                                                                                                        \
     if (dw_stride == 2) FQ_PWDW_F(KT_, CW_, 2, 0)                                                                          \
-    else if (p.lz == 0) FQ_PWDW_F(KT_, CW_, 1, 0) else FQ_PWDW_F(KT_, CW_, 1, 2)                                            \
+    else if (ns) {                                                                                                         \
+      if (p.lz == 0) FQ_PWDW_N(KT_, CW_, 0) else FQ_PWDW_N(KT_, CW_, 2)                                                    \
+    } else if (p.lz == 0) FQ_PWDW_F(KT_, CW_, 1, 0) else FQ_PWDW_F(KT_, CW_, 1, 2)                                          \
   }
 #define FQ_PWDW_K(KT_)                                                                                                      \
   case KT_:                                                                                                                \
@@ -1017,6 +1106,7 @@
   }
 #undef FQ_PWDW_K
 #undef FQ_PWDW_S
+#undef FQ_PWDW_N
 #undef FQ_PWDW_F
 #undef FQ_PWDW_C
 #undef FQ_PWDW_GO
@@ -1024,4 +1114,18 @@
   return FQ_OK;
 }
 
-}
+extern "C" {
+
+int fq_pwdw_fused(const float* x, const int8_t* wcodes, const float* wscale, const int32_t* wsum, const float* pw_bias,
+                  int64_t n, int64_t cin, int64_t cin_pad, int64_t cout_pad, int64_t cout, int64_t h, int64_t w,
+                  const float* in_stat, const float* in_thr, int in_width, unsigned in_flags, const float* pw_bn_scale,
+                  const float* pw_bn_shift, int pw_act, const float* mid_stat, const float* mid_thr, int mid_width,
+                  unsigned mid_flags, float* mid_current_max, const float* dw_w, const float* dw_bias, int dw_stride,
+                  const float* dw_bn_scale, const float* dw_bn_shift, int dw_act, float* y, float* stat_out,
+                  const void* x_codes, fqStream_t stream, void* mid_codes_out) {
+  return pwdw_fused_impl(x, wcodes, wscale, wsum, pw_bias, n, cin, cin_pad, cout_pad, cout, h, w, in_stat, in_thr, in_width,
+                         in_flags, pw_bn_scale, pw_bn_shift, pw_act, mid_stat, mid_thr, mid_width, mid_flags, mid_current_max,
+                         dw_w, dw_bias, dw_stride, dw_bn_scale, dw_bn_shift, dw_act, y, mid_codes_out, stat_out, x_codes, stream);
+}
+
+}
diff --git a/quantization/mxnet_amd/ops.py b/quantization/mxnet_amd/ops.py
--- a/quantization/mxnet_amd/ops.py
+++ b/quantization/mxnet_amd/ops.py
@@ -598,7 +598,7 @@
     n, cin, h, w = (int(v) for v in xshape)
     lib = _lib_()
     return bool(lib.fq_pwconv_i8_stat_supported(n, cin, int(cout), h * w, 0, 0)) and \
-        bool(lib.fq_pwdw_fused_supported(n, cin, int(cout), h, w, int(stride)))
+        bool(lib.fq_pwdw_fused_supported(n, cin, int(cout), h, w, int(stride), 0))
 
 
 def pwconv_front_supported(xshape, cout):
@@ -668,9 +668,16 @@
     return stat
 
 
+def pwdw_chain_supported(xshape, cout):
+    n, cin, h, w = (int(v) for v in xshape)
+    lib = _lib_()
+    return lib.fq_version() >= 102 and bool(lib.fq_pwdw_fused_supported(n, cin, int(cout), h, w, 1, 1))
+
+
 def pwdw_fused(x, wcodes, wscale, wsum, dw_w, pw_bias=None, in_stat=None, in_thr=None, width=8, flags=0, pw_bn_scale=None,
                pw_bn_shift=None, pw_act=None, mid_stat=None, mid_thr=None, mid_width=8, mid_flags=0, mid_cur_out=None,
-               dw_bias=None, stride=1, dw_bn_scale=None, dw_bn_shift=None, dw_act=None, want_stat=True, x_codes=None):
+               dw_bias=None, stride=1, dw_bn_scale=None, dw_bn_shift=None, dw_act=None, want_stat=True, x_codes=None,
+               store=True, mid_codes_out=None):
     _check(x, "x")
     _check(wcodes, "wcodes", torch.int8)
     _check(wscale, "wscale")
@@ -693,14 +700,24 @@
     if x_codes is not None:
         _check_pair_codes(x_codes, "x_codes", x)
     ho, wo = (h - 1) // stride + 1, (w - 1) // stride + 1
-    y = torch.empty((n, cout, ho, wo), dtype=torch.float32, device=x.device)
+    if (mid_codes_out is None) == (not store):
+        raise ValueError("pwdw_fused keeps the codes of the 1x1 output in its statistic mode only: store=False and mid_codes_out "
+                         "go together")
+    if not store:
+        if not want_stat or stride != 1 or x_codes is None:
+            raise ValueError("pwdw_fused(store=False) wants want_stat, stride 1 and x_codes")
+        _check_front_codes(mid_codes_out, "mid_codes_out", (n, cout, h, w), x.device)
+        if not pwdw_chain_supported(x.shape, cout):
+            raise ValueError("pwdw_fused(store=False) does not take x %s -> %d channels: see pwdw_chain_supported"
+                             % (tuple(x.shape), cout))
+    y = torch.empty((n, cout, ho, wo), dtype=torch.float32, device=x.device) if store else None
     stat, zflag = _stat_target(n, x.device, want_stat)
     check_call(_lib_().fq_pwdw_fused(_ptr(x), _ptr(wcodes), _ptr(wscale), _ptr(wsum), _ptr(pw_bias), n, cin, cin_pad, cout_pad,
                                      cout, h, w, _ptr(in_stat), _ptr(in_thr), int(width), int(flags), _ptr(pw_bn_scale),
                                      _ptr(pw_bn_shift), _ACTS[pw_act], _ptr(mid_stat), _ptr(mid_thr), int(mid_width),
                                      int(mid_flags), _ptr(mid_cur_out), _ptr(dw_w), _ptr(dw_bias), int(stride),
                                      _ptr(dw_bn_scale), _ptr(dw_bn_shift), _ACTS[dw_act] | zflag, _ptr(y), _ptr(stat),
-                                     _ptr(x_codes), _stream(x)))
+                                     _ptr(x_codes), _stream(x), _ptr(mid_codes_out)))
     return y, stat
 
 
diff --git a/quantization/mxnet_amd/quantize/convert/convert_conv2d.py b/quantization/mxnet_amd/quantize/convert/convert_conv2d.py
--- a/quantization/mxnet_amd/quantize/convert/convert_conv2d.py
+++ b/quantization/mxnet_amd/quantize/convert/convert_conv2d.py
@@ -148,10 +148,11 @@
     return ops.dwconv3x3(kw.pop("x"), **kw, **more)
 
 
-def front_target(block, fz, x, plan):
+def front_target(block, fz, x, plan, level=None):
     from .. import fuse as _fuse
     nxt = fz.get("front_pw")
-    if nxt is None or not _fuse.PAIR_CODES or not (int(_fuse.PAIR_FRONT) >= 2 or (_fuse.PAIR_FRONT and ops.in_flight())) \
+    level = int(_fuse.PAIR_FRONT) if level is None else int(level)
+    if nxt is None or not _fuse.PAIR_CODES or not (level >= 2 or (level and ops.in_flight())) \
             or block._kwargs["stride"] != (1, 1) \
             or block.quantize_args.fake_bn or "in_stat" not in plan or "in_thr" in plan or plan["width"] > 8:
         return None
@@ -380,17 +381,31 @@
     return nxt
 
 
+def _front_tensor(front):
+    return front["store"]() if front.get("store") is not None else _dwconv3x3(front["call"])
+
+
 def _materialise(x):
     d = x._fq_deferred
     if d.get("kind") == "front":
-        y, stat = _dwconv3x3(d["call"])
+        y, stat = _front_tensor(d)
     else:
-        src = d["x"] if d.get("front") is None else _dwconv3x3(d["front"]["call"])[0]
+        src = d["x"] if d.get("front") is None else _front_tensor(d["front"])[0]
         y, stat = ops.pwconv_i8(src, *d["codes"], d["bias"], bn_scale=d["bn"][0], bn_shift=d["bn"][1], act=d["act"],
                                 **d["plan"])
     out = NDArray(y)
     out._fq_stat = stat
     return out
+
+
+def chain_target(block, fz, x, d, width):
+    from .. import fuse as _fuse
+    if d.get("x_codes") is None or fz.get("front_pw") is None:
+        return None
+    nxt = front_target(block, fz, x, dict(in_stat=x._fq_stat, width=width), level=_fuse.PAIR_CHAIN)
+    if nxt is None or not ops.pwdw_chain_supported(tuple(d["x"].shape), block._kwargs["num_filter"]):
+        return None
+    return nxt
 
 
 def depthwise_recompute(block, x, weight_q, bias, flags, width):
@@ -405,16 +420,31 @@
     if rows is not None and rows.device == src.device and rows.numel() >= n:
         rows[:n].copy_(stat)
     p = d["plan"]
-    z, zstat = ops.pwdw_fused(src, *d["codes"], contiguous(weight_q._t), pw_bias=d["bias"], in_stat=p["in_stat"],
+    dw_w, dw_b = contiguous(weight_q._t), None if bias is None else bias._t
+
+    def fused(**more):
+        return ops.pwdw_fused(src, *d["codes"], dw_w, pw_bias=d["bias"], in_stat=p["in_stat"],
                               width=p["width"], flags=p["flags"], pw_bn_scale=d["bn"][0], pw_bn_shift=d["bn"][1],
                               pw_act=d["act"], mid_stat=stat, mid_width=width, mid_flags=flags, mid_cur_out=cur,
-                              dw_bias=None if bias is None else bias._t, stride=block._kwargs["stride"][0],
-                              dw_bn_scale=scale, dw_bn_shift=shift, dw_act=fz["act"], x_codes=d.get("x_codes"))
+                              dw_bias=dw_b, stride=block._kwargs["stride"][0],
+                              dw_bn_scale=scale, dw_bn_shift=shift, dw_act=fz["act"], x_codes=d.get("x_codes"), **more)
+    chain = chain_target(block, fz, x, d, width)
+    if chain is not None:
+        oshape = tuple(x._t.shape)
+        ycodes = torch.empty(ops.front_codes_shape(oshape), dtype=torch.int8, device=src.device)
+        zstat = fused(store=False, mid_codes_out=ycodes)[1]
+        out = NDArray(_placeholder(oshape, src.device))
+        out._fq_stat = zstat
+        out._fq_deferred = dict(kind="front", consumer=chain, x_codes=ycodes, store=fused,
+                                call=dict(w=dw_w, bias=dw_b, bn_scale=scale, bn_shift=shift, act=fz["act"], in_stat=stat,
+                                          width=width, flags=flags))
+    else:
+        z, zstat = fused()
+        out = NDArray(z)
+        out._fq_stat = zstat
     if not side:
         block._fq_last_n = n
         block.current_input_max = DeviceScalar(cur)
-    out = NDArray(z)
-    out._fq_stat = zstat
     return out
 
 
diff --git a/quantization/mxnet_amd/quantize/fuse.py b/quantization/mxnet_amd/quantize/fuse.py
--- a/quantization/mxnet_amd/quantize/fuse.py
+++ b/quantization/mxnet_amd/quantize/fuse.py
@@ -130,6 +130,7 @@
 RECOMPUTE_MAX_CIN = int(_os.environ.get("FQ_RECOMPUTE_MAX_CIN", "128"))
 PAIR_CODES = _os.environ.get("FQ_PWDW_CODES", "1") != "0"
 PAIR_FRONT = int(_os.environ.get("FQ_PWDW_FRONT", "1"))
+PAIR_CHAIN = int(_os.environ.get("FQ_PWDW_CHAIN", "1"))
 SUBSAMPLE = _os.environ.get("FQ_SUBSAMPLE", "1") != "0"
 GAP_FUSE = _os.environ.get("FQ_GAP_FUSE", "1") != "0"
 SHORTCUT_FUSE = _os.environ.get("FQ_SHORTCUT_FUSE", "1") != "0"
```
